# QuentinHuan/ENSEM3A_OpenCLRaytracer

Hardware: AMD Instinct MI355X
Metric: Msamples/s Cornell box 1024x1024 64spp; 1/2/4/8-GPU scaling; HBM %peak (higher is better)
Workload: dtype f32; 1 GPU; cornell_1024_s64; scene=cornell, width=1024, height=1024, spp=64, max_bounce=4, traversal=fast, bvh=sah, parallelism=row-interleaved x1

## Files before the change

### ensem3a_openclraytracer_amd/_native.py

```python
from __future__ import annotations

import ctypes
import os
import threading

import numpy as np

from ._build import LIB

_lock = threading.Lock()
_lib = None
_host = None

RT_TRAVERSAL_FAST = 0
RT_TRAVERSAL_REF = 1
RT_BVH_REFERENCE = 0
RT_BVH_SAH = 1
RT_ERR_ARG = 1
RT_ERR_STATE = 3
RT_ACCUM_MAX_SAMPLES = 1 << 24

EXPORTED = (
    "rt_create", "rt_destroy", "rt_last_error", "rt_set_scene", "rt_set_env", "rt_set_option",
    "rt_render", "rt_render_device", "rt_tile_rows", "rt_count_work", "rt_count_work_detail", "rt_work_bytes", "rt_gamma",
    "rt_render_rgb8", "rt_rgb8_device", "rt_rgb8",
    "rt_accum_begin", "rt_accum_add", "rt_accum_add_rgb8", "rt_accum_read", "rt_accum_samples", "rt_accum_end",
    "rt_accum_begin_device", "rt_accum_add_device",
    "rt_accum_mark", "rt_accum_select", "rt_accum_select_mask", "rt_accum_select_all", "rt_accum_selection",
    "rt_accum_sample_map", "rt_accum_add_selected", "rt_accum_mark_device", "rt_accum_select_device",
    "rt_accum_select_mask_device", "rt_accum_select_all_device", "rt_accum_add_selected_device",
    "rt_accum_guides", "rt_accum_guides_device", "rt_denoise_device", "rt_accum_denoise",
    "rt_trace", "rt_trace_device",
    "rt_bvh_build", "rt_device_count", "rt_debug_math", "rt_debug_fn", "rt_debug_trace", "rt_debug_scene_info", "rt_debug_pixel_log",
    "rt_debug_wave_counts", "rt_debug_quantise_axis", "rt_debug_timings", "rt_debug_brute_layout",
    "rt_debug_brute_clusters", "rt_debug_brute_shell", "rt_debug_brute_near", "rt_debug_brute_slices",
    "rt_debug_last_slices",
    "rt_debug_brute_refill", "rt_debug_last_refill", "rt_debug_last_launch",
    "rt_obj_parse", "rt_obj_size", "rt_obj_copy", "rt_obj_free", "rt_obj_last_error",
    "rt_scene_check", "rt_scene_last_error",
)
HOST_ONLY = ("rt_bvh_build", "rt_obj_parse", "rt_obj_size", "rt_obj_copy", "rt_obj_free", "rt_obj_last_error",
             "rt_scene_check", "rt_scene_last_error", "rt_debug_quantise_axis", "rt_debug_brute_layout",
             "rt_debug_brute_clusters", "rt_debug_brute_shell", "rt_debug_brute_near")

_c_p = ctypes.c_void_p
_i64 = ctypes.c_int64
_i32 = ctypes.c_int


class DenoiseParams(ctypes.Structure):
    _fields_ = [("passes", ctypes.c_int), ("normal_squarings", ctypes.c_int),
                ("sigma_c", ctypes.c_float), ("sigma_p", ctypes.c_float)]

    def __init__(self, passes: int = 5, normal_squarings: int = 5, sigma_c: float = 1.5, sigma_p: float = 0.02):
        super().__init__(int(passes), int(normal_squarings), float(sigma_c), float(sigma_p))


GUIDE_FLOATS = 12

HIT_DTYPE = np.dtype([("k", np.float32), ("tri", np.int32), ("u", np.float32), ("v", np.float32)])
RAY_FLOATS = 8
RT_QUERY_CLOSEST = 0
RT_QUERY_ANY = 1
QUERY_HORIZON = 1000.0


def pack_rays(origins, directions, tmax=None) -> np.ndarray:
    o = np.asarray(origins, dtype=np.float32).reshape(-1, 3)
    d = np.asarray(directions, dtype=np.float32).reshape(-1, 3)
    if len(o) != len(d):
        raise ValueError(f"{len(o)} origins but {len(d)} directions")
    rays = np.zeros((len(o), RAY_FLOATS), np.float32)
    rays[:, 0:3] = d
    rays[:, 3:6] = o
    rays[:, 6] = QUERY_HORIZON if tmax is None else np.asarray(tmax, dtype=np.float32)
    return rays


class NativeError(RuntimeError):

    def __init__(self, status: int, message: str):
        super().__init__(f"[rt status {status}] {message}")
        self.status = status


def _preload_hip_runtime() -> None:
    import importlib.util
    try:
        spec = importlib.util.find_spec("torch")
    except (ImportError, ValueError):
        spec = None
    for d in (spec.submodule_search_locations or []) if spec else []:
        p = os.path.join(d, "lib", "libamdhip64.so")
        if os.path.exists(p):
            ctypes.CDLL(p, mode=ctypes.RTLD_GLOBAL)
            return


def lib():
    global _lib
    if _lib is not None:
        return _lib
    with _lock:
        if _lib is not None:
            return _lib
        _preload_hip_runtime()
        lib_path = os.environ.get("ENSEM3A_RT_LIB", LIB)
        if not os.path.exists(lib_path):
            raise RuntimeError(
                f"native library {lib_path} is missing: build it with "
                "`python -m ensem3a_openclraytracer_amd._build` (there is no CPU fallback)")
        L = ctypes.CDLL(lib_path)
        sig = {
            "rt_create": (_i32, [_i32, _c_p, ctypes.POINTER(_c_p)]),
            "rt_destroy": (None, [_c_p]),
            "rt_last_error": (ctypes.c_char_p, [_c_p]),
            "rt_set_scene": (_i32, [_c_p, _c_p, _i64, _c_p, _i64, _c_p, _i64, _c_p, _i64, _c_p, _i64, _c_p, _i64]),
            "rt_set_env": (_i32, [_c_p, _c_p, _i32, _i32]),
            "rt_set_option": (_i32, [_c_p, ctypes.c_char_p, _i64]),
            "rt_render": (_i32, [_c_p, _c_p, _c_p, _i64, _i32, _i32, _c_p]),
            "rt_render_device": (_i32, [_c_p, _i32, _c_p, _c_p, _i64, _i32, _i32, _i32, _i32, _c_p, _c_p]),
            "rt_tile_rows": (_i64, [_i64, _i32, _i32, _i32]),
            "rt_count_work": (_i32, [_c_p, _c_p, _c_p, _i64, _i32, _i32, _i32, _i32, _c_p]),
            "rt_count_work_detail": (_i32, [_c_p, _c_p, _c_p, _i64, _i32, _i32, _i32, _i32, _c_p]),
            "rt_work_bytes": (_i32, [_c_p, _c_p]),
            "rt_gamma": (_i32, [_c_p, _c_p, _c_p, _i64]),
            "rt_render_rgb8": (_i32, [_c_p, _c_p, _c_p, _i64, _i32, _i32, _i32, _c_p]),
            "rt_rgb8_device": (_i32, [_c_p, _i32, _c_p, _c_p, _i64, _i32, _c_p]),
            "rt_rgb8": (_i32, [_c_p, _c_p, _c_p, _i64, _i32]),
            "rt_accum_begin": (_i32, [_c_p, _c_p, _c_p, _i64, _i32]),
            "rt_accum_add": (_i32, [_c_p, _i32, _c_p]),
            "rt_accum_add_rgb8": (_i32, [_c_p, _i32, _i32, _c_p]),
            "rt_accum_read": (_i32, [_c_p, _c_p]),
            "rt_accum_samples": (_i64, [_c_p]),
            "rt_accum_end": (_i32, [_c_p]),
            "rt_accum_begin_device": (_i32, [_c_p, _i32, _c_p, _c_p, _i64, _i32, _i32, _i32]),
            "rt_accum_add_device": (_i32, [_c_p, _i32, _i32, _c_p, _c_p]),
            "rt_accum_mark": (_i32, [_c_p]),
            "rt_accum_select": (_i32, [_c_p, ctypes.c_float, ctypes.POINTER(_i64)]),
            "rt_accum_select_mask": (_i32, [_c_p, _c_p]),
            "rt_accum_select_all": (_i32, [_c_p]),
            "rt_accum_selection": (_i32, [_c_p, _c_p]),
            "rt_accum_sample_map": (_i32, [_c_p, _c_p]),
            "rt_accum_add_selected": (_i32, [_c_p, _i32, _c_p]),
            "rt_accum_mark_device": (_i32, [_c_p, _i32, _c_p]),
            "rt_accum_select_device": (_i32, [_c_p, _i32, ctypes.c_float, _c_p]),
            "rt_accum_select_mask_device": (_i32, [_c_p, _i32, _c_p, _c_p]),
            "rt_accum_select_all_device": (_i32, [_c_p, _i32, _c_p]),
            "rt_accum_add_selected_device": (_i32, [_c_p, _i32, _i32, _c_p, _c_p]),
            "rt_accum_guides": (_i32, [_c_p, _c_p]),
            "rt_accum_guides_device": (_i32, [_c_p, _i32, _c_p, _c_p]),
            "rt_denoise_device": (_i32, [_c_p, _i32, _c_p, _c_p, _i64, _i32, ctypes.POINTER(DenoiseParams), _c_p, _c_p]),
            "rt_accum_denoise": (_i32, [_c_p, ctypes.POINTER(DenoiseParams), _c_p]),
            "rt_trace": (_i32, [_c_p, _c_p, _i64, _i32, _c_p]),
            "rt_trace_device": (_i32, [_c_p, _i32, _c_p, _i64, _i32, _c_p, _c_p]),
            "rt_bvh_build": (_i32, [_c_p, _i64, _c_p, _i64, _c_p, ctypes.POINTER(_i64)]),
            "rt_device_count": (_i32, []),
            "rt_obj_parse": (_i32, [_c_p, _i64, ctypes.POINTER(_c_p)]),
            "rt_obj_size": (_i64, [_c_p, _i32]),
            "rt_obj_copy": (_i32, [_c_p, _c_p, _c_p, _c_p, _c_p]),
            "rt_obj_free": (None, [_c_p]),
            "rt_obj_last_error": (ctypes.c_char_p, []),
            "rt_scene_check": (_i32, [_c_p, _i64, _c_p, _i64, _c_p, _i64, _c_p, _i64, _c_p, _i64, _i32, _c_p]),
            "rt_scene_last_error": (ctypes.c_char_p, []),
            "rt_debug_brute_layout": (_i32, [_c_p, _i64, _c_p, _i64, _c_p, _i64, _c_p, _i64, _c_p, _i64, _i32, _c_p, _i64,
                                             _c_p]),
            "rt_debug_brute_clusters": (_i32, [_c_p, _i64, _c_p, _i64, _c_p, _i64, _c_p, _i64, _c_p, _i64, _i32, _i32,
                                               _c_p, _i64, _c_p, _i64, _c_p]),
            "rt_debug_brute_shell": (_i32, [_c_p, _i64, _c_p, _i64, _c_p, _i64, _c_p, _i64, _c_p, _i64, _i32, _i32, _i32,
                                            _c_p, _i64, _c_p]),
            "rt_debug_brute_near": (_i32, [_c_p, _i64, _c_p, _i64, _c_p, _i64, _c_p, _i64, _c_p, _i64, _i32, _i32, _i32,
                                           _c_p, _i64, _c_p, _c_p]),
            "rt_debug_brute_slices": (_i32, [_i64, _i64, _i32, _i32, _i32, _c_p]),
            "rt_debug_last_slices": (_i32, []),
            "rt_debug_brute_refill": (_i32, [_i64, _i64, _i32, _c_p]),
            "rt_debug_last_refill": (_i32, [_c_p]),
            "rt_debug_last_launch": (_i32, [_c_p]),
            "rt_debug_math": (_i32, [_c_p, _i32, _c_p, _c_p, _c_p, _i64]),
            "rt_debug_fn": (_i32, [_c_p, _i32, _c_p, _c_p, _i64]),
            "rt_debug_trace": (_i32, [_c_p, _i32, _c_p, _c_p, _i64]),
            "rt_debug_scene_info": (_i32, [_c_p, _c_p]),
            "rt_debug_timings": (_i32, [_c_p, _c_p]),
            "rt_debug_wave_counts": (_i32, [_c_p, _c_p, _c_p, _i64, _i32, _i32, _c_p]),
            "rt_debug_pixel_log": (_i32, [_c_p, _i32, _c_p, _c_p, _i64, _i32, _i32, _i64, _c_p, _i32, _c_p, _c_p]),
        }
        _bind(L, sig)
        _lib = L
    return _lib


_HOST_SIG = {}


def _bind(L, sig, names=None):
    for name, (res, args) in sig.items():
        if names is not None and name not in names:
            continue
        fn = getattr(L, name)
        fn.restype = res
        fn.argtypes = args
        if name in HOST_ONLY:
            _HOST_SIG[name] = (res, args)


def host_lib():
    global _host
    if _host is not None:
        return _host
    L = lib()
    path = os.environ.get("ENSEM3A_HOST_LIB")
    if path:
        with _lock:
            if _host is None:
                H = ctypes.CDLL(path)
                _bind(H, _HOST_SIG)
                _host = H
        return _host
    _host = L
    return _host


def check(status: int, ctx=None) -> None:
    if status != 0:
        msg = lib().rt_last_error(ctx)
        raise NativeError(status, msg.decode(errors="replace") if msg else "unknown error")


def f32(a) -> np.ndarray:
    return np.ascontiguousarray(a, dtype=np.float32)


def i32(a) -> np.ndarray:
    return np.ascontiguousarray(a, dtype=np.int32)


def ptr(a: np.ndarray):
    return a.ctypes.data if a is not None and a.size else None


def device_count() -> int:
    return int(lib().rt_device_count())


class Context:

    def __init__(self, n_devices: int = 1, device_ids=None):
        ids = None
        if device_ids is not None:
            ids = (ctypes.c_int * len(device_ids))(*device_ids)
            n_devices = len(device_ids)
        out = _c_p()
        check(lib().rt_create(int(n_devices), ids, ctypes.byref(out)))
        self._ctx = out
        self.n_devices = int(n_devices)

# ... 286 lines not shown

    def wave_counts(self, cam, env, npix, spp, max_bounce):
        c, e = f32(cam), f32(env)
        out = np.zeros(9, dtype=np.uint64)
        self._check(lib().rt_debug_wave_counts(self.handle, ptr(c), ptr(e), int(npix), int(spp), int(max_bounce),
                                               out.ctypes.data))
        keys = ("node_fetches", "tri_tests", "rays", "env_lookups", "stack_drops", "wave_trav_iters",
                "wave_render_iters", "cycles_shade", "cycles_trav")
        return {k: int(v) for k, v in zip(keys, out)}

    def scene_info(self):
        out = np.zeros(8, dtype=np.int64)
        self._check(lib().rt_debug_scene_info(self.handle, out.ctypes.data))
        return dict(fast_ok=bool(out[0]), depth=int(out[1]), nodes=int(out[2]), tris=int(out[3]),
                    brute_records=int(out[4]), brute_boxes=int(out[5]), wdq_omax=int(out[6]) * 1e-6)

    def timings(self) -> dict:
        out = np.zeros(4, dtype=np.float64)
        self._check(lib().rt_debug_timings(self.handle, out.ctypes.data))
        return dict(pack_ms=float(out[0]), upload_ms=float(out[1]), env_ms=float(out[2]), render_ms=float(out[3]))


def parse_obj(text):
    data = text.encode() if isinstance(text, str) else bytes(text)
    h = _c_p()
    H = host_lib()
    if H.rt_obj_parse(data, len(data), ctypes.byref(h)) != 0:
        raise ValueError("OBJ parse failed: " + H.rt_obj_last_error().decode(errors="replace"))
    try:
        n = [int(H.rt_obj_size(h, k)) for k in range(5)]
        vp, vn, vuv = (np.zeros(n[k], np.float32) for k in range(3))
        face = np.zeros(n[3], np.int32)
        H.rt_obj_copy(h, vp.ctypes.data, vn.ctypes.data, vuv.ctypes.data, face.ctypes.data)
    finally:
        H.rt_obj_free(h)
    return vp, vn, vuv, face, n[4]


def scene_check(V_p, V_n, faceData, materialData, bvh, layout: int = RT_BVH_SAH) -> dict:
    vp, vn, face, mat, b = f32(V_p), f32(V_n), i32(faceData), f32(materialData), f32(bvh)
    info = np.zeros(8, np.int64)
    H = host_lib()
    st = H.rt_scene_check(ptr(vp), vp.size, ptr(vn), vn.size, ptr(face), face.size, ptr(mat), mat.size,
                          ptr(b), b.size, int(layout), info.ctypes.data)
    msg = H.rt_scene_last_error().decode(errors="replace")
    if st != 0:
        raise NativeError(st, msg)
    return dict(tris=int(info[0]), nodes=int(info[1]), depth=int(info[2]), wnodes=int(info[3]),
                wdepth=int(info[4]), brute_records=int(info[5]), brute_boxes=int(info[6]), fast_ok=bool(info[7]),
                note=msg)


def brute_layout(V_p, V_n, faceData, materialData, bvh, layout: int = RT_BVH_SAH):
    vp, vn, face, mat, b = f32(V_p), f32(V_n), i32(faceData), f32(materialData), f32(bvh)
    H = host_lib()
    info = np.zeros(3, np.int64)
    args = (ptr(vp), vp.size, ptr(vn), vn.size, ptr(face), face.size, ptr(mat), mat.size, ptr(b), b.size, int(layout))
    st = H.rt_debug_brute_layout(*args, None, 0, info.ctypes.data)
    if st != 0:
        raise NativeError(st, H.rt_scene_last_error().decode(errors="replace"))
    boxes = np.zeros(int(info[2]), np.float32)
    st = H.rt_debug_brute_layout(*args, boxes.ctypes.data, boxes.size, info.ctypes.data)
    if st != 0:
        raise NativeError(st, H.rt_scene_last_error().decode(errors="replace"))
    return boxes.reshape(-1, 8), int(info[0]), int(info[1])


def brute_clusters(V_p, V_n, faceData, materialData, bvh, cluster: int = -1, layout: int = RT_BVH_SAH):
    vp, vn, face, mat, b = f32(V_p), f32(V_n), i32(faceData), f32(materialData), f32(bvh)
    H = host_lib()
    info = np.zeros(4, np.int64)
    args = (ptr(vp), vp.size, ptr(vn), vn.size, ptr(face), face.size, ptr(mat), mat.size, ptr(b), b.size, int(layout),
            int(cluster))
    st = H.rt_debug_brute_clusters(*args, None, 0, None, 0, info.ctypes.data)
    if st != 0:
        raise NativeError(st, H.rt_scene_last_error().decode(errors="replace"))
    slots, rows = np.zeros(int(info[2]), np.float32), np.zeros(int(info[3]), np.float32)
    st = H.rt_debug_brute_clusters(*args, slots.ctypes.data, slots.size, rows.ctypes.data, rows.size, info.ctypes.data)
    if st != 0:
        raise NativeError(st, H.rt_scene_last_error().decode(errors="replace"))
    return slots.reshape(-1, 8), rows.reshape(-1, 8), int(info[1])


SHELL_REC_FLOATS = 20


def brute_shell(V_p, V_n, faceData, materialData, bvh, cluster: int = -1, shell: int = -1, layout: int = RT_BVH_SAH):
    vp, vn, face, mat, b = f32(V_p), f32(V_n), i32(faceData), f32(materialData), f32(bvh)
    H = host_lib()
    info = np.zeros(3, np.int64)
    args = (ptr(vp), vp.size, ptr(vn), vn.size, ptr(face), face.size, ptr(mat), mat.size, ptr(b), b.size, int(layout),
            int(cluster), int(shell))
    st = H.rt_debug_brute_shell(*args, None, 0, info.ctypes.data)
    if st != 0:
        raise NativeError(st, H.rt_scene_last_error().decode(errors="replace"))
    if int(info[0]) == 0:
        return None
    rec = np.zeros(int(info[2]), np.float32)
    st = H.rt_debug_brute_shell(*args, rec.ctypes.data, rec.size, info.ctypes.data)
    if st != 0:
        raise NativeError(st, H.rt_scene_last_error().decode(errors="replace"))
    ints = rec[:SHELL_REC_FLOATS].view(np.int32)
    return dict(box=rec[:6].copy(), nrest=int(ints[6]), nfaces=int(ints[7]), faces=ints[8:20].reshape(6, 2).copy(),
                rest=rec[SHELL_REC_FLOATS:].reshape(-1, 8).copy())


NEAR_FLOOR = np.float32(0.0001) * (np.float32(1.0) - np.float32(2.0 ** -12))


def brute_near(V_p, V_n, faceData, materialData, bvh, cluster: int = -1, shell: int = -1, layout: int = RT_BVH_SAH):
    vp, vn, face, mat, b = f32(V_p), f32(V_n), i32(faceData), f32(materialData), f32(bvh)
    H = host_lib()
    info = np.zeros(2, np.int64)
    floor = np.zeros(1, np.float32)
    args = (ptr(vp), vp.size, ptr(vn), vn.size, ptr(face), face.size, ptr(mat), mat.size, ptr(b), b.size, int(layout),
            int(cluster), int(shell))
    st = H.rt_debug_brute_near(*args, None, 0, floor.ctypes.data, info.ctypes.data)
    if st != 0:
        raise NativeError(st, H.rt_scene_last_error().decode(errors="replace"))
    flags = np.zeros(int(info[0]), np.int32)
    st = H.rt_debug_brute_near(*args, flags.ctypes.data if flags.size else None, flags.size, floor.ctypes.data,
                               info.ctypes.data)
    if st != 0:
        raise NativeError(st, H.rt_scene_last_error().decode(errors="replace"))
    return flags.astype(bool), np.float32(floor[0]), int(info[1])


def brute_slices(nloc: int, lanes: int, spp: int, option: int = -1, accum_base: int = -1):
    out = np.zeros(3, np.int32)
    st = lib().rt_debug_brute_slices(int(nloc), int(lanes), int(spp), int(option), int(accum_base), out.ctypes.data)
    if st != 0:
        raise NativeError(st, "rt_debug_brute_slices: bad arguments")
    return bool(out[0]), int(out[1]), int(out[2])


def last_slices() -> int:
    return int(lib().rt_debug_last_slices())


def brute_refill(nloc: int, lanes: int, option: int = -1) -> int:
    out = np.zeros(1, np.int32)
    st = lib().rt_debug_brute_refill(int(nloc), int(lanes), int(option), out.ctypes.data)
    if st != 0:
        raise NativeError(st, "rt_debug_brute_refill: bad arguments")
    return int(out[0])


def last_refill():
    out = np.zeros(3, np.int64)
    st = lib().rt_debug_last_refill(out.ctypes.data)
    if st != 0:
        raise NativeError(st, "rt_debug_last_refill: bad arguments")
    return int(out[0]), int(out[1]), int(out[2])


LAUNCH_FIELDS = ("trav", "count", "log", "smem", "ovf", "resume", "step", "wide", "brute", "ts", "acc",
                 "team", "walk_team", "slices", "refill", "grid", "lds", "shell", "near")
BRUTE_SLICED = 4
BRUTE_REFILL = 8


def last_launch() -> dict:
    out = np.zeros(len(LAUNCH_FIELDS), np.int32)
    st = lib().rt_debug_last_launch(out.ctypes.data)
    if st != 0:
        raise NativeError(st, "rt_debug_last_launch: bad arguments")
    return {name: int(v) for name, v in zip(LAUNCH_FIELDS, out)}


def tile_rows(npix: int, width: int, row0: int, row_step: int) -> int:
    return int(lib().rt_tile_rows(int(npix), int(width), int(row0), int(row_step)))
```

### ensem3a_openclraytracer_amd/csrc/rt_api.hip

```cpp
#include <hip/hip_runtime.h>

#include <cmath>
#include <cstdarg>
#include <cstdio>
#include <algorithm>
#include <array>
#include <atomic>
#include <chrono>
#include <cstring>
#include <map>
#include <string>
#include <thread>
#include <vector>

#include "../../include/rt_api.h"
#include "../../include/rt_debug.h"
#include "rt_internal.h"
#include "scene_pack.h"

constexpr int kResumeMinBvh2 = 36, kResumeMinWide = 48;
constexpr int kDenoiseLds = 1;

using rt::HostScene;

namespace {

thread_local std::string g_thread_error;

struct DevBuf {
    void* p = nullptr;
    size_t bytes = 0;
    DevBuf() = default;
    DevBuf(const DevBuf&) = delete;
    DevBuf& operator=(const DevBuf&) = delete;
    DevBuf(DevBuf&& o) noexcept : p(o.p), bytes(o.bytes) { o.p = nullptr, o.bytes = 0; }
    DevBuf& operator=(DevBuf&& o) noexcept {
        std::swap(p, o.p);
        std::swap(bytes, o.bytes);
        return *this;
    }
    ~DevBuf() { release(); }
    void release() {
        if (p) (void)hipFree(p);
        p = nullptr;
        bytes = 0;
    }
};

struct Device {
    int id = 0;
    hipStream_t stream = nullptr;
    int cus = 0;
    DevBuf stack_ovf;
    DevBuf nodes, wnodes, wleaves, tri_fast, brute, brute_box, brute_cbox, brute_crow, bvh9, tri_geo, tri_shade, tri_frame, mat, ibl, ibl_sum, out, out8, counts, work, scratch_a, scratch_b;
    DevBuf pilot;
    DevBuf spec;
    DevBuf slice;
    DevBuf accum;
    bool acc_open = false;
    bool acc_valid = false;
    float acc_cam[10] = {0}, acc_env[5] = {0};
    int64_t acc_npix = 0, acc_nloc = 0, acc_samples = 0;
    int acc_max_bounce = 0, acc_row0 = 0, acc_row_step = 1;
    DevBuf mark, sel, all;
    bool acc_marked = false, acc_selected = false, acc_all_ready = false;
    bool acc_uniform = true;
    bool sel_all = false;
    int64_t sel_known = -1;
    int64_t acc_full = 0;
    DevBuf dn, dn_const, guides, dn_rgb, dn_guides, dn_out;
    DevBuf q_counter, q_rays, q_out;
    char* host_stage = nullptr;
    int* host_pick = nullptr;
    size_t host_stage_bytes = 0;
    hipEvent_t done = nullptr;
    hipStream_t last = nullptr;
    bool pending = false;

    Device() = default;
    Device(const Device&) = delete;
    Device& operator=(const Device&) = delete;
    ~Device() {
        (void)hipSetDevice(id);
        if (host_stage) (void)hipHostFree(host_stage);
        if (host_pick) (void)hipHostFree(host_pick);
        if (stream) (void)hipStreamDestroy(stream);
        if (done) (void)hipEventDestroy(done);
    }
};

}

struct rt_ctx {
    std::vector<Device> devs;
    HostScene hs;
    bool have_scene = false;
    bool have_env = false;
    int ibl_w = 0, ibl_h = 0;
    int traversal = RT_TRAVERSAL_FAST;
    int bvh_layout = RT_BVH_SAH;
    int brute_max = RT_BRUTE_MAX_DEFAULT;
    int brute_cluster = -1;
    int brute_shell = -1;
    int brute_near = -1;
    int resume_min = -1;
    int team = 0;
    int walk_team = 0;
    int max_waves = 0;
    int step = 0;
    int sun_skip = 1;
    int sun_any = 1;
    int block = 128;
    int bvh_width = 0;
    int fixed_point = 1;
    int sun_cache = 1;
    int pilot = -1;
    int pilot_chunk = 0;
    int pilot_levels = 0;
    int stack_lds = 0;
    int ref_stack = 20;
    int spec = -1;
    int wdq = 1;
    int handout = -1;
    int slices = -1;
    int brute_refill = -1;
    int denoise_lds = -1;
    int query_engine = 0;
    int query_grid = 0;
    bool accum_host = false;
    double t_pack_ms = 0, t_upload_ms = 0, t_env_ms = 0, t_render_ms = 0;
    std::string err;
};

namespace {

int set_err(rt_ctx* ctx, int code, const char* fmt, ...) {
    char buf[1024];
    va_list ap;
    va_start(ap, fmt);
    vsnprintf(buf, sizeof buf, fmt, ap);
    va_end(ap);
    if (ctx) ctx->err = buf;
    g_thread_error = buf;
    return code;
}

#define HIP_OR_RET(ctx, call)                                                                           \
    do {                                                                                                \
        hipError_t e_ = (call);                                                                         \
        if (e_ != hipSuccess)                                                                           \
            return set_err((ctx), RT_ERR_HIP, "%s failed: %s", #call, hipGetErrorString(e_));           \
    } while (0)

hipError_t grow(Device& d, DevBuf& b, size_t bytes) {
    bytes = std::max<size_t>(bytes, 16);
    if (b.p && b.bytes >= bytes) return hipSuccess;
    hipError_t e = d.pending ? hipEventSynchronize(d.done) : hipSuccess;
    if (e != hipSuccess) return e;
    if (b.p && (e = hipFree(b.p)) != hipSuccess) return e;
    b.p = nullptr;
    b.bytes = 0;
    if ((e = hipMalloc(&b.p, bytes)) == hipSuccess) b.bytes = bytes;
    return e;
}

hipError_t grow_stage(Device& d, size_t bytes) {
    if (d.host_stage_bytes >= bytes) return hipSuccess;
    hipError_t e = d.host_stage ? hipHostFree(d.host_stage) : hipSuccess;
    if (e != hipSuccess) return e;
    d.host_stage = nullptr;
    d.host_stage_bytes = 0;
    if ((e = hipHostMalloc((void**)&d.host_stage, bytes, hipHostMallocDefault)) == hipSuccess) d.host_stage_bytes = bytes;
    return e;
}

}

namespace {

constexpr int kStackLdsMin = 8;
hipError_t ensure_stack_ovf(Device& d, const HostScene& hs) {
    const int64_t extra = (int64_t)std::max(hs.depth, hs.wdepth) - kStackLdsMin;
    if (extra <= 0) return hipSuccess;
    return grow(d, d.stack_ovf, (size_t)std::max(d.cus, 1) * rt::kMaxLanesPerCu * (size_t)extra * sizeof(int2));
}

hipError_t order_after_last(Device& d, hipStream_t s) {
// ... 6 lines not shown
    d.pending = true;
    return hipEventRecord(d.done, s);
}

template <typename T>
hipError_t upload(Device& d, DevBuf& b, const std::vector<T>& v) {
    const size_t bytes = v.size() * sizeof(T);
    hipError_t e = grow(d, b, bytes);
    if (e != hipSuccess || bytes == 0) return e;
    return hipMemcpyAsync(b.p, v.data(), bytes, hipMemcpyHostToDevice, d.stream);
}

hipError_t upload_cbox(Device& d, const HostScene& hs) {
    if (hs.brute_shell.empty()) return upload(d, d.brute_cbox, hs.brute_cbox);
    std::vector<float> v(hs.brute_cbox);
    v.insert(v.end(), hs.brute_shell.begin(), hs.brute_shell.end());
    const hipError_t e = upload(d, d.brute_cbox, v);
    return e != hipSuccess ? e : hipStreamSynchronize(d.stream);
}

int upload_fast(rt_ctx* ctx, Device& d, const HostScene& hs) {
    HIP_OR_RET(ctx, hipSetDevice(d.id));
    HIP_OR_RET(ctx, order_after_last(d, d.stream));
    HIP_OR_RET(ctx, upload(d, d.nodes, hs.nodes));
    HIP_OR_RET(ctx, upload(d, d.wnodes, hs.wnodes));
    HIP_OR_RET(ctx, upload(d, d.wleaves, hs.wleaves));
    HIP_OR_RET(ctx, upload(d, d.brute, hs.brute));
    HIP_OR_RET(ctx, upload(d, d.brute_box, hs.brute_box));
    HIP_OR_RET(ctx, upload_cbox(d, hs));
    HIP_OR_RET(ctx, upload(d, d.brute_crow, hs.brute_crow));
    HIP_OR_RET(ctx, upload(d, d.tri_geo, hs.tri_geo));
    HIP_OR_RET(ctx, upload(d, d.tri_fast, hs.tri_fast));
    HIP_OR_RET(ctx, ensure_stack_ovf(d, hs));
    return RT_OK;
}

int effective_traversal(const rt_ctx* ctx) {
    return (ctx->traversal == RT_TRAVERSAL_FAST && ctx->hs.fast_ok) ? RT_TRAVERSAL_FAST : RT_TRAVERSAL_REF;
}

bool use_wide(const rt_ctx* ctx) {
    if (ctx->hs.wnodes.empty() || ctx->bvh_width == 2) return false;
    return ctx->bvh_width == 4 || (size_t)ctx->hs.nnodes * 16 * rt::kNodeF4 > rt::kWideMinBytes;
}

int resume_min_of(const rt_ctx* ctx) {
    return ctx->resume_min >= 0 ? ctx->resume_min : use_wide(ctx) ? kResumeMinWide : kResumeMinBvh2;
}

rt::DevScene dev_scene(const rt_ctx* ctx, const Device& d) {
    rt::DevScene s{};
    s.nodes = (const float4*)d.nodes.p;
    s.nnodes = ctx->hs.nnodes;
    s.root_ref = ctx->hs.root_ref;
    const bool wide = use_wide(ctx);
    s.wnodes = wide ? (const float4*)d.wnodes.p : nullptr;
    s.wleaves = wide ? (const float4*)d.wleaves.p : nullptr;
    s.wroot_ref = ctx->hs.wroot_ref;
    s.wdq_omax = wide ? ctx->hs.wdq_omax : 0.0f;
    for (int k = 0; k < 6; ++k) s.root_box[k] = ctx->hs.root_box[k];
    s.bvh9 = (const float*)d.bvh9.p;
    s.nbvh9 = ctx->hs.nbvh9;
    s.ref_stack = ctx->ref_stack;
    s.tri_geo = (const float4*)d.tri_geo.p;
    s.tri_fast = (const float4*)d.tri_fast.p;
    s.tri_shade = (const float4*)d.tri_shade.p;
    s.tri_frame = (const float4*)d.tri_frame.p;
    s.ntri = ctx->hs.ntri;
    s.mat = (const float*)d.mat.p;
    s.nmat = ctx->hs.nmat;
    s.ibl_sum = (const uint32_t*)d.ibl_sum.p;
    s.ibl_w = ctx->ibl_w;
    s.ibl_h = ctx->ibl_h;
    s.depth = wide ? std::max(ctx->hs.depth, ctx->hs.wdepth) : ctx->hs.depth;
    s.brute = (const float4*)d.brute.p;
    s.brute_box = (const float4*)d.brute_box.p;
    s.nbrute = ctx->hs.nbrute;
    s.nbox = ctx->hs.nbox;
    s.brute_cbox = (const float4*)d.brute_cbox.p;
    s.brute_crow = (const float4*)d.brute_crow.p;
    s.ncluster = ctx->hs.ncluster;
    s.ncslot = (int32_t)(ctx->hs.brute_cbox.size() / 8);
    s.nsingle4 = s.ncslot - rt::kClusterSlots * s.ncluster;
    s.cluster_auto = ctx->brute_cluster < 0 ? 1 : 0;
    s.nsingle = ctx->hs.nsingle;
    s.shell = ctx->hs.nshell > 0 ? 2 * s.ncslot : 0;
    s.near_floor = s.shell && ctx->brute_near != 0 ? ctx->hs.shell_floor : 0.0f;
    s.near_mask_lo = s.near_floor != 0.0f ? (uint32_t)ctx->hs.shell_mask : 0u;
    s.near_mask_hi = s.near_floor != 0.0f ? (uint32_t)(ctx->hs.shell_mask >> 32) : 0u;
    s.stack_lds = std::min<int32_t>(s.depth > 0 ? s.depth : 1,
                                    ctx->stack_lds > 0 ? ctx->stack_lds : wide ? rt::kStackLdsWide : rt::kStackLds);
    s.stack_ovf = (int2*)d.stack_ovf.p;
    return s;
}

int check_frame(rt_ctx* ctx, const float* cam, const float* env, int64_t npix, int spp, int max_bounce, int row0,
                int row_step, rt::FrameParams* fp) {
    if (!ctx) return set_err(nullptr, RT_ERR_ARG, "null context");
    if (!ctx->have_scene) return set_err(ctx, RT_ERR_STATE, "rt_set_scene has not been called");
    if (!ctx->have_env) return set_err(ctx, RT_ERR_STATE, "rt_set_env has not been called");
    if (!cam || !env) return set_err(ctx, RT_ERR_ARG, "cam/env must not be NULL");
    if (!(cam[6] >= 1.0f) || !(cam[6] < 2147483648.0f))
        return set_err(ctx, RT_ERR_ARG, "cam[6] (row width) must be >= 1, got %g", (double)cam[6]);
    if (npix <= 0 || npix > 0x7fffffff) return set_err(ctx, RT_ERR_ARG, "pixel count %lld out of range", (long long)npix);
    if (spp < 0) return set_err(ctx, RT_ERR_ARG, "spp must be >= 0");
    if (row0 < 0 || row_step <= 0) return set_err(ctx, RT_ERR_ARG, "bad row tiling (%d, %d)", row0, row_step);
    if (max_bounce > 4096) return set_err(ctx, RT_ERR_ARG, "maxBounce %d > 4096", max_bounce);
    std::memcpy(fp->cam, cam, sizeof fp->cam);
    std::memcpy(fp->env, env, sizeof fp->env);
    fp->width = (int32_t)cam[6];
    fp->npix = npix;
    fp->spp = spp;
    fp->max_bounce = max_bounce;
    fp->row0 = row0;
    fp->row_step = row_step;
    fp->nloc = rt_tile_rows(npix, fp->width, row0, row_step) * fp->width;
    fp->log_pixel = -1;
    fp->resume_min = resume_min_of(ctx);
    fp->step = ctx->step;
    fp->sun_skip = (ctx->sun_skip && env[3] == 0.0f && env[4] >= 0.0f && ctx->hs.colors_finite) ? 1 : 0;
    fp->sun_any = (ctx->sun_any && !ctx->hs.has_glass) ? 1 : 0;
    fp->wide = use_wide(ctx) ? 1 : 0;
    fp->wdq = ctx->wdq;
    fp->fixed_point = ctx->fixed_point;
    fp->sun_cache = ctx->fixed_point && ctx->sun_cache ? 1 : 0;
    fp->pass = 0;
    fp->pilot = 0;
    fp->pilot_chunk = 1;
    fp->pilot_levels = 256;
    fp->pilot_state = nullptr;
    fp->pilot_draws = nullptr;
    fp->spec = 0;
    fp->spec_log = nullptr;
    fp->spec_cap = 0;
    fp->slices = 0;
    fp->refill = ctx->brute_refill;
    fp->slice_state = nullptr;
    fp->slice_ready = nullptr;
    fp->pilot_cost = nullptr;
    fp->pilot_order = nullptr;
    fp->team = ctx->team;
    fp->walk_team = ctx->walk_team;
    fp->max_waves = ctx->max_waves;
    fp->handout = ctx->handout >= 0 ? ctx->handout : (use_wide(ctx) && effective_traversal(ctx) == RT_TRAVERSAL_FAST);
    fp->log_buf = nullptr;
    fp->log_cap = 0;
    fp->log_count = nullptr;
    return RT_OK;
}

void invalidate_accum(rt_ctx* ctx) {
    for (auto& d : ctx->devs) {
        d.acc_valid = false;
        d.acc_marked = false;
        d.acc_selected = false;
    }
}

int slot_of(rt_ctx* ctx, int device_index, Device** d, const char* what = "device index") {
    if (!ctx) return set_err(nullptr, RT_ERR_ARG, "null context");
    if (device_index < 0 || device_index >= (int)ctx->devs.size())
        return set_err(ctx, RT_ERR_ARG, "%s %d out of range", what, device_index);
    *d = &ctx->devs[device_index];
    return RT_OK;
}

int repack_scene(rt_ctx* ctx) {
    if (!ctx->have_scene) return RT_OK;
    HostScene& hs = ctx->hs;
    std::string why;
    rt::pack_checked(hs, hs.bvh9.data(), hs.nbvh9, hs.ntri, ctx->bvh_layout, ctx->brute_max, ctx->brute_cluster,
                     ctx->brute_shell, why);
    for (auto& d : ctx->devs) {
        const int st = upload_fast(ctx, d, hs);
        if (st) return st;
        HIP_OR_RET(ctx, hipStreamSynchronize(d.stream));
    }
    if (!hs.fast_ok) ctx->err = "FAST traversal unavailable (" + why + "); REF traversal will be used";
    return RT_OK;
}

struct Accepts {
    enum Kind { kRange, kZeroOrRange, kSet } kind;
    int n;
    int64_t v[5];
    bool operator()(int64_t x) const {
        if (kind == kSet) return std::find(v, v + n, x) != v + n;
        return (kind == kZeroOrRange && x == 0) || (x >= v[0] && x <= v[1]);
    }
};
Accepts range(int64_t lo, int64_t hi) { return {Accepts::kRange, 2, {lo, hi}}; }
Accepts zero_or(int64_t lo, int64_t hi) { return {Accepts::kZeroOrRange, 2, {lo, hi}}; }
Accepts one_of(std::initializer_list<int64_t> members) {
    Accepts a{Accepts::kSet, (int)members.size(), {}};
    std::copy(members.begin(), members.end(), a.v);
    return a;
}

enum class Effect { kNone, kInvalidate, kRepack };

struct Option {
    const char* key;
    int rt_ctx::*field;
    Accepts accepts;
    std::string message;
    Effect effect;
};

std::string bounds_message(const char* fmt, int a, int b = 0) {
    char buf[128];
    snprintf(buf, sizeof buf, fmt, a, b);
    return buf;
}

const std::vector<Option>& options() {
    constexpr Effect none = Effect::kNone, invalidate = Effect::kInvalidate, repack = Effect::kRepack;
    static const std::vector<Option> table = {
        {"traversal", &rt_ctx::traversal, range(RT_TRAVERSAL_FAST, RT_TRAVERSAL_REF), "traversal must be 0 (fast) or 1 (ref)", invalidate},
        {"brute_near", &rt_ctx::brute_near, range(-1, 1), "brute_near must be -1 (auto), 0 (off) or 1 (auto)", none},
        {"bvh", &rt_ctx::bvh_layout, range(RT_BVH_REFERENCE, RT_BVH_SAH), "bvh must be 0 (reference tree) or 1 (sah)", repack},
        {"brute_cluster", &rt_ctx::brute_cluster, range(-1, 1), "brute_cluster must be -1 (auto), 0 (off) or 1 (force)", repack},
        {"brute_shell", &rt_ctx::brute_shell, range(-1, 1), "brute_shell must be -1 (auto), 0 (off) or 1 (force)", repack},
        {"brute_max", &rt_ctx::brute_max, range(0, 4096), "brute_max must be in 0..4096", repack},
        {"resume_min", &rt_ctx::resume_min, range(-1, 64), "resume_min must be -1 (auto) or 0..64", none},
        {"team", &rt_ctx::team, one_of({0, 1, 2, 4, 8}), "team must be 0 (auto), 1, 2, 4 or 8", none},
        {"walk_team", &rt_ctx::walk_team, one_of({0, 1, 2, 4, 8}), "walk_team must be 0 (auto), 1, 2, 4 or 8", none},
        {"sun_any", &rt_ctx::sun_any, range(0, 1), "sun_any must be 0 or 1", none},
        {"sun_skip", &rt_ctx::sun_skip, range(0, 1), "sun_skip must be 0 or 1", none},
        {"step", &rt_ctx::step, range(0, 2), "step must be 0 (auto), 1 (item) or 2 (round)", none},
        {"waves", &rt_ctx::max_waves, range(0, 8), "waves must be in 0..8", none},
        {"pilot", &rt_ctx::pilot, range(-1, 1 << 20), "pilot must be -1 (auto), 0 (off) or a sample count", none},
        {"pilot_chunk", &rt_ctx::pilot_chunk, range(0, 4096), "pilot_chunk must be in 0..4096 (0 = auto)", none},
        {"pilot_levels", &rt_ctx::pilot_levels, zero_or(2, 256), "pilot_levels must be 0 (auto) or 2..256", none},
        {"stack_lds", &rt_ctx::stack_lds, zero_or(kStackLdsMin, rt::kStackLds),
         bounds_message("stack_lds must be 0 (auto) or %d..%d", kStackLdsMin, rt::kStackLds), none},
        {"sun_cache", &rt_ctx::sun_cache, range(0, 1), "sun_cache must be 0 or 1", none},
        {"fixed_point", &rt_ctx::fixed_point, range(0, 1), "fixed_point must be 0 or 1", none},
        {"bvh_width", &rt_ctx::bvh_width, one_of({0, 2, 4}), "bvh_width must be 0 (auto), 2 or 4", none},
        {"ref_stack", &rt_ctx::ref_stack, range(20, 64), "ref_stack must be in 20..64 (20 = the reference's)", invalidate},
        {"slices", &rt_ctx::slices, range(-1, 16), "slices must be -1 (auto), 0 (off) or 1..16", none},
        {"brute_refill", &rt_ctx::brute_refill, range(-1, rt::kRefillMax),
         bounds_message("brute_refill must be -1 (auto), 0 or 1 (off) or 2..%d", rt::kRefillMax), none},
        {"denoise_lds", &rt_ctx::denoise_lds, range(-1, 1), "denoise_lds must be -1 (auto), 0 or 1", none},
        {"query_engine", &rt_ctx::query_engine, range(0, 2), "query_engine must be 0 (auto), 1 (plain) or 2 (persistent)", none},
        {"query_grid", &rt_ctx::query_grid, range(0, 1 << 20), "query_grid must be 0 (auto) or a block count", none},
        {"wdq", &rt_ctx::wdq, range(0, 1), "wdq must be 0 or 1", none},
        {"handout", &rt_ctx::handout, range(-1, 1), "handout must be -1 (auto), 0 or 1", none},
        {"spec", &rt_ctx::spec, one_of({-1, 0, 2, 4, 8}), "spec must be -1 (auto), 0 (off), 2, 4 or 8", none},
        {"block", &rt_ctx::block, one_of({64, 128, 256}), "block must be 64/128/256", none},
    };
    return table;
}

}

extern "C" {

int rt_device_count(void) {
    int n = 0;
    if (hipGetDeviceCount(&n) != hipSuccess) return 0;
    return n;
}

int rt_create(int n_devices, const int* device_ids, rt_ctx** out) {
    if (!out) return set_err(nullptr, RT_ERR_ARG, "out must not be NULL");
    *out = nullptr;
    int avail = 0;
    hipError_t e = hipGetDeviceCount(&avail);
    if (e != hipSuccess || avail <= 0)
        return set_err(nullptr, RT_ERR_HIP, "no HIP device available (%s)", hipGetErrorString(e));
    if (n_devices <= 0) n_devices = 1;
    if (!device_ids && n_devices > avail)
        return set_err(nullptr, RT_ERR_ARG, "requested %d devices, %d available", n_devices, avail);
    if (n_devices > 64) return set_err(nullptr, RT_ERR_ARG, "at most 64 device slots, got %d", n_devices);
    rt_ctx* ctx = new rt_ctx();
    ctx->devs = std::vector<Device>(n_devices);
    for (int i = 0; i < n_devices; ++i) {
        const int id = device_ids ? device_ids[i] : i;
        if (id < 0 || id >= avail) {
            delete ctx;
            return set_err(nullptr, RT_ERR_ARG, "device id %d out of range", id);
        }
        ctx->devs[i].id = id;
        if ((e = hipSetDevice(id)) != hipSuccess ||
            (e = hipStreamCreateWithFlags(&ctx->devs[i].stream, hipStreamNonBlocking)) != hipSuccess ||
            (e = hipEventCreateWithFlags(&ctx->devs[i].done, hipEventDisableTiming)) != hipSuccess ||
            (e = hipDeviceGetAttribute(&ctx->devs[i].cus, hipDeviceAttributeMultiprocessorCount, id)) != hipSuccess) {
            rt_destroy(ctx);
            return set_err(nullptr, RT_ERR_HIP, "device %d init failed: %s", id, hipGetErrorString(e));
        }
    }
    *out = ctx;
    return RT_OK;
}

void rt_destroy(rt_ctx* ctx) {
    if (!ctx) return;
    for (auto& d : ctx->devs) {
        if (hipSetDevice(d.id) != hipSuccess) continue;
        if (d.pending) (void)hipEventSynchronize(d.done);
        if (d.stream) (void)hipStreamSynchronize(d.stream);
    }
    delete ctx;
}

const char* rt_last_error(rt_ctx* ctx) { return ctx ? ctx->err.c_str() : g_thread_error.c_str(); }

int rt_set_option(rt_ctx* ctx, const char* key, int64_t value) {
    if (!ctx || !key) return set_err(ctx, RT_ERR_ARG, "null argument");
    for (const Option& o : options()) {
        if (std::strcmp(key, o.key)) continue;
        if (!o.accepts(value)) return set_err(ctx, RT_ERR_ARG, "%s", o.message.c_str());
        ctx->*o.field = (int)value;
        if (o.effect == Effect::kInvalidate) invalidate_accum(ctx);
        return o.effect == Effect::kRepack ? repack_scene(ctx) : RT_OK;
    }
    return set_err(ctx, RT_ERR_ARG, "unknown option '%s'", key);
}

int rt_set_scene(rt_ctx* ctx, const float* vp, int64_t nvp, const float* vn, int64_t nvn, const float* vuv,
                 int64_t nvuv, const int32_t* face, int64_t nface, const float* mat, int64_t nmat, const float* bvh9,
                 int64_t nbvh) {
    (void)vuv;
    (void)nvuv;
    if (!ctx) return set_err(nullptr, RT_ERR_ARG, "null context");
    const auto t0 = std::chrono::steady_clock::now();
    HostScene hs;
    std::string msg, why;
    const int rc = rt::scene_prepare(hs, vp, nvp, vn, nvn, face, nface, mat, nmat, bvh9, nbvh, ctx->bvh_layout,
                                     ctx->brute_max, ctx->brute_cluster, ctx->brute_shell, msg, why);
    if (rc != RT_OK) return set_err(ctx, rc, "%s", msg.c_str());
    invalidate_accum(ctx);
    const auto t1 = std::chrono::steady_clock::now();
    for (auto& d : ctx->devs) {
        const int st = upload_fast(ctx, d, hs);
        if (st) return st;
        HIP_OR_RET(ctx, upload(d, d.bvh9, hs.bvh9));
        HIP_OR_RET(ctx, upload(d, d.tri_shade, hs.tri_shade));
        HIP_OR_RET(ctx, upload(d, d.mat, hs.mat));
        HIP_OR_RET(ctx, grow(d, d.tri_frame, (size_t)std::max<int64_t>(hs.ntri, 1) * 3 * sizeof(float4)));
        HIP_OR_RET(ctx, grow(d, d.work, rt::kWorkBytes));
        HIP_OR_RET(ctx, hipStreamSynchronize(d.stream));
    }
    ctx->hs = std::move(hs);
    for (auto& d : ctx->devs) {
        HIP_OR_RET(ctx, hipSetDevice(d.id));
        HIP_OR_RET(ctx, rt::launch_prep_frames(dev_scene(ctx, d), (float4*)d.tri_frame.p, d.stream));
        HIP_OR_RET(ctx, hipStreamSynchronize(d.stream));
    }
    ctx->have_scene = true;
    ctx->t_pack_ms = std::chrono::duration<double, std::milli>(t1 - t0).count();
    ctx->t_upload_ms = std::chrono::duration<double, std::milli>(std::chrono::steady_clock::now() - t1).count();
    if (!ctx->hs.fast_ok) ctx->err = "FAST traversal unavailable (" + why + "); REF traversal will be used";
    return RT_OK;
}

int rt_set_env(rt_ctx* ctx, const uint8_t* rgba, int w, int h) {
    if (!ctx) return set_err(nullptr, RT_ERR_ARG, "null context");
    if (!rgba || w <= 0 || h <= 0) return set_err(ctx, RT_ERR_ARG, "bad IBL image (%d x %d)", w, h);
    const size_t bytes = (size_t)w * h * 4;
    invalidate_accum(ctx);
    const auto t0 = std::chrono::steady_clock::now();
    for (auto& d : ctx->devs) {
        HIP_OR_RET(ctx, hipSetDevice(d.id));
        HIP_OR_RET(ctx, order_after_last(d, d.stream));
        HIP_OR_RET(ctx, grow(d, d.ibl, bytes));
        HIP_OR_RET(ctx, grow(d, d.ibl_sum, (size_t)(w + 1) * (size_t)(h + 1) * sizeof(uint32_t)));
        HIP_OR_RET(ctx, hipMemcpyAsync(d.ibl.p, rgba, bytes, hipMemcpyHostToDevice, d.stream));
        HIP_OR_RET(ctx, rt::launch_ibl_sum((const uchar4*)d.ibl.p, w, h, (uint32_t*)d.ibl_sum.p, d.stream));
        HIP_OR_RET(ctx, hipStreamSynchronize(d.stream));
    }
    ctx->ibl_w = w;
    ctx->ibl_h = h;
    ctx->have_env = true;
    ctx->t_env_ms = std::chrono::duration<double, std::milli>(std::chrono::steady_clock::now() - t0).count();
    return RT_OK;
}

int64_t rt_tile_rows(int64_t npix, int width, int row0, int row_step) {
    if (npix <= 0 || width <= 0 || row0 < 0 || row_step <= 0) return 0;
    const int64_t H = (npix + width - 1) / width;
    if (row0 >= H) return 0;
    return (H - row0 + row_step - 1) / row_step;
}

namespace {
constexpr int kSlicesWide = 8;
constexpr int kSlicesWideSmall = 12;
constexpr int64_t kSlicesMinPerLane = 4;
using rt::kAccumSliceMin;

hipError_t setup_pilot(rt_ctx* ctx, Device& d, rt::FrameParams& fp) {
    if (ctx->pilot == 0 || effective_traversal(ctx) != RT_TRAVERSAL_FAST || fp.nloc <= 0 || use_wide(ctx))
        return hipSuccess;
    int k = ctx->pilot;
    if (k < 0) {
        const int64_t lanes = (int64_t)std::max(d.cus, 1) * rt::kWalkLanesPerCu;
        if (ctx->hs.nbrute > 0 || use_wide(ctx) || fp.spp < 16 || fp.nloc > 16 * lanes) return hipSuccess;
        if (ctx->slices != 0 && fp.nloc >= kSlicesMinPerLane * lanes) return hipSuccess;
        k = fp.spp / 8;
    }
    if (k >= fp.spp) return hipSuccess;
    const size_t n = (size_t)fp.nloc;
    const size_t need = n * 40 + 2 * 256 * sizeof(uint32_t) + 2 * (n + 1) * sizeof(uint32_t) +
                        (n + 256) * sizeof(uint32_t) + n * sizeof(uint32_t);
    hipError_t e = grow(d, d.pilot, need);
    if (e != hipSuccess) return e;
    char* base = (char*)d.pilot.p;
    fp.pilot = k;
    fp.pilot_chunk = ctx->pilot_chunk > 0 ? ctx->pilot_chunk : (ctx->hs.nbrute > 0 ? 64 : 1);
    fp.pilot_levels = ctx->pilot_levels > 0 ? ctx->pilot_levels : 256;
    fp.pilot_state = (float4*)base;
    fp.pilot_cost = (uint32_t*)(base + n * 32);
// ... 973 lines not shown
    Device& d = ctx->devs[0];
    HIP_OR_RET(ctx, hipSetDevice(d.id));
    const size_t ibytes = (size_t)n * wi * sizeof(float);
    const size_t obytes = ((size_t)n * wo * sizeof(float) + 15) & ~(size_t)15;
    HIP_OR_RET(ctx, grow(d, d.scratch_a, ibytes));
    HIP_OR_RET(ctx, grow(d, d.scratch_b, obytes + rt::debug_fn_scratch_bytes(fn, n)));
    HIP_OR_RET(ctx, hipMemcpyAsync(d.scratch_a.p, in, ibytes, hipMemcpyHostToDevice, d.stream));
    HIP_OR_RET(ctx, order_after_last(d, d.stream));
    HIP_OR_RET(ctx, rt::launch_debug_fn(dev_scene(ctx, d), fn, (const float*)d.scratch_a.p, (float*)d.scratch_b.p, n,
                                        (char*)d.scratch_b.p + obytes, d.stream));
    HIP_OR_RET(ctx, hipMemcpyAsync(out, d.scratch_b.p, (size_t)n * wo * sizeof(float), hipMemcpyDeviceToHost, d.stream));
    HIP_OR_RET(ctx, hipStreamSynchronize(d.stream));
    return RT_OK;
}

int rt_debug_trace(rt_ctx* ctx, int traversal, const float* rays, float* out, int64_t n) {
    if (!ctx || !rays || !out || n < 0) return set_err(ctx, RT_ERR_ARG, "bad arguments");
    if (!ctx->have_scene) return set_err(ctx, RT_ERR_STATE, "no scene");
    if (traversal == RT_TRAVERSAL_FAST && !ctx->hs.fast_ok)
        return set_err(ctx, RT_ERR_STATE, "FAST traversal unavailable for this scene");
    if (!n) return RT_OK;
    Device& d = ctx->devs[0];
    HIP_OR_RET(ctx, hipSetDevice(d.id));
    HIP_OR_RET(ctx, grow(d, d.scratch_a, (size_t)n * 6 * sizeof(float)));
    HIP_OR_RET(ctx, grow(d, d.scratch_b, (size_t)n * 2 * sizeof(float)));
    HIP_OR_RET(ctx, hipMemcpyAsync(d.scratch_a.p, rays, (size_t)n * 6 * sizeof(float), hipMemcpyHostToDevice, d.stream));
    HIP_OR_RET(ctx, order_after_last(d, d.stream));
    HIP_OR_RET(ctx, rt::launch_debug_trace(dev_scene(ctx, d), traversal, (const float*)d.scratch_a.p,
                                           (float*)d.scratch_b.p, n, d.stream));
    HIP_OR_RET(ctx, hipMemcpyAsync(out, d.scratch_b.p, (size_t)n * 2 * sizeof(float), hipMemcpyDeviceToHost, d.stream));
    HIP_OR_RET(ctx, hipStreamSynchronize(d.stream));
    return RT_OK;
}

int rt_debug_pixel_log(rt_ctx* ctx, int traversal, const float cam[10], const float env[5], int64_t npix, int spp,
                       int max_bounce, int64_t pixel, float* log, int cap, int* n_events, float out3[3]) {
    rt::FrameParams fp;
    if (!cam) return set_err(ctx, RT_ERR_ARG, "null cam");
    const int W = (int)cam[6];
    if (W <= 0 || pixel < 0 || pixel >= npix) return set_err(ctx, RT_ERR_ARG, "pixel out of range");
    int st = check_frame(ctx, cam, env, npix, spp, 0, (int)(pixel / W), (int)npix, &fp);
    if (st) return st;
    if (!log || cap <= 0 || !n_events || !out3) return set_err(ctx, RT_ERR_ARG, "bad log buffer");
    if (traversal == RT_TRAVERSAL_FAST && !ctx->hs.fast_ok) traversal = RT_TRAVERSAL_REF;
    fp.max_bounce = max_bounce;
    fp.sun_skip = 0;
    fp.sun_any = 0;
    Device& d = ctx->devs[0];
    HIP_OR_RET(ctx, hipSetDevice(d.id));
    const size_t obytes = (size_t)fp.nloc * 3 * sizeof(float);
    const size_t lbytes = (size_t)cap * 16 * sizeof(float);
    HIP_OR_RET(ctx, grow(d, d.scratch_a, obytes + lbytes + 16));
    float* dout = (float*)d.scratch_a.p;
    fp.log_buf = dout + fp.nloc * 3;
    fp.log_count = (int32_t*)(fp.log_buf + (size_t)cap * 16);
    fp.log_cap = cap;
    fp.log_pixel = pixel;
    HIP_OR_RET(ctx, hipMemsetAsync(fp.log_count, 0, sizeof(int32_t), d.stream));
    HIP_OR_RET(ctx, order_after_last(d, d.stream));
    HIP_OR_RET(ctx, rt::launch_debug_log(dev_scene(ctx, d), fp, traversal, dout, (unsigned int*)d.work.p, d.stream));
    HIP_OR_RET(ctx, mark_launch(d, d.stream));
    int32_t n = 0;
    HIP_OR_RET(ctx, hipMemcpyAsync(&n, fp.log_count, sizeof n, hipMemcpyDeviceToHost, d.stream));
    HIP_OR_RET(ctx, hipStreamSynchronize(d.stream));
    if (n > cap) n = cap;
    HIP_OR_RET(ctx, hipMemcpy(log, fp.log_buf, (size_t)n * 16 * sizeof(float), hipMemcpyDeviceToHost));
    HIP_OR_RET(ctx, hipMemcpy(out3, dout + 3 * (pixel % W), 3 * sizeof(float), hipMemcpyDeviceToHost));
    *n_events = n;
    return RT_OK;
}

int rt_debug_brute_slices(int64_t nloc, int64_t lanes, int spp, int option, int accum_base, int32_t out[3]) {
    if (!out || nloc < 0 || lanes < 0 || option < -1 || option > 16) return RT_ERR_ARG;
    const int todo = spp - std::max(accum_base, 0);
    const int v = rt::brute_slice_launch(rt::brute_slice_offer(option, todo, accum_base >= 0), nloc, lanes);
    out[0] = v != 0;
    out[1] = v & 0xff;
    out[2] = v >> 8;
    return RT_OK;
}

int rt_debug_last_slices(void) { return rt::last_launch().slices; }

int rt_debug_last_launch(int32_t out[19]) {
    if (!out) return RT_ERR_ARG;
    const rt::LaunchNote n = rt::last_launch();
    const rt::KernelKey& k = n.key;
    const int64_t v[19] = {k.trav, k.count, k.log,  k.smem,       k.ovf,    k.resume, k.step, k.wide,          k.brute,
                           k.ts,   k.acc,   n.team, n.walk_team,  n.slices, n.refill, n.grid, (int64_t)n.lds,
                           n.shell, n.near};
    for (int i = 0; i < 19; ++i) out[i] = (int32_t)std::min<int64_t>(v[i], INT32_MAX);
    return RT_OK;
}

int rt_debug_brute_refill(int64_t nloc, int64_t lanes, int option, int32_t* out) {
    if (!out || nloc < 0 || lanes < 0 || option < -1 || option > rt::kRefillMax) return RT_ERR_ARG;
    *out = rt::brute_refill_launch(option, nloc, lanes);
    return RT_OK;
}

int rt_debug_last_refill(int64_t out[3]) {
    if (!out) return RT_ERR_ARG;
    out[0] = rt::last_launch().refill;
    out[1] = g_refill_events.load(std::memory_order_relaxed);
    out[2] = g_refill_lanes.load(std::memory_order_relaxed);
    return RT_OK;
}

int rt_debug_timings(rt_ctx* ctx, double out[4]) {
    if (!ctx || !out) return set_err(ctx, RT_ERR_ARG, "bad arguments");
    out[0] = ctx->t_pack_ms;
    out[1] = ctx->t_upload_ms;
    out[2] = ctx->t_env_ms;
    out[3] = ctx->t_render_ms;
    return RT_OK;
}

int rt_debug_scene_info(rt_ctx* ctx, int64_t out[8]) {
    if (!ctx || !out) return set_err(ctx, RT_ERR_ARG, "bad arguments");
    out[0] = ctx->hs.fast_ok ? 1 : 0;
    out[1] = ctx->hs.depth;
    out[2] = ctx->hs.nnodes;
    out[3] = ctx->hs.ntri;
    out[4] = effective_traversal(ctx) == RT_TRAVERSAL_FAST ? ctx->hs.nbrute : 0;
    out[5] = out[4] ? ctx->hs.nbox : 0;
    out[6] = ctx->hs.wnodes.empty() ? 0 : (int64_t)std::llround((double)ctx->hs.wdq_omax * 1e6);
    out[7] = 0;
    return RT_OK;
}

}
```

### ensem3a_openclraytracer_amd/csrc/rt_device.h

```cpp
#pragma once
#include <algorithm>
#include <climits>

#include "rt_internal.h"
#include "rtm.h"

namespace rt {

namespace {

constexpr size_t kLdsSceneMax = 24 * 1024;

constexpr int TRAV_FAST = 0;
constexpr int TRAV_REF = 1;
constexpr int REF_STACK = 20;

struct Hit {
    float k;
    int tri;
};

struct Cnt {
    unsigned long long nodes, tris, rays, env, dropped;
    unsigned long long wave_trav;
// ... 261 lines not shown
    const char* const tb = reinterpret_cast<const char*>(tris);
    const unsigned kstride = SOA ? 16u * (unsigned)S.nnodes : 16u;
    const float ix = dev_recip(d.x), iy = dev_recip(d.y), iz = dev_recip(d.z);
    float tmin, tmax;
    slab(S.root_box[0], S.root_box[3], S.root_box[1], S.root_box[4], S.root_box[2], S.root_box[5], o, ix, iy, iz,
         tmin, tmax);
    if (!(tmax >= tmin && tmax >= 0.0f)) return best;
    int item = S.root_ref;
    unsigned soff = 0;
    while (true) {
        if (COUNT) count_wave(c.wave_trav);
        if (item >= 0) {
            if (COUNT) { c.nodes++; c.boxes += 2; }
            const char* np = nb + (SOA ? 16u : 16u * kNodeF4) * (unsigned)item;
            const int next = node_step<OVF>(np, kstride, o, ix, iy, iz, best.k * CULL_MARGIN, st, soff);
            if (next != INT_MIN) {
                item = next;
                continue;
            }
        } else {
            if (COUNT) c.tris++;
            float k;
            int rank;
            const unsigned toff = ~(unsigned)item;
            int index;
            if (mt_flat(tb, toff, o, d, &k, &rank, &index) && k > 0.0001f &&
                (k < best.k || (k == best.k && rank < best_rank))) {
                best.k = k;
                best.tri = 48 * index;
                best_rank = rank;
            }
        }
        item = 0x7fffffff;
        while (soff > 0) {
            soff -= sstride;
            const int2 en = st.template get<OVF>(soff);
            if (__int_as_float(en.y) <= best.k * CULL_MARGIN) {
                item = en.x;
                break;
            }
        }
        if (item == 0x7fffffff) break;
    }
    if (best.tri >= 0) best.tri = (int)((unsigned)best.tri / 48u);
    return best;
}

typedef const float __attribute__((address_space(4))) const_f;
struct ConstF4 {
    const const_f* p;
    __device__ __forceinline__ float4 operator[](int i) const {
        return make_float4(p[4 * i], p[4 * i + 1], p[4 * i + 2], p[4 * i + 3]);
    }
};
__device__ __forceinline__ ConstF4 as_const(const float4* p) {
    return ConstF4{(const const_f*)(const float*)(p)};
}

__device__ __forceinline__ float sgpr1(float x) {
    return __int_as_float(__builtin_amdgcn_readfirstlane(__float_as_int(x)));
}
__device__ __forceinline__ float4 sgpr4(float4 v) {
    return make_float4(sgpr1(v.x), sgpr1(v.y), sgpr1(v.z), sgpr1(v.w));
}

constexpr unsigned BRUTE_RING = 256u;
constexpr unsigned BRUTE_OWNERS = 128u;
constexpr int BRUTE_INV_OFF = 64 * 6 * 4 + 64 * 8 + (BRUTE_RING + 64) * 4;
constexpr int BRUTE_WAVE_LDS = BRUTE_INV_OFF + 64 * 3 * 4 + BRUTE_OWNERS * 4;
static_assert(kClusterLockNum >= 0 && kClusterLockNum <= 8 && BRUTE_OWNERS >= 64 + 64 / kClusterSlots + 2, "owner list");

__device__ __forceinline__ unsigned lane_prefix(unsigned long long m, unsigned base) {
    return __builtin_amdgcn_mbcnt_hi((unsigned)(m >> 32), __builtin_amdgcn_mbcnt_lo((unsigned)m, base));
}

__device__ __forceinline__ void wave_lds_sync() {
    __builtin_amdgcn_fence(__ATOMIC_SEQ_CST, "wavefront");
    __builtin_amdgcn_wave_barrier();
}

__device__ __forceinline__ float near_floor_of(const DevScene& S, int g) {
    const uint32_t m = g < 32 ? S.near_mask_lo : S.near_mask_hi;
    return g < 64 && ((m >> (g & 31)) & 1u) ? kNearFloor : 0.0f;
}

template <int N> struct IntC { static constexpr int value = N; };
static_assert(kBoxGroup == 1 || kBoxGroup == 2 || kBoxGroup == 4 || kBoxGroup == 8, "the lock-step tail is cut into powers of two");

template <bool COUNT, bool CLU = false>
__device__ Hit trace_brute_compact(const DevScene& S, rtm_f3 o, rtm_f3 d, char* wl, const float4* mtrec,
                                   unsigned mtstride, Cnt& c, int ts = 1, const float4* boxrec = nullptr) {
    const unsigned lane = threadIdx.x & 63;
    const unsigned sub = lane & (unsigned)(ts - 1), tl = lane - sub;
    if (COUNT && sub == 0) c.rays++;
    const unsigned long long act = __ballot(1);
    const int nact = __popcll(act);
    const int myrank = (int)lane_prefix(act, 0u);
    float* ray = reinterpret_cast<float*>(wl);
    unsigned long long* bestk = reinterpret_cast<unsigned long long*>(wl + 64 * 6 * 4);
    unsigned* ring = reinterpret_cast<unsigned*>(wl + 64 * 6 * 4 + 64 * 8);
    ray[0 * 64 + lane] = o.x; ray[1 * 64 + lane] = o.y; ray[2 * 64 + lane] = o.z;
    ray[3 * 64 + lane] = d.x; ray[4 * 64 + lane] = d.y; ray[5 * 64 + lane] = d.z;
    const unsigned long long nokey = ((unsigned long long)__float_as_uint(1000.0f) << 32) | 0xffffffffull;
    bestk[lane] = nokey;
    wave_lds_sync();
    const float ix = dev_recip(d.x), iy = dev_recip(d.y), iz = dev_recip(d.z);
    float bk = 1000.0f;
    unsigned head = 0, tail = 0;
    auto run_batch = [&](int n) __attribute__((always_inline)) {
        if (myrank < n) {
            const unsigned e = ring[(head + myrank) & (BRUTE_RING - 1)];
            const unsigned ow = e >> 16, q = e & 0xffffu;
            const rtm_f3 ro = rtm_v3(ray[ow], ray[64 + ow], ray[128 + ow]);
            const rtm_f3 rd = rtm_v3(ray[192 + ow], ray[256 + ow], ray[320 + ow]);
            const float4* rq = mtrec + mtstride * q;
            const float4 r1 = rq[0], r2 = rq[1], r3 = rq[2];
            const rtm_f3 a = rtm_v3(r1.z, r1.w, r2.x), e1 = rtm_v3(r2.y, r2.z, r2.w), e2 = rtm_v3(r3.x, r3.y, r3.z);
            const rtm_f3 h = rtm_cross(rd, e2);
            const float det = rtm_dot(e1, h);
            const float f = mt_recip(det);
            const rtm_f3 sv = rtm_sub(ro, a);
            const float u = f * rtm_dot(sv, h);
            const rtm_f3 qv = rtm_cross(sv, e1);
            const float v = f * rtm_dot(rd, qv);
            const float k = f * rtm_dot(e2, qv);
            const bool parallel = det > -0.0000001f && det < 0.0000001f;
            const bool hit = !parallel && !(u < 0.0f || u > 1.0f) && !(v < 0.0f || u + v > 1.0f) &&
                             (k > 0.0000001f) && k > 0.0001f && k < 1000.0f;
            if (hit) atomicMin(&bestk[ow], ((unsigned long long)__float_as_uint(k) << 32) | q);
        }
        head += n;
        wave_lds_sync();
    };
    auto enqueue = [&](bool pass, unsigned qa, int qb) __attribute__((always_inline)) {
        const unsigned long long m = __ballot(pass);
        if (m == 0) return;
        const unsigned n = (unsigned)__popcll(m);
        if (COUNT && pass) c.tris += qb >= 0 ? 2 : 1;
        const unsigned r = lane_prefix(m, tail);
        ring[pass ? (r & (BRUTE_RING - 1)) : BRUTE_RING + lane] = (tl << 16) | qa;
        if (qb >= 0) ring[pass ? ((r + n) & (BRUTE_RING - 1)) : BRUTE_RING + lane] = (tl << 16) | (unsigned)qb;
        tail += qb >= 0 ? 2 * n : n;
        wave_lds_sync();
        if ((int)(tail - head) >= nact) {
            do run_batch(nact); while ((int)(tail - head) >= nact);
            bk = __uint_as_float((unsigned)(bestk[tl] >> 32));
        }
    };
    auto group = [&](auto wc, const ConstF4 cb, int g0, int nreal) __attribute__((always_inline)) {
        constexpr int W = decltype(wc)::value;
        float4 bx[2 * W];
#pragma unroll
        for (int j = 0; j < 2 * W; ++j) bx[j] = sgpr4(cb[2 * g0 + j]);
        const float cull = bk * CULL_MARGIN;
        bool pass[W];
#pragma unroll
        for (int j = 0; j < W; ++j) {
            float tn, tx;
            slab(bx[2 * j].x, bx[2 * j].y, bx[2 * j].z, bx[2 * j].w, bx[2 * j + 1].x, bx[2 * j + 1].y, o, ix, iy, iz,
                 tn, tx);
            if constexpr (COUNT && !CLU) pass[j] = fmaxf(tn, near_floor_of(S, g0 + j)) <= fminf(tx, cull);
            else pass[j] = box_hit(tn, tx, cull);
        }
#pragma unroll
        for (int j = 0; j < W; ++j) {
            if (COUNT && g0 + j >= nreal) break;
            const int qa = __float_as_int(bx[2 * j + 1].z), qb = __float_as_int(bx[2 * j + 1].w);
            if (COUNT) {
                c.boxes++;
                count_wave(c.wave_trav); c.nodes++;
                if (qb >= 0) { count_wave(c.wave_trav); c.nodes++; }
            }
            enqueue(pass[j], (unsigned)qa, qb);
        }
    };
    auto lockstep_padded = [&](const ConstF4 cb, int gb, int ge) __attribute__((always_inline)) {
        for (int g0 = gb; g0 < ge; g0 += kBoxGroup) group(IntC<kBoxGroup>{}, cb, g0, ge);
    };
    auto lockstep = [&](const ConstF4 cb, int gb, int ge) __attribute__((always_inline)) {
        int g0 = gb;
        for (; g0 + kBoxGroup <= ge; g0 += kBoxGroup) group(IntC<kBoxGroup>{}, cb, g0, ge);
        const int rem = ge - g0;
        if constexpr (kBoxGroup > 4) if (rem & 4) group(IntC<4>{}, cb, g0 + (rem & ~7), ge);
        if constexpr (kBoxGroup > 2) if (rem & 2) group(IntC<2>{}, cb, g0 + (rem & ~3), ge);
        if constexpr (kBoxGroup > 1) if (rem & 1) group(IntC<1>{}, cb, g0 + (rem & ~1), ge);
    };
    if (CLU) {
        float* inv = reinterpret_cast<float*>(wl + BRUTE_INV_OFF);
        unsigned* olist = reinterpret_cast<unsigned*>(wl + BRUTE_INV_OFF + 64 * 3 * 4);
        const unsigned* besthi = reinterpret_cast<const unsigned*>(bestk) + 1;
        inv[lane] = ix; inv[64 + lane] = iy; inv[128 + lane] = iz;
        const ConstF4 cb = as_const(S.brute_cbox);
        ConstF4 sb = cb;
        int ns = S.nsingle;
        if (S.shell) {
            const ConstF4 sh{cb.p + 4 * S.shell};
            const float4 h0 = sgpr4(sh[0]), h1 = sgpr4(sh[1]), fx = sgpr4(sh[2]), fy = sgpr4(sh[3]), fz = sgpr4(sh[4]);
            const float cull = bk * CULL_MARGIN, nearf = S.near_floor;
            const float x0 = (h0.x - o.x) * ix, x1 = (h0.y - o.x) * ix;
            const float y0 = (h0.z - o.y) * iy, y1 = (h0.w - o.y) * iy;
            const float z0 = (h1.x - o.z) * iz, z1 = (h1.y - o.z) * iz;
            const float t[6] = {x0, x1, y0, y1, z0, z1};
            const float mn[3] = {fminf(x0, x1), fminf(y0, y1), fminf(z0, z1)};
            const float mx[3] = {fmaxf(x0, x1), fmaxf(y0, y1), fmaxf(z0, z1)};
            const int q[12] = {__float_as_int(fx.x), __float_as_int(fx.y), __float_as_int(fx.z), __float_as_int(fx.w),
                               __float_as_int(fy.x), __float_as_int(fy.y), __float_as_int(fy.z), __float_as_int(fy.w),
                               __float_as_int(fz.x), __float_as_int(fz.y), __float_as_int(fz.z), __float_as_int(fz.w)};
            bool pass[6];
#pragma unroll
            for (int f = 0; f < 6; ++f) {
                const int a = f >> 1;
                const float tn = fmaxf(fmaxf(a == 0 ? t[f] : mn[0], a == 1 ? t[f] : mn[1]), a == 2 ? t[f] : mn[2]);
                const float tx = fminf(fminf(a == 0 ? t[f] : mx[0], a == 1 ? t[f] : mx[1]), a == 2 ? t[f] : mx[2]);
                pass[f] = fmaxf(tn, nearf) <= fminf(tx, cull);
            }
            unsigned long long many = 0;
            int npass = 0;
#pragma unroll
            for (int f = 0; f < 6; ++f) {
                const unsigned long long mf = __ballot(pass[f]);
                many |= mf;
                npass += __popcll(mf);
            }
            if (npass == __popcll(many)) {
                unsigned pk = ~0u;
#pragma unroll
                for (int f = 0; f < 6; ++f) pk = pass[f] ? ((unsigned)q[2 * f] | ((unsigned)q[2 * f + 1] << 16)) : pk;
                const bool p1 = pk != ~0u, p2 = pk < 0xffff0000u;
                const unsigned long long m1 = __ballot(p1);
                if (m1 != 0) {
                    const unsigned long long m2 = __ballot(p2);
                    const unsigned n1 = (unsigned)__popcll(m1);
                    if (COUNT && p1) c.tris += p2 ? 2 : 1;
                    const unsigned r1 = lane_prefix(m1, tail), r2 = lane_prefix(m2, tail + n1);
                    ring[p1 ? (r1 & (BRUTE_RING - 1)) : BRUTE_RING + lane] = (tl << 16) | (pk & 0xffffu);
                    ring[p2 ? (r2 & (BRUTE_RING - 1)) : BRUTE_RING + lane] = (tl << 16) | (pk >> 16);
                    tail += n1 + (unsigned)__popcll(m2);
                    wave_lds_sync();
                    if ((int)(tail - head) >= nact) {
                        do run_batch(nact); while ((int)(tail - head) >= nact);
                        bk = __uint_as_float((unsigned)(bestk[tl] >> 32));
                    }
                }
            } else {
#pragma unroll
                for (int f = 0; f < 6; ++f)
                    if (q[2 * f] >= 0) enqueue(pass[f], (unsigned)q[2 * f], q[2 * f + 1]);
            }
            sb = ConstF4{sh.p + kShellRecF};
            ns = __float_as_int(h1.z);
        }
        lockstep(sb, 0, ns);
        unsigned ihead = 0, itail = 0;
        auto run_items = [&](int n) __attribute__((always_inline)) {
            bool pass = false;
            unsigned ow = 0, qa = 0;
            int qb = -1;
            if (myrank < n) {
                const unsigned i = ihead + (unsigned)myrank;
                const unsigned e = olist[(i >> kClusterShift) & (BRUTE_OWNERS - 1)];
                ow = e & 63u;
                const unsigned slot = (e >> 8) + (i & (unsigned)(kClusterSlots - 1));
                const rtm_f3 ro = rtm_v3(ray[ow], ray[64 + ow], ray[128 + ow]);
                const float4 b0 = boxrec[2 * slot], b1 = boxrec[2 * slot + 1];
                float tn, tx;
                slab(b0.x, b0.y, b0.z, b0.w, b1.x, b1.y, ro, inv[ow], inv[64 + ow], inv[128 + ow], tn, tx);
                pass = box_hit(tn, tx, __uint_as_float(besthi[2 * ow]) * CULL_MARGIN);
                qa = (unsigned)__float_as_int(b1.z);
                qb = __float_as_int(b1.w);
            }
            ihead += (unsigned)n;
            const bool pass2 = pass && qb >= 0;
            const unsigned long long m = __ballot(pass), m2 = __ballot(pass2);
            if (m == 0) return;
            const unsigned np = (unsigned)__popcll(m);
            if (pass) ring[lane_prefix(m, tail) & (BRUTE_RING - 1)] = (ow << 16) | qa;
            if (pass2) ring[lane_prefix(m2, tail + np) & (BRUTE_RING - 1)] = (ow << 16) | (unsigned)qb;
            tail += np + (unsigned)__popcll(m2);
            wave_lds_sync();
            if ((int)(tail - head) >= nact) {
                do run_batch(nact); while ((int)(tail - head) >= nact);
                bk = __uint_as_float((unsigned)(bestk[tl] >> 32));
            }
        };
        const ConstF4 cr = as_const(S.brute_crow);
        const int lock = (nact * kClusterLockNum) >> 3;
        for (int cl = 0; cl < S.ncluster; ++cl) {
            const float4 u0 = sgpr4(cr[2 * cl]), u1 = sgpr4(cr[2 * cl + 1]);
            float tn, tx;
            slab(u0.x, u0.y, u0.z, u0.w, u1.x, u1.y, o, ix, iy, iz, tn, tx);
            const bool pass = box_hit(tn, tx, bk * CULL_MARGIN);
            const unsigned long long m = __ballot(pass);
            if (m == 0) continue;
            const int np = __popcll(m);
            const int first = __float_as_int(u1.z);
            if (np > lock) {
                lockstep(cb, first, first + __float_as_int(u1.w));
                continue;
            }
            if (pass) olist[lane_prefix(m, itail >> kClusterShift) & (BRUTE_OWNERS - 1)] = lane | ((unsigned)first << 8);
            itail += (unsigned)np << kClusterShift;
            wave_lds_sync();
            while ((int)(itail - ihead) >= nact) run_items(nact);
        }
        while (itail != ihead) run_items(min((int)(itail - ihead), nact));
    } else if (ts == 1) {
        lockstep_padded(as_const(S.brute_box), 0, S.nbox);
    } else {
        const int rounds = (S.nbox + ts - 1) / ts;
        for (int gg = 0; gg < rounds; ++gg) {
            if (COUNT) { count_wave(c.wave_trav); count_wave(c.wave_trav); }
            const int g = gg * ts + (int)sub;
            bool pass = false;
            int qa = 0, qb = -1;
            if (g < S.nbox) {
                const float4 b0 = boxrec[2 * g], b1 = boxrec[2 * g + 1];
                float tn, tx;
                slab(b0.x, b0.y, b0.z, b0.w, b1.x, b1.y, o, ix, iy, iz, tn, tx);
                if constexpr (COUNT) pass = fmaxf(tn, near_floor_of(S, g)) <= fminf(tx, bk * CULL_MARGIN);
                else pass = box_hit(tn, tx, bk * CULL_MARGIN);
                qa = __float_as_int(b1.z);
                qb = __float_as_int(b1.w);
                if (COUNT) { c.nodes += qb >= 0 ? 2 : 1; c.boxes++; }
            }
            enqueue(pass, (unsigned)qa, -1);
            enqueue(pass && qb >= 0, (unsigned)qb, -1);
        }
    }
    while (tail != head) run_batch(min((int)(tail - head), nact));
    const unsigned long long key = bestk[tl];
    Hit best{1000.0f, -1};
    if (key != nokey) {
        best.k = __uint_as_float((unsigned)(key >> 32));
        best.tri = __float_as_int(mtrec[mtstride * (unsigned)(key & 0xffffffffu) + 2].w);
    }
    return best;
}

template <int TRAV, bool COUNT, bool SOA = false, bool OVF = false, bool BLDS = false, bool CLU = false>
__device__ __forceinline__ Hit trace(const DevScene& S, const float4* nodes, const float4* tris, rtm_f3 o, rtm_f3 d,
                                     int* stk, int B, const LaneStack& st, Cnt& c, const float4* mtrec = nullptr,
                                     int ts = 1, const float4* boxrec = nullptr) {
    if (TRAV == TRAV_REF) return trace_ref<COUNT>(S, o, d, stk, B, c);
    if (S.nbrute > 0)
        return trace_brute_compact<COUNT, CLU>(S, o, d, reinterpret_cast<char*>(stk - threadIdx.x) +
                                                        (threadIdx.x >> 6) * BRUTE_WAVE_LDS,
                                          BLDS ? mtrec : S.brute + 1, BLDS ? 3u : 4u, c, BLDS ? ts : 1, boxrec);
    return trace_fast<COUNT, SOA, OVF>(S, nodes, tris, o, d, st, c);
}

struct LaunchConst {
    rtm_rot cam_rx, cam_ry, cam_rz;
    rtm_rot ibl_x, ibl_y;
    rtm_f3 focal, position, sun;
    float pas;
};

__host__ __device__ inline LaunchConst make_const(const FrameParams& F) {
    LaunchConst c;
    const float* cam = F.cam;
    c.focal = rtm_v3(cam[0], cam[1] - (1.0f / (2.0f * rtm_tan(cam[9] / 2.0f))), cam[2]);
    c.position = rtm_v3(cam[0], cam[1], cam[2]);
    c.pas = 1.0f / cam[6];
    c.cam_rx = rtm_rot_prepare(cam[3] * (3.14f / 180.0f), rtm_v3(1, 0, 0));
    c.cam_ry = rtm_rot_prepare(cam[4] * (3.14f / 180.0f), rtm_v3(0, 1, 0));
    c.cam_rz = rtm_rot_prepare(cam[5] * (3.14f / 180.0f), rtm_v3(0, 0, 1));
    c.ibl_x = rtm_rot_prepare(90.0f * (3.14f / 180.0f), rtm_v3(1, 0, 0));
    c.ibl_y = rtm_rot_prepare(90.0f * (3.14f / 180.0f), rtm_v3(0, 1, 0));
    rtm_f3 sun = rtm_v3(1, 1, 1);
    sun = rtm_rotate(F.env[0] * (3.14f / 180.0f), rtm_v3(1, 0, 0), sun);
    sun = rtm_rotate(F.env[1] * (3.14f / 180.0f), rtm_v3(0, 1, 0), sun);
    sun = rtm_rotate(F.env[2] * (3.14f / 180.0f), rtm_v3(0, 0, 1), sun);
    c.sun = sun;
    return c;
}

__global__ void make_const_kernel(FrameParams F, LaunchConst* __restrict__ out) {
    if (blockIdx.x == 0 && threadIdx.x == 0) *out = make_const(F);
}

inline size_t stack_lds_bytes(const DevScene& sc, int traversal, int block) {
    const int depth = traversal == TRAV_REF ? sc.ref_stack : (sc.nbrute > 0 ? 1 : 2 * std::max(sc.stack_lds, 1));
    const size_t lds = (size_t)depth * block * sizeof(int);
    return traversal == TRAV_FAST && sc.nbrute > 0 ? std::max(lds, (size_t)(block / 64) * BRUTE_WAVE_LDS) : lds;
}
inline size_t brute_lds_bytes(const DevScene& sc, int block) {
    return (size_t)(block / 64) * BRUTE_WAVE_LDS + (size_t)sc.nbrute * 48 + (size_t)sc.nbox * 32 +
           (size_t)sc.ntri * 64 + (size_t)sc.nmat * (4 * kMatF) + (size_t)sc.ncslot * 32;
}
inline size_t staged_scene_bytes(const DevScene& sc) {
    return (size_t)(kNodeF4 * sc.nnodes + 3 * sc.ntri) * sizeof(float4);
}

inline hipError_t setup_work_block(const FrameParams& f, unsigned int* d_work, hipStream_t stream,
                                   const LaunchConst** lconst) {
    static_assert(kConstOffset >= kGroups * kCounterStride && kConstOffset + sizeof(LaunchConst) <= kWorkBytes,
                  "work block layout");
    const hipError_t e = hipMemsetAsync(d_work, 0, (size_t)kGroups * kCounterStride, stream);
    if (e != hipSuccess) return e;
    LaunchConst* lc = reinterpret_cast<LaunchConst*>(reinterpret_cast<char*>(d_work) + kConstOffset);
    hipLaunchKernelGGL(make_const_kernel, dim3(1), dim3(64), 0, stream, f, lc);
    *lconst = lc;
    return hipGetLastError();
}

__device__ __forceinline__ rtm_f3 camera_dir(const LaunchConst& C, int W, int i) {
    const int pixelY = (i + 1) % W;
    const int pixelX = (i - pixelY) / W;
    const rtm_f3 pc = rtm_v3(fmaf((float)pixelY, C.pas, -0.5f), 0.0f, fmaf(-(float)pixelX, C.pas, 0.5f));
    rtm_f3 d = dev_normalize(rtm_sub(rtm_add(C.position, pc), C.focal));
    d = rtm_rot_apply(C.cam_rx, d);
    d = rtm_rot_apply(C.cam_ry, d);
    return rtm_rot_apply(C.cam_rz, d);
}

__global__ void ibl_sum_kernel(const uchar4* __restrict__ rgba, int w, int h, uint32_t* __restrict__ sum) {
    const int64_t n = (int64_t)(w + 1) * (h + 1);
    for (int64_t q = (int64_t)blockIdx.x * blockDim.x + threadIdx.x; q < n; q += (int64_t)gridDim.x * blockDim.x) {
        const int X = (int)(q % (w + 1)), Y = (int)(q / (w + 1));
        const int x0 = max(min(X - 1, w - 1), 0), x1 = min(X, w - 1);
        const int y0 = max(min(Y - 1, h - 1), 0), y1 = min(Y, h - 1);
        const uchar4 t00 = rgba[(int64_t)y0 * w + x0], t10 = rgba[(int64_t)y0 * w + x1];
        const uchar4 t01 = rgba[(int64_t)y1 * w + x0], t11 = rgba[(int64_t)y1 * w + x1];
        const uint32_t r = (uint32_t)t00.x + t10.x + t01.x + t11.x;
        const uint32_t g = (uint32_t)t00.y + t10.y + t01.y + t11.y;
        const uint32_t b = (uint32_t)t00.z + t10.z + t01.z + t11.z;
        sum[q] = r | (g << 10) | (b << 20);
    }
}

template <bool COUNT>
__device__ rtm_f3 sample_ibl(const DevScene& S, const LaunchConst& C, rtm_f3 dir, Cnt& c) {
    if (COUNT) c.env++;
    dir = rtm_rot_apply(C.ibl_x, dir);
    dir = rtm_rot_apply(C.ibl_y, dir);
    float u = rtm_atan2(dir.z, dir.x), v = rtm_asin(dir.y);
    u = u * 0.1591f;
    v = v * 0.3183f;
    u = u + 0.5f;
    v = v + 0.5f;
    const int W = S.ibl_w, H = S.ibl_h;
    const int x = rtm_f2i(u * (float)W);
    const int y = rtm_f2i(v * (float)H);
    const int X = min(max(x, 0), W), Y = min(max(y, 0), H);
    const uint32_t s4 = S.ibl_sum[(int64_t)Y * (W + 1) + X];
    const float sr = (float)(int)(s4 & 1023u);
    const float sg = (float)(int)((s4 >> 10) & 1023u);
    const float sb = (float)(int)(s4 >> 20);
    const float w = 1.0f / 1020.0f;
    return rtm_scale(rtm_v3(sr * w, sg * w, sb * w), 1.0f);
}

template <bool COUNT>
__device__ __forceinline__ rtm_f3 sample_ibl_if(const DevScene& S, const LaunchConst& C, rtm_f3 dir, float power,
                                               Cnt& c) {
    if (power == 0.0f) return rtm_v3(0.0f, 0.0f, 0.0f);
    return sample_ibl<COUNT>(S, C, dir, c);
}

__device__ __forceinline__ rtm_f3 hemi_cosine(rtm_f3 n, float4 f0, float4 f1, float4 f2, uint32_t* s0,
                                              uint32_t* s1, float* invPdf) {
    const float u = rtm_rand(s0, s1);
    const float theta = rtm_rand(s0, s1) * 2.0f * 3.14f;
    const float r = dev_sqrt(u);
    float st, ct;
    rtm_sincos(theta, &st, &ct);
    const rtm_f3 localV = rtm_v3(r * ct, r * st, dev_sqrt(rtm_fmax(0.0f, 1.0f - u)));
    rtm_f3 l;
    if (f2.w != 0.0f) {
        l = rtm_scale(localV, n.z);
    } else {
// ... 755 lines not shown
```

### ensem3a_openclraytracer_amd/csrc/rt_internal.h

```cpp
#pragma once
#include <hip/hip_runtime.h>
#include <cstdint>

#include "rt_layout.h"
#include "rt_slices.h"

namespace rt {

struct DevScene {
    const float4* nodes;
    int32_t nnodes;
    int32_t root_ref;
    const float4* wnodes;
    const float4* wleaves;
    int32_t wroot_ref;
    float wdq_omax;
    float root_box[6];
    const float* bvh9;
    int32_t nbvh9;
    int32_t ref_stack;
    const float4* tri_geo;
    const float4* tri_fast;
    const float4* tri_shade;
    const float4* tri_frame;
    int32_t ntri;
    const float* mat;
    int32_t nmat;
    uint32_t near_mask_hi;
    const uint32_t* ibl_sum;
    int32_t ibl_w, ibl_h;
    int32_t depth;
    int32_t stack_lds;
    int2* stack_ovf;
    const float4* brute;
    int32_t nbrute;
    uint32_t near_mask_lo;
    const float4* brute_box;
    int32_t nbox;
    float near_floor;
    const float4* brute_cbox;
    const float4* brute_crow;
    int32_t ncluster, ncslot, nsingle4;
    int32_t cluster_auto;
    int32_t nsingle;
    int32_t shell;
};

struct FrameParams {
    float cam[10];
    float env[5];
    int32_t width;
    int64_t npix;
    int32_t spp;
    int32_t max_bounce;
    int32_t row0, row_step;
    int64_t nloc;
    int32_t resume_min;
    int32_t team;
    int32_t walk_team;
    int32_t max_waves;
    int32_t handout;
    int32_t step;
    int32_t sun_skip;
    int32_t sun_any;
    int32_t wide;
    int32_t wdq;
    int32_t fixed_point;
    int32_t sun_cache;
    int32_t pass;
    int32_t pilot;
    int32_t pilot_chunk;
    int32_t pilot_levels;
    float4* pilot_state;
    uint32_t* pilot_cost;
    uint32_t* pilot_draws;
    int32_t spec;
    int32_t refill;
    float4* spec_log;
    int32_t spec_cap;
    int32_t slices;
    float4* slice_state;
    uint32_t* slice_ready;
    const uint32_t* pilot_order;
    int64_t log_pixel;
    float* log_buf;
    int32_t log_cap;
    int32_t* log_count;
};

struct RenderPending {
    bool pick = false;
    int* host_pick = nullptr;
    FrameParams b{};
    bool spec_ok = false;
};
hipError_t launch_render(const DevScene& sc, const FrameParams& fp, int traversal, int block,
                         float* d_out, unsigned long long* d_counts, unsigned int* d_work, hipStream_t stream,
                         RenderPending* pend = nullptr);
hipError_t launch_render_finish(const DevScene& sc, int traversal, int block, float* d_out, unsigned int* d_work,
                                hipStream_t stream, RenderPending& pend);
hipError_t launch_accum(const DevScene& sc, const FrameParams& fp, float4* state, int base, int traversal, int block,
                        float* d_out, unsigned int* d_work, hipStream_t stream);
hipError_t launch_accum_listed(const DevScene& sc, const FrameParams& fp, float4* state, const uint32_t* list,
                               const uint32_t* count, int traversal, int block, float* d_out, unsigned int* d_work,
                               hipStream_t stream);
size_t select_scratch_words(int64_t n);
hipError_t launch_accum_mark(const float4* state, float4* mark, int64_t n, hipStream_t stream);
hipError_t launch_select_error(const float4* state, const float4* mark, uint8_t* flag, const FrameParams& fp,
                               float threshold, hipStream_t stream);
hipError_t launch_select_mask(const uint8_t* src, uint8_t* flag, const FrameParams& fp, hipStream_t stream);
hipError_t launch_select_compact(const uint8_t* flag, int64_t n, uint32_t* scratch, uint32_t* list, uint32_t* count,
                                 hipStream_t stream);
hipError_t launch_list_all(uint32_t* list, int64_t n, uint32_t* count, hipStream_t stream);
hipError_t launch_sample_map(const float4* state, int32_t* out, int64_t n, hipStream_t stream);
size_t launch_const_bytes();
hipError_t launch_accum_guides(const DevScene& sc, const FrameParams& fp, const float4* state, void* lconst,
                               float4* d_guides, hipStream_t stream);
size_t denoise_scratch_bytes(int64_t npix);
hipError_t launch_denoise(const float* d_rgb, const float4* d_guides, int64_t npix, int width, int passes, int nsq,
                          float sigma_c, float sigma_p, bool lds, float4* scratch, float* d_out,
                          hipStream_t stream);
hipError_t launch_accum_resolve(const float4* state, float* d_out, int64_t n, hipStream_t stream);
hipError_t launch_prep_frames(const DevScene& sc, float4* frame, hipStream_t stream);
hipError_t launch_ibl_sum(const uchar4* rgba, int w, int h, uint32_t* sum, hipStream_t stream);
hipError_t launch_gamma(const float* d_in, float* d_out, int64_t n, hipStream_t stream);
hipError_t launch_rgb8(const float* d_in, uint8_t* d_out, int64_t n, bool gamma, hipStream_t stream);
constexpr int kSpecTrails = 8;
constexpr int kSpecPick = 10;
constexpr int kSpecCapMax = 256;
constexpr int kWalkLanesPerCu = 4 * 4 * 64;
size_t spec_log_bytes(const FrameParams& fp, int cus);
hipError_t launch_spec(const DevScene& sc, const FrameParams& fp, int block, float* d_out, unsigned int* d_work,
                       hipStream_t stream);
constexpr int kRefillBrute = 4;
constexpr int kRefillMax = 64;
inline int brute_refill_launch(int option, int64_t nloc, int64_t lanes) {
    if (option >= 0) return option >= 2 ? (int)std::min<int64_t>(option, kRefillMax) : 0;
    return brute_auto_slices(nloc, lanes) ? kRefillBrute : 0;
}
struct KernelKey {
    int trav;
    int count;
    int log;
    int smem;
    int ovf;
    int resume;
    int step;
    int wide;
    int brute;
    int ts;
    int acc;
};
inline bool operator==(const KernelKey& a, const KernelKey& b) {
    return a.trav == b.trav && a.count == b.count && a.log == b.log && a.smem == b.smem && a.ovf == b.ovf &&
           a.resume == b.resume && a.step == b.step && a.wide == b.wide && a.brute == b.brute && a.ts == b.ts &&
           a.acc == b.acc;
}
KernelKey choose_kernel(const DevScene& sc, const FrameParams& fp, int traversal, bool count, bool log, int acc,
                        int block);
int64_t resident_blocks(const void* fn, int block, size_t lds, int max_waves, hipError_t* err);
struct QueryOptions {
    int engine;
    int grid_cap;
    int resume_min;
    int max_waves;
    int block;
};
hipError_t launch_query(const DevScene& sc, int traversal, int any, const float4* rays, float4* out, int64_t n,
                        const QueryOptions& q, unsigned int* counter, hipStream_t stream);
struct LaunchNote {
    KernelKey key;
    int team, walk_team, slices, refill;
    int64_t grid;
    size_t lds;
    int shell;
    int near;
};
void note_launch(const LaunchNote& n);
LaunchNote last_launch();
hipError_t launch_debug_math(int fn, const float* x, const float* y, float* out, int64_t n, hipStream_t stream);
hipError_t launch_debug_log(const DevScene& sc, const FrameParams& fp, int traversal, float* d_out,
                            unsigned int* d_work, hipStream_t stream);
hipError_t launch_debug_trace(const DevScene& sc, int traversal, const float* rays, float* out, int64_t n,
                              hipStream_t stream);
constexpr int kDebugFns = 9;
constexpr int debug_fn_in(int fn) {
    constexpr int w[kDebugFns] = {11, 5, 6, 13, 4, 24, 24, 12, 13};
    return fn >= 0 && fn < kDebugFns ? w[fn] : 0;
}
constexpr int debug_fn_out(int fn) {
    constexpr int w[kDebugFns] = {3, 3, 24, 3, 6, 2, 2, 1, 3};
    return fn >= 0 && fn < kDebugFns ? w[fn] : 0;
}
size_t debug_fn_scratch_bytes(int fn, int64_t n);
hipError_t launch_debug_fn(const DevScene& sc, int fn, const float* in, float* out, int64_t n, void* scratch,
                           hipStream_t stream);

}
```

### ensem3a_openclraytracer_amd/csrc/rt_kernels.hip

```cpp
#include <mutex>
#include <vector>

#include "rt_device.h"

namespace rt {

namespace {

__device__ __forceinline__ void save_state(float4* __restrict__ st, int p, rtm_f3 acc, float kc, uint32_t seed0,
                                           uint32_t seed1, int tc, int s) {
    st[2 * (int64_t)p] = make_float4(acc.x, acc.y, acc.z, kc);
    st[2 * (int64_t)p + 1] =
        make_float4(__uint_as_float(seed0), __uint_as_float(seed1), __int_as_float(tc), __int_as_float(s));
}

[[maybe_unused]] constexpr int kAccAdd = 1;
constexpr int kAccListed = 2;
constexpr int kBruteSliced = 4;
constexpr int kBruteRefill = 8;
template <int TRAV, bool COUNT, bool LOG = false, bool SMEM = false, bool OVF = false, int BRUTE_ = 0, int ACC = 0>
#ifndef RT_RENDER_WAVES
#define RT_RENDER_WAVES 5
#endif
__global__ void __launch_bounds__(256) __attribute__((amdgpu_waves_per_eu(RT_RENDER_WAVES))) render_kernel(DevScene S, FrameParams F, float* __restrict__ out,
                                               unsigned long long* __restrict__ counts,
                                               unsigned int* __restrict__ work_counter,
                                               const LaunchConst* __restrict__ lconst) {
    constexpr int BRUTE = BRUTE_ & 3;
    constexpr bool SLICED = (BRUTE_ & kBruteSliced) != 0;
    static_assert(!SLICED || BRUTE == 1 || BRUTE == 3, "sample slices: the one-lane brute-force loops");
    constexpr bool kRefill = (BRUTE == 1 || BRUTE == 3) && ((BRUTE_ & kBruteRefill) != 0 || COUNT || LOG);
    static_assert(!(BRUTE_ & kBruteRefill) || BRUTE == 1 || BRUTE == 3, "refill threshold: the one-lane brute-force loops");
    extern __shared__ int lds_stack[];
    const int B = blockDim.x;
    int* stk = lds_stack + threadIdx.x;
    const LaneStack lst = lane_stack(S, lds_stack);
    Cnt c{};
    const float4* mtrec = nullptr;
    const float4* boxrec = nullptr;
    const float4* tshade = S.tri_shade;
    const float4* tframe = S.tri_frame;
    const float* tmat = S.mat;
    if (BRUTE) {
        float4* lr = reinterpret_cast<float4*>(reinterpret_cast<char*>(lds_stack) + (B / 64) * BRUTE_WAVE_LDS);
        float4* lb = lr + 3 * S.nbrute;
        if (BRUTE == 2) {
            for (int q = threadIdx.x; q < 2 * S.nbox; q += B) lb[q] = S.brute_box[q];
            boxrec = lb;
        }
        float4* ls = lb + 2 * S.nbox;
        float4* lf = ls + S.ntri;
        float* lm = reinterpret_cast<float*>(lf + 3 * S.ntri);
        for (int q = threadIdx.x; q < 3 * S.nbrute; q += B) lr[q] = S.brute[4 * (q / 3) + 1 + q % 3];
        for (int q = threadIdx.x; q < S.ntri; q += B) ls[q] = S.tri_shade[q];
        for (int q = threadIdx.x; q < 3 * S.ntri; q += B) lf[q] = S.tri_frame[q];
        for (int q = threadIdx.x; q < kMatF * S.nmat; q += B) lm[q] = S.mat[q];
        if (BRUTE == 3) {
            float4* lc = reinterpret_cast<float4*>(lm + kMatF * S.nmat);
            for (int q = threadIdx.x; q < 2 * S.ncslot; q += B) lc[q] = S.brute_cbox[q];
            boxrec = lc;
        }
        __syncthreads();
        mtrec = lr;
        tshade = ls;
        tframe = lf;
        tmat = lm;
    }
    const LaunchConst& C = *lconst;
    const float4* nodes = S.nodes;
    const float4* tris = S.tri_fast;
    if (SMEM) {
        float4* ln = reinterpret_cast<float4*>(lds_stack + 2 * S.stack_lds * B);
        float4* lt = ln + kNodeF4 * S.nnodes;
        for (int q = threadIdx.x; q < kNodeF4 * S.nnodes; q += B)
            ln[(q % kNodeF4) * S.nnodes + q / kNodeF4] = S.nodes[q];
        for (int q = threadIdx.x; q < 3 * S.ntri; q += B) lt[q] = S.tri_fast[q];
        __syncthreads();
        nodes = ln;
        tris = lt;
    }
    const int W = F.width;
    const int imgSize = (int)F.npix;
    const float e3 = F.env[3], e4 = F.env[4];
    const int spp = F.spp, maxB = F.max_bounce;
    const unsigned int nloc = ACC == kAccListed ? (unsigned int)__builtin_amdgcn_readfirstlane((int)*F.pilot_cost)
                                                : (unsigned int)F.nloc;
    const int lane = threadIdx.x & 63;
    const int ts = BRUTE == 2 ? F.team : 1;
    const int team_lane0 = lane & ~(ts - 1);
    const bool team_leader = lane == team_lane0;
    const unsigned long long team_leaders = ts == 1 ? ~0ull : ts == 2 ? 0x5555555555555555ull
                                             : ts == 4 ? 0x1111111111111111ull : 0x0101010101010101ull;

    int phase = FETCH;
    PixelQueue pq;
    pq.per = (F.handout && F.pass != 2) ? (unsigned)(((ACC == kAccListed ? (int64_t)nloc : F.nloc) + kGroups - 1) / kGroups) : 0u;
    if constexpr (kRefill) pq.dry = F.refill > 1 ? (unsigned)min(F.refill, 64) << kQueueRefillShift : 0u;
    int p = 0, i = 0;
    bool logme = false;
    uint32_t seed0 = 0, seed1 = 0;
    rtm_f3 cd = rtm_v3(0, 0, 0);
    float kc = 1000.0f;
    int tc = -1;
    rtm_f3 so = rtm_v3(1, 1, 1);
    float k = 1000.0f;
    int tri = -1, j = 0;
    rtm_f3 Bo = rtm_v3(0, 0, 0), Bd = rtm_v3(0, 0, 0);
    rtm_f3 acc = rtm_v3(0, 0, 0);
    int s = 0;
    [[maybe_unused]] int plim = 0;
    auto slimit = [&]() __attribute__((always_inline)) { if constexpr (ACC == kAccListed) return plim; else return spp; };
    int cost = 0;
    int sun0 = -2;
    unsigned long long t_prev = 0;
    [[maybe_unused]] unsigned long long refill_ev = 0, refill_lanes = 0;
    auto save_pilot = [&]() __attribute__((always_inline)) {
        F.pilot_state[2 * (int64_t)p] = make_float4(acc.x, acc.y, acc.z, kc);
        F.pilot_state[2 * (int64_t)p + 1] =
            make_float4(__uint_as_float(seed0), __uint_as_float(seed1), __int_as_float(tc), __int_as_float(s));
        F.pilot_cost[p] = s >= spp ? 0u : (unsigned)cost;
    };

    const unsigned nsl = SLICED ? (unsigned)F.slices & 0xffu : 1u;
    const unsigned stail = SLICED ? (unsigned)F.slices >> 8 : 0u;
    const int sb = ACC ? F.pilot : 0;
    const unsigned sl_q = (unsigned)(spp - sb) / nsl, sl_r = (unsigned)(spp - sb) % nsl, sl_m = (65536u + nsl - 1u) / nsl;
    auto send = [&](unsigned k) { return sb + (int)((k + 1u) * sl_q + (((k + 1u) * sl_r * sl_m) >> 16)); };
    int lim = spp;
    auto save_slice = [&](rtm_f3 cdv) __attribute__((always_inline)) {
        slice_publish(F, (gu64*)(F.slice_state + 3 * (int64_t)p), p, acc, kc, seed0, seed1,
                      (unsigned)(tc + 1) | ((unsigned)(sun0 + 2) << 16), s, true, cdv);
    };

    while (true) {
        if (COUNT && lane == 0) {
            const unsigned long long now = clock64();
            if (t_prev) c.cyc_shade += now - t_prev;
            t_prev = now;
        }
        unsigned long long need = __ballot(phase == FETCH) & team_leaders;
        if constexpr (kRefill) {
            if (need && (unsigned)__popcll(need) < (pq.dry >> kQueueRefillShift)) {
// ... 872 lines not shown
hipError_t launch_prep_frames(const DevScene& sc, float4* frame, hipStream_t stream) {
    if (sc.ntri <= 0) return hipSuccess;
    hipLaunchKernelGGL(prep_frames_kernel, dim3((unsigned)((sc.ntri + 255) / 256)), dim3(256), 0, stream, sc.tri_shade,
                       sc.mat, sc.ntri, frame);
    return hipGetLastError();
}

hipError_t launch_debug_trace(const DevScene& sc, int traversal, const float* rays, float* out, int64_t n,
                              hipStream_t stream) {
    if (n <= 0) return hipSuccess;
    const int block = 128;
    DevScene s2 = sc;
    s2.stack_lds = sc.depth > 0 ? sc.depth : 1;
    s2.stack_ovf = nullptr;
    const size_t lds = stack_lds_bytes(s2, traversal == TRAV_REF ? TRAV_REF : TRAV_FAST, block);
    if (traversal == TRAV_REF)
        hipLaunchKernelGGL(debug_trace_kernel<TRAV_REF>, dim3((unsigned)((n + block - 1) / block)), dim3(block), lds,
                           stream, s2, rays, out, n);
    else
        hipLaunchKernelGGL(debug_trace_kernel<TRAV_FAST>, dim3((unsigned)((n + block - 1) / block)), dim3(block), lds,
                           stream, s2, rays, out, n);
    return hipGetLastError();
}

static bool stage_in_lds(const DevScene& sc) {
    const size_t scene_bytes = (size_t)(kNodeF4 * sc.nnodes + 3 * sc.ntri) * sizeof(float4);
    return sc.ntri > 0 && sc.nbrute == 0 && scene_bytes <= kLdsSceneMax && sc.stack_lds >= sc.depth;
}

KernelKey choose_kernel(const DevScene& sc, const FrameParams& fp, int traversal, bool count, bool log, int acc,
                        int block) {
    KernelKey k{traversal, count, log,  0,  0,  0,  1,  0,  0,  1, acc};
    if (traversal == TRAV_REF) return k;
    k.ovf = sc.nbrute == 0 && sc.stack_lds < sc.depth;
    if (log) return k;
    if (sc.ntri > 0 && sc.nbrute == 0 && fp.resume_min > 0) {
        k.resume = 1;
        if (fp.wide && sc.wnodes && !stage_in_lds(sc)) {
            const bool cam_in = std::fabs(fp.cam[0]) <= sc.wdq_omax && std::fabs(fp.cam[1]) <= sc.wdq_omax &&
                                std::fabs(fp.cam[2]) <= sc.wdq_omax;
            k.step = fp.step != 2;
            k.wide = (k.step && fp.wdq != 0 && sc.wdq_omax > 0.0f && cam_in) ? 2 : 1;
            return k;
        }
        k.step = fp.step == 1 || (fp.step == 0 && (size_t)sc.nnodes * kNodeF4 * 16 <= kStepMaxBytes);
        k.smem = stage_in_lds(sc);
        return k;
    }
    if (sc.ntri > 0 && sc.nbrute > 0 && brute_lds_bytes(sc, block) <= 80 * 1024) k.brute = 1;
    else k.smem = stage_in_lds(sc);
    return k;
}

#endif

namespace {
const void* kernel_fn(const KernelKey& k) {
    static const std::vector<KernelRow> table = [] {
        std::vector<KernelRow> t;
#ifndef RT_ACCUM_TU
        log_rows(t);
        head_rows<true>(t);
        head_rows<false>(t);
        engine_rows<true>(t);
#else
        head_rows<false>(t);
#endif
        engine_rows<false>(t);
        return t;
    }();
    for (const KernelRow& r : table)
        if (r.key == k) return r.fn;
    return nullptr;
}

hipError_t launch_pick(const DevScene& sc, const FrameParams& fp, KernelKey k, int block, float* d_out,
                       unsigned long long* d_counts, unsigned int* d_work, hipStream_t stream) {
    if (fp.nloc <= 0) return hipSuccess;
    const bool brute = k.brute != 0, product = !k.count && !k.log, listed = k.acc == kAccListed;
    const size_t lds = (brute ? brute_lds_bytes(sc, block) : stack_lds_bytes(sc, k.trav, block)) +
                       (k.smem ? staged_scene_bytes(sc) : 0);
    hipError_t e = hipSuccess;
    auto resident = [&](int max_waves) { return resident_blocks(kernel_fn(k), block, lds, max_waves, &e); };
    if (brute && product && sc.ncluster > 0 && !(sc.cluster_auto && fp.nloc < resident(0) * block)) k.brute = 3;
    const int64_t lanes = resident(fp.max_waves) * block;
    if (e != hipSuccess) return e;
    FrameParams f = fp;
    int bslices = 0;
    if (brute && !listed && fp.pass == 0 && fp.team <= 1 && fp.slice_state && fp.slice_ready &&
        sc.ntri + 2 < 65536 && fp.npix <= INT_MAX)
        bslices = brute_slice_launch(fp.slices, fp.nloc, lanes);
    if (!k.resume) f.slices = bslices;
    f.team = !brute ? 1 : bslices ? 1 : fp.team;
    if (f.team == 0) f.team = (!listed && fp.nloc * 4 <= lanes) ? 4 : 1;
    f.walk_team = 1;
    if (k.resume && k.step && !k.wide && !k.log) {
        f.walk_team = fp.walk_team ? fp.walk_team : listed ? 1 : auto_walk_team(fp.nloc, lanes);
        if (f.walk_team != 2 && f.walk_team != 4 && f.walk_team != 8) f.walk_team = 1;
    }
    f.refill = (brute && f.team <= 1) ? brute_refill_launch(fp.refill, fp.nloc, lanes) : 0;
    k.ts = f.walk_team;
    if (brute && f.team > 1) k.brute = 2;
    else if (brute) k.brute |= (bslices ? kBruteSliced : 0) | (product && f.refill > 1 ? kBruteRefill : 0);
    const void* fn = kernel_fn(k);
    const int64_t need = (fp.nloc * f.team * f.walk_team + block - 1) / block;
    const int64_t grid = std::min(need, resident(fp.max_waves));
    if (e != hipSuccess) return e;
    if (bslices) e = hipMemsetAsync(f.slice_ready, 0, (size_t)fp.nloc * sizeof(uint32_t), stream);
    const LaunchConst* lc = nullptr;
    if (e == hipSuccess) e = setup_work_block(f, d_work, stream, &lc);
    if (e != hipSuccess) return e;
    const int shell = (k.brute & 3) == 3 && sc.shell != 0;
    note_launch({k, f.team, f.walk_team, f.slices, f.refill, grid, lds, shell, shell && sc.near_floor != 0.0f});
    DevScene a0 = sc;
    void* args[] = {&a0, &f, &d_out, &d_counts, &d_work, &lc};
    return hipLaunchKernel(fn, dim3((unsigned)grid), dim3(block), args, lds, stream);
}

}

#ifndef RT_ACCUM_TU
hipError_t launch_debug_log(const DevScene& sc, const FrameParams& fp, int traversal, float* d_out,
                            unsigned int* d_work, hipStream_t stream) {
    return launch_pick(sc, fp, choose_kernel(sc, fp, traversal, false, true, 0, 64), 64, d_out, nullptr, d_work, stream);
}

constexpr int kCostBins = 256;

__global__ void pilot_chunk_kernel(const uint32_t* __restrict__ cost, int64_t nfull, int chunk,
                                   uint32_t* __restrict__ ccost) {
    for (int64_t c = (int64_t)blockIdx.x * blockDim.x + threadIdx.x; c < nfull; c += (int64_t)gridDim.x * blockDim.x) {
        uint32_t t = 0;
        for (int k = 0; k < chunk; ++k) t += cost[c * chunk + k];
        ccost[c] = t;
    }
}

__device__ __forceinline__ uint32_t cost_bin(uint32_t v, uint32_t scale, uint32_t maxbin) {
    return min(maxbin, (uint32_t)(((uint64_t)v * scale) >> 16));
}

constexpr int kSortSeg = kCostBins;

__global__ void pilot_seg_hist_kernel(const uint32_t* __restrict__ ccost, int64_t n, int64_t nseg, uint32_t scale,
                                      uint32_t maxbin, uint32_t* __restrict__ seghist) {
    __shared__ uint32_t h[kCostBins];
    const int64_t seg = blockIdx.x;
    h[threadIdx.x] = 0;
    __syncthreads();
    const int64_t q = seg * kSortSeg + threadIdx.x;
    if (q < n) atomicAdd(&h[cost_bin(ccost[q], scale, maxbin)], 1u);
    __syncthreads();
    seghist[threadIdx.x * nseg + seg] = h[threadIdx.x];
}

__global__ void pilot_seg_scan_kernel(uint32_t* __restrict__ seghist, int64_t nseg, uint32_t* __restrict__ total) {
    __shared__ uint32_t t[kCostBins];
    uint32_t* row = seghist + (int64_t)blockIdx.x * nseg;
    const int i0 = threadIdx.x;
    uint32_t carry = 0;
    for (int64_t base = 0; base < nseg; base += kCostBins) {
        const int64_t i = base + i0;
        const uint32_t v = i < nseg ? row[i] : 0u;
        t[i0] = v;
        __syncthreads();
        for (int off = 1; off < kCostBins; off <<= 1) {
            const uint32_t a = i0 >= off ? t[i0 - off] : 0u;
            __syncthreads();
            t[i0] += a;
            __syncthreads();
        }
        if (i < nseg) row[i] = carry + t[i0] - v;
        carry += t[kCostBins - 1];
        __syncthreads();
    }
    if (i0 == 0) total[blockIdx.x] = carry;
}

__global__ void pilot_scan_kernel(const uint32_t* __restrict__ hist, uint32_t* __restrict__ offs) {
    __shared__ uint32_t t[kCostBins];
    const int b = threadIdx.x;
    t[b] = hist[b];
    __syncthreads();
    uint32_t above = 0;
    for (int c = b + 1; c < kCostBins; ++c) above += t[c];
    offs[b] = above;
}

__global__ void pilot_seg_scatter_kernel(const uint32_t* __restrict__ ccost, int64_t n, int64_t nseg, uint32_t scale,
                                         uint32_t maxbin, const uint32_t* __restrict__ seghist,
                                         const uint32_t* __restrict__ offs, uint32_t* __restrict__ corder) {
    __shared__ uint32_t bins[kSortSeg];
    const int64_t seg = blockIdx.x;
    const int64_t q = seg * kSortSeg + threadIdx.x;
    const uint32_t b = q < n ? cost_bin(ccost[q], scale, maxbin) : 0xffffffffu;
    bins[threadIdx.x] = b;
// ... 341 lines not shown
```

### ensem3a_openclraytracer_amd/csrc/rt_layout.h

```cpp
#pragma once
#include <cstddef>
#include <cstdint>

namespace rt {

constexpr int kStackLds = 20;
constexpr int kStackLdsWide = 11;
#ifndef RT_WIDE_WAVES
#define RT_WIDE_WAVES 7
#endif
constexpr int kWideWaves = RT_WIDE_WAVES;
constexpr int kNodeF4 = 4;
constexpr int kMaxLanesPerCu = 2048;
#ifndef RT_BOX_GROUP
#define RT_BOX_GROUP 4
#endif
constexpr int kBoxGroup = RT_BOX_GROUP;
constexpr int kClusterShift = 3;
constexpr int kClusterSlots = 1 << kClusterShift;
constexpr double kClusterKappa = 1.9;
constexpr double kClusterGain = 0.75;
constexpr int kClusterLockNum = 4;
constexpr int kShellRecF = 20;
constexpr int kShellMinFaces = 3;
constexpr float kNearFloor = 0.0001f * (1.0f - 0x1p-12f);
constexpr double kNearKappa = 256.0;
constexpr int kNearExp = 40;
#ifndef RT_BRUTE_MAX_DEFAULT
#define RT_BRUTE_MAX_DEFAULT 64
#endif
constexpr int kMatF = 8;
constexpr size_t kWideMinBytes = 16u << 20;

constexpr int kGroups = 8;
constexpr int kCounterStride = 64;
constexpr int kTeamOffset = 512;
constexpr int kConstOffset = 1024;
constexpr int kWorkBytes = 2048;
constexpr int kChunkShift = 10;

}
```

### ensem3a_openclraytracer_amd/csrc/scene_pack.cpp

```cpp
#include "scene_pack.h"

#include <algorithm>
#include <array>
#include <cmath>
#include <cstdarg>
#include <cstdio>
#include <cstring>
#include <atomic>
#include <functional>
#include <map>
#include <mutex>
#include <new>
#include <stdexcept>
#include <string>
#include <system_error>
#include <thread>
#include <vector>

#include "../../include/rt_api.h"
#include "../../include/rt_debug.h"
#include "../../include/rt_scene.h"
#include "bvh_sah.h"

using rt::HostScene;
// ... 361 lines not shown
            for (int32_t g : mem)
                for (int k = 0; k < 6; ++k) take = take && std::isfinite(hs.brute_box[8 * (size_t)g + k]);
            if (take && mode < 0) {
                const double p = root > 0.0 && std::isfinite(root) ? std::min(1.0, area(i) / root) : 1.0;
                take = 1.0 + rt::kClusterKappa * p * rt::kClusterSlots < rt::kClusterGain * m;
            }
            if (take) {
                std::sort(mem.begin(), mem.end());
                clusters.push_back(mem);
                return;
            }
        }
        cut(st.L[i]);
        cut(st.R[i]);
    };
    cut(0);
    if (clusters.empty()) return;
    std::sort(singles.begin(), singles.end());
    std::sort(clusters.begin(), clusters.end());
    const size_t ns4 = (singles.size() + rt::kBoxGroup - 1) / rt::kBoxGroup * rt::kBoxGroup;
    const size_t nslot = ns4 + clusters.size() * rt::kClusterSlots;
    hs.brute_cbox.assign(8 * nslot, 0.0f);
    for (size_t s = 0; s < nslot; ++s) pad_box(hs.brute_cbox.data() + 8 * s);
    auto put = [&](size_t s, int32_t g) {
        std::memcpy(hs.brute_cbox.data() + 8 * s, hs.brute_box.data() + 8 * (size_t)g, 8 * sizeof(float));
    };
    for (size_t s = 0; s < singles.size(); ++s) put(s, singles[s]);
    hs.brute_crow.assign(8 * clusters.size(), 0.0f);
    for (size_t c = 0; c < clusters.size(); ++c) {
        const size_t first = ns4 + c * rt::kClusterSlots;
        float* r = hs.brute_crow.data() + 8 * c;
        for (size_t j = 0; j < clusters[c].size(); ++j) {
            put(first + j, clusters[c][j]);
            const float* b = hs.brute_box.data() + 8 * (size_t)clusters[c][j];
            for (int k = 0; k < 6; ++k)
                r[k] = j == 0 ? b[k] : (k & 1) ? std::max(r[k], b[k]) : std::min(r[k], b[k]);
        }
        for (int32_t g : clusters[c]) {
            const float* b = hs.brute_box.data() + 8 * (size_t)g;
            for (int a = 0; a < 3; ++a) {
                if (b[2 * a] != b[2 * a + 1]) continue;
                if (r[2 * a] == b[2 * a]) r[2 * a] = std::nextafterf(r[2 * a], -INFINITY);
                if (r[2 * a + 1] == b[2 * a]) r[2 * a + 1] = std::nextafterf(r[2 * a + 1], INFINITY);
            }
        }
        r[6] = as_f32((int32_t)first);
        r[7] = as_f32((int32_t)clusters[c].size());
    }
    hs.ncluster = (int32_t)clusters.size();
    hs.nsingle = (int32_t)singles.size();
}

bool near_safe(const HostScene& hs, const float* b) {
    int nf = 0, ax = -1;
    const double lim_lo = std::ldexp(1.0, -rt::kNearExp), lim_hi = std::ldexp(1.0, rt::kNearExp);
    auto in_range = [&](double v) { return v == 0.0 || (std::fabs(v) >= lim_lo && std::fabs(v) <= lim_hi); };
    for (int a = 0; a < 3; ++a) {
        if (!std::isfinite(b[2 * a]) || !std::isfinite(b[2 * a + 1])) return false;
        if (!in_range(b[2 * a]) || !in_range(b[2 * a + 1])) return false;
        if (b[2 * a] == b[2 * a + 1]) { ++nf; ax = a; }
        else if (!(b[2 * a] < b[2 * a + 1])) return false;
    }
    if (nf != 1) return false;
    const double h = b[2 * ax];
    const int u = (ax + 1) % 3, v = (ax + 2) % 3;
    int32_t q[2];
    std::memcpy(q, b + 6, 8);
    for (int j = 0; j < 2; ++j) {
        if (j == 1 && q[1] < 0) break;
        if (q[j] < 0 || q[j] >= hs.nbrute) return false;
        const float* r = hs.brute.data() + 16 * (size_t)q[j];
        const float *p0 = r + 6, *e1 = r + 9, *e2 = r + 12;
        for (int k = 0; k < 3; ++k)
            if (!std::isfinite(p0[k]) || !std::isfinite(e1[k]) || !std::isfinite(e2[k]) || !in_range(p0[k]) ||
                !in_range(e1[k]) || !in_range(e2[k]))
                return false;
        if ((double)p0[ax] != h || e1[ax] != 0.0f || e2[ax] != 0.0f) return false;
        const double t1 = (double)e1[u] * e2[v], t2 = (double)e1[v] * e2[u], N = t1 - t2;
        if (N == 0.0 || !((std::fabs(t1) + std::fabs(t2)) <= rt::kNearKappa * std::fabs(N))) return false;
    }
    return true;
}

void build_shell(HostScene& hs, int mode) {
    hs.brute_shell.clear();
    hs.nshell = 0;
    hs.nrest = 0;
    hs.shell_floor = 0.0f;
    hs.shell_mask = 0;
    if (mode == 0 || hs.ncluster == 0) return;
    const int32_t n = hs.nsingle;
    auto bits = [](float f) {
        uint32_t u;
        std::memcpy(&u, &f, 4);
        return u;
    };
    auto same = [&](float a, float b) { return bits(a) == bits(b); };
    auto box = [&](int32_t s) { return hs.brute_cbox.data() + 8 * (size_t)s; };
    std::vector<int> flat((size_t)n, -1);
    for (int32_t s = 0; s < n; ++s) {
        const float* b = box(s);
        int nf = 0, ax = -1;
        bool ok = true;
        for (int a = 0; a < 3; ++a) {
            ok = ok && std::isfinite(b[2 * a]) && std::isfinite(b[2 * a + 1]);
            if (same(b[2 * a], b[2 * a + 1])) { ++nf; ax = a; }
            else ok = ok && b[2 * a] < b[2 * a + 1];
        }
        if (ok && nf == 1) flat[s] = ax;
    }
    typedef std::array<uint32_t, 6> Key;
    std::map<Key, std::array<int32_t, 6>> shells;
    auto add_face = [&](std::array<int32_t, 6>& f, const float* S, int32_t s) {
        const int a = flat[s];
        const int pos = 2 * a + (same(box(s)[2 * a], S[2 * a]) ? 0 : 1);
        if (f[pos] < 0 || s < f[pos]) f[pos] = s;
    };
    for (int32_t s = 0; s < n; ++s) {
        if (flat[s] < 0) continue;
        for (int32_t t = s + 1; t < n; ++t) {
            if (flat[t] < 0) continue;
            const float *p = box(s), *q = box(t);
            const int a = flat[s], b = flat[t];
            float S[6];
            if (a == b) {
                bool ok = !same(p[2 * a], q[2 * a]);
                for (int k = 0; k < 3; ++k)
                    if (k != a) ok = ok && same(p[2 * k], q[2 * k]) && same(p[2 * k + 1], q[2 * k + 1]);
                if (!ok) continue;
                for (int k = 0; k < 6; ++k) S[k] = p[k];
                S[2 * a] = std::min(p[2 * a], q[2 * a]);
                S[2 * a + 1] = std::max(p[2 * a], q[2 * a]);
                if (!(S[2 * a] < S[2 * a + 1])) continue;
            } else {
                const int c = 3 - a - b;
                if (!(same(p[2 * a], q[2 * a]) || same(p[2 * a], q[2 * a + 1]))) continue;
                if (!(same(q[2 * b], p[2 * b]) || same(q[2 * b], p[2 * b + 1]))) continue;
                if (!(same(p[2 * c], q[2 * c]) && same(p[2 * c + 1], q[2 * c + 1]))) continue;
                S[2 * a] = q[2 * a]; S[2 * a + 1] = q[2 * a + 1];
                S[2 * b] = p[2 * b]; S[2 * b + 1] = p[2 * b + 1];
                S[2 * c] = p[2 * c]; S[2 * c + 1] = p[2 * c + 1];
            }
            Key key;
            for (int k = 0; k < 6; ++k) key[k] = bits(S[k]);
            auto it = shells.find(key);
            if (it == shells.end()) it = shells.emplace(key, std::array<int32_t, 6>{-1, -1, -1, -1, -1, -1}).first;
            add_face(it->second, S, s);
            add_face(it->second, S, t);
        }
    }
    const Key* best = nullptr;
    std::vector<int32_t> best_slots;
    for (const auto& kv : shells) {
        std::vector<int32_t> slots;
        for (int32_t s : kv.second)
            if (s >= 0) slots.push_back(s);
        std::sort(slots.begin(), slots.end());
        if (!best || slots.size() > best_slots.size() || (slots.size() == best_slots.size() && slots < best_slots)) {
            best = &kv.first;
            best_slots = slots;
        }
    }
    const int need = mode < 0 ? rt::kShellMinFaces : 2;
    if (!best || (int)best_slots.size() < need) return;
    const std::array<int32_t, 6>& face = shells[*best];
    const int32_t nrest = n - (int32_t)best_slots.size();
    const size_t nr4 = ((size_t)nrest + rt::kBoxGroup - 1) / rt::kBoxGroup * rt::kBoxGroup;
    hs.brute_shell.assign(rt::kShellRecF + 8 * nr4, 0.0f);
    float* r = hs.brute_shell.data();
    for (int k = 0; k < 6; ++k) std::memcpy(r + k, &(*best)[k], 4);
    r[6] = as_f32(nrest);
    r[7] = as_f32((int32_t)best_slots.size());
    for (int f = 0; f < 6; ++f) {
        r[8 + 2 * f] = face[f] < 0 ? as_f32(-1) : box(face[f])[6];
        r[9 + 2 * f] = face[f] < 0 ? as_f32(-1) : box(face[f])[7];
    }
    float* o = r + rt::kShellRecF;
    for (size_t s = 0; s < nr4; ++s) pad_box(o + 8 * s);
    for (int32_t s = 0; s < n; ++s)
        if (!std::binary_search(best_slots.begin(), best_slots.end(), s)) {
            std::memcpy(o, box(s), 8 * sizeof(float));
            o += 8;
        }
    hs.nshell = (int32_t)best_slots.size();
    hs.nrest = nrest;
    bool near = true;
    for (int32_t s : best_slots) near = near && near_safe(hs, box(s));
    hs.shell_floor = near ? rt::kNearFloor : 0.0f;
    for (int32_t s : best_slots)
        for (int32_t g = 0; g < hs.nbox && g < 64; ++g)
            if (as_i32(hs.brute_box[8 * (size_t)g + 6]) == as_i32(box(s)[6])) hs.shell_mask |= 1ull << g;
}

bool pack_fast(HostScene& hs, const float* bvh9, int64_t nn, int64_t ntri, int layout, int brute_max, int cluster,
               int shell, std::string& why) {
    if (nn <= 0) {
        why = "empty BVH";
        return false;
    }
    if (ntri > 0x7fffffff / 48) {
        why = "more than 44.7M triangles";
        return false;
    }
    std::vector<int32_t> L(nn), R(nn), T(nn);
    for (int64_t i = 0; i < nn; ++i) {
        if (!fidx(bvh9[9 * i + 0], nn, &L[i]) || !fidx(bvh9[9 * i + 1], nn, &R[i]) ||
            !fidx(bvh9[9 * i + 8], ntri, &T[i])) {
            why = "index out of range";
            return false;
        }
    }
    std::vector<uint8_t> seen(nn, 0);
    auto is_leaf = [&](int64_t i) { return L[i] == -1 && R[i] == -1 && T[i] >= 0; };
    auto is_inner = [&](int64_t i) { return L[i] >= 0 && R[i] >= 0 && T[i] == -1; };
    if (!is_leaf(0) && !is_inner(0)) {
        why = "root is neither a one-triangle leaf nor a two-child node";
        return false;
    }
    std::vector<int32_t> tri_seen(ntri, 0), leaves;
    std::vector<int32_t> queue{0};
    seen[0] = 1;
    for (size_t h = 0; h < queue.size(); ++h) {
        const int32_t n = queue[h];
        if (is_leaf(n)) {
            if (tri_seen[T[n]]++) {
                why = "triangle in two leaves";
                return false;
            }
            leaves.push_back(n);
            continue;
        }
        if (!is_inner(n)) {
            why = "node with one child, or with both a triangle and children";
            return false;
        }
        for (int32_t ch : {L[n], R[n]}) {
            if (seen[ch]) {
                why = "node reachable twice (not a tree)";
                return false;
            }
            seen[ch] = 1;
            queue.push_back(ch);
        }
    }
    std::vector<int32_t> rank(ntri, 0x7fffffff);
    {
        std::vector<int32_t> st;
        st.push_back(0);
        int32_t r = 0;
        while (!st.empty()) {
            const int32_t n = st.back();
            st.pop_back();
            if (T[n] >= 0) rank[T[n]] = r++;
            if (L[n] >= 0) st.push_back(L[n]);
            if (R[n] >= 0) st.push_back(R[n]);
        }
    }
    for (int64_t t = 0; t < ntri; ++t) {
        hs.tri_geo[12 * t + 3] = as_f32(rank[t]);
        hs.tri_geo[12 * t + 7] = as_f32((int32_t)t);
    }
    hs.brute.clear();
    hs.brute_box.clear();
    hs.nbrute = 0;
    hs.nbox = 0;
    hs.brute_cbox.clear();
    hs.brute_crow.clear();
    hs.ncluster = 0;
    hs.nsingle = 0;
    hs.brute_shell.clear();
    hs.nshell = 0;
    hs.nrest = 0;
    hs.brute_near.clear();
    hs.shell_floor = 0.0f;
    hs.shell_mask = 0;
    if ((int64_t)leaves.size() <= (int64_t)brute_max) {
        std::vector<int32_t> by_rank(leaves.size());
        for (int32_t n : leaves) by_rank[rank[T[n]]] = n;
        hs.brute.assign(16 * by_rank.size(), 0.0f);
        for (size_t q = 0; q < by_rank.size(); ++q) {
            const float* nd = bvh9 + 9 * (int64_t)by_rank[q];
            const int32_t t = T[by_rank[q]];
            const float* g = hs.tri_geo.data() + 12 * t;
            float* r = hs.brute.data() + 16 * q;
            r[0] = nd[2]; r[1] = nd[3]; r[2] = nd[4]; r[3] = nd[5];
            r[4] = nd[6]; r[5] = nd[7]; r[6] = g[0]; r[7] = g[1];
            r[8] = g[2]; r[9] = g[4]; r[10] = g[5]; r[11] = g[6];
            r[12] = g[8]; r[13] = g[9]; r[14] = g[10]; r[15] = as_f32(t);
        }
        hs.nbrute = (int32_t)by_rank.size();
        std::vector<std::array<int32_t, 2>> groups;
        {
            std::map<std::array<uint32_t, 6>, size_t> open;
            for (size_t q = 0; q < by_rank.size(); ++q) {
                const float* r = hs.brute.data() + 16 * q;
                std::array<uint32_t, 6> key;
                for (int k = 0; k < 6; ++k) std::memcpy(&key[k], r + k, 4);
                auto it = open.find(key);
                if (it != open.end()) {
                    groups[it->second][1] = (int32_t)q;
                    open.erase(it);
                } else {
                    open[key] = groups.size();
                    groups.push_back({(int32_t)q, -1});
                }
            }
        }
        hs.nbox = (int32_t)groups.size();
        const size_t ng = (groups.size() + rt::kBoxGroup - 1) / rt::kBoxGroup * rt::kBoxGroup;
        hs.brute_box.assign(8 * ng, 0.0f);
        for (size_t g = 0; g < ng; ++g) {
            float* b = hs.brute_box.data() + 8 * g;
            if (g < groups.size()) {
                const float* r = hs.brute.data() + 16 * groups[g][0];
                b[0] = r[0]; b[1] = r[3];
                b[2] = r[1]; b[3] = r[4];
                b[4] = r[2]; b[5] = r[5];
                b[6] = as_f32(groups[g][0]); b[7] = as_f32(groups[g][1]);
            } else {
                pad_box(b);
            }
        }
        hs.brute_near.assign((size_t)hs.nbox, 0);
        for (int32_t g = 0; g < hs.nbox; ++g) hs.brute_near[g] = near_safe(hs, hs.brute_box.data() + 8 * (size_t)g);
        build_clusters(hs, cluster);
        build_shell(hs, shell);
    }
    if (layout == RT_BVH_SAH && leaves.size() > 1) {
        std::vector<float> lb(6 * leaves.size());
        std::vector<int32_t> ids(leaves.size());
        for (size_t q = 0; q < leaves.size(); ++q) {
            const float* nd = bvh9 + 9 * (int64_t)leaves[q];
            for (int k = 0; k < 6; ++k) lb[6 * q + k] = nd[2 + k];
            ids[q] = T[leaves[q]];
        }
        rt::SahTree st;
        rt::sah_build(lb.data(), ids.data(), (int64_t)leaves.size(), st);
        emit_bvh(hs, st.L.data(), st.R.data(), st.leaf.data(), st.box.data(), (int64_t)st.L.size());
        return true;
    }
    std::vector<float> box(6 * nn);
    for (int64_t i = 0; i < nn; ++i)
        for (int k = 0; k < 6; ++k) box[6 * i + k] = bvh9[9 * i + 2 + k];
    emit_bvh(hs, L.data(), R.data(), T.data(), box.data(), nn);
    return true;
}

}

namespace rt {

void pack_checked(HostScene& hs, const float* bvh9, int64_t nb, int64_t ntri, int layout, int brute_max, int cluster,
                  int shell, std::string& why) {
    hs.fast_ok = (ntri > 0) ? pack_fast(hs, bvh9, nb, ntri, layout, brute_max, cluster, shell, why) : true;
    if (hs.fast_ok && ntri > 0) {
        double m1 = 0.0, m2 = 0.0;
        for (int64_t t = 0; t < ntri; ++t) {
            const float* g = hs.tri_geo.data() + 12 * t;
            const double l1 = std::sqrt((double)g[4] * g[4] + (double)g[5] * g[5] + (double)g[6] * g[6]);
            const double l2 = std::sqrt((double)g[8] * g[8] + (double)g[9] * g[9] + (double)g[10] * g[10]);
            if (std::isfinite(l1)) m1 = std::max(m1, l1);
            if (std::isfinite(l2)) m2 = std::max(m2, l2);
        }
        if (!(m1 * m2 <= std::ldexp(1.0, 120))) {
            hs.fast_ok = false;
            why = "triangle edges beyond 2^60 (the FAST reciprocal needs |e1 . (d x e2)| <= 2^126)";
        }
    }
    if (ntri == 0) {
        hs.nnodes = 0; hs.root_ref = 0; hs.depth = 1; hs.nodes.clear();
        hs.nwnodes = 0; hs.wroot_ref = 0; hs.wdepth = 1; hs.wnodes.clear(); hs.wleaves.clear();
        hs.brute.clear(); hs.brute_box.clear(); hs.nbrute = 0; hs.nbox = 0;
    }
    if (!hs.fast_ok) { hs.brute.clear(); hs.brute_box.clear(); hs.nbrute = 0; hs.nbox = 0; }
    if (hs.nbrute == 0) { hs.brute_cbox.clear(); hs.brute_crow.clear(); hs.ncluster = 0; hs.nsingle = 0; hs.brute_near.clear(); }
    if (hs.ncluster == 0) { hs.brute_shell.clear(); hs.nshell = 0; hs.nrest = 0; hs.shell_floor = 0.0f; hs.shell_mask = 0; }
    if (!hs.fast_ok || hs.wdepth > 64) { hs.wnodes.clear(); hs.wleaves.clear(); hs.nwnodes = 0; hs.wdepth = 1; }
    if (hs.fast_ok && hs.depth > 64) {
        hs.fast_ok = false;
        why = "tree deeper than 64 levels";
    }
    if (hs.nodes.empty()) hs.nodes.assign(4 * rt::kNodeF4, 0.0f);
    if (hs.brute.empty()) hs.brute.assign(16, 0.0f);
    if (hs.brute_box.empty()) {
        hs.brute_box.assign(8 * rt::kBoxGroup, 0.0f);
        for (int g = 0; g < rt::kBoxGroup; ++g) pad_box(hs.brute_box.data() + 8 * g);
    }
}

namespace {

int scene_prepare_(HostScene& hs, const float* vp, int64_t nvp, const float* vn, int64_t nvn, const int32_t* face,
                   int64_t nface, const float* mat, int64_t nmat, const float* bvh9, int64_t nbvh, int layout,
                   int brute_max, int cluster, int shell, std::string& msg, std::string& why) {
    if (nvp < 0 || nvp % 3 || nvn < 0 || nvn % 3 || nface < 0 || nface % 10 || nmat <= 0 || nmat % 6 || nbvh < 0 ||
        nbvh % 9)
        return fail(msg, RT_ERR_ARG,
                       "bad array sizes (V_p %lld, V_n %lld, faceData %lld, materialData %lld, BVH %lld)",
                       (long long)nvp, (long long)nvn, (long long)nface, (long long)nmat, (long long)nbvh);
    if ((nface && (!vp || !vn || !face)) || !mat || (nbvh && !bvh9))
        return fail(msg, RT_ERR_ARG, "null array");
    const int64_t T = nface / 10, NV = nvp / 3, NN = nvn / 3, M = nmat / 6, NB = nbvh / 9;
    if (T > 0x3fffffff || NB > 0x7fffffff) return fail(msg, RT_ERR_ARG, "scene too large");
    if (T > 0 && NB == 0) return fail(msg, RT_ERR_SCENE, "triangles given without a BVH");
    for (int64_t m = 0; m < M; ++m) {
        const float tf = mat[6 * m];
        if (!(tf > -1.0f && tf < 4.0f))
            return fail(msg, RT_ERR_SCENE, "material %lld has type %g; the kernel defines types 0..3", (long long)m,
                           (double)tf);
    }
    hs.ntri = (int32_t)T;
    hs.nmat = (int32_t)M;
    hs.nbvh9 = (int32_t)NB;
    hs.mat.assign((size_t)rt::kMatF * M, 0.0f);
    for (int64_t m = 0; m < M; ++m) {
        for (int k = 0; k < 6; ++k) hs.mat[(size_t)rt::kMatF * m + k] = mat[6 * m + k];
        for (int k = 1; k < 4; ++k) hs.colors_finite = hs.colors_finite && std::isfinite(mat[6 * m + k]);
        hs.has_glass = hs.has_glass || (int)mat[6 * m] == 3;
    }
    if (bvh9) hs.bvh9.assign(bvh9, bvh9 + nbvh);
    hs.tri_geo.assign((size_t)T * 12, 0.0f);
    hs.tri_shade.assign((size_t)T * 4, 0.0f);
    for (int64_t t = 0; t < T; ++t) {
        const int32_t* f = face + 10 * t;
        if (f[0] < 0 || f[0] >= M)
            return fail(msg, RT_ERR_ARG, "triangle %lld: material %d out of range [0,%lld)", (long long)t, f[0],
                           (long long)M);
        for (int j = 7; j < 10; ++j)
            if (f[j] < 0 || f[j] >= NV)
                return fail(msg, RT_ERR_ARG, "triangle %lld: position index %d out of range", (long long)t, f[j]);
        if (f[4] < 0 || f[4] >= NN)
            return fail(msg, RT_ERR_ARG, "triangle %lld: normal index %d out of range", (long long)t, f[4]);
        const float* a = vp + 3 * (int64_t)f[7];
        const float* b = vp + 3 * (int64_t)f[8];
        const float* c = vp + 3 * (int64_t)f[9];
        float* g = hs.tri_geo.data() + 12 * t;
        g[0] = a[0]; g[1] = a[1]; g[2] = a[2]; g[3] = 0.0f;
        g[4] = b[0] - a[0]; g[5] = b[1] - a[1]; g[6] = b[2] - a[2]; g[7] = 0.0f;
        g[8] = c[0] - a[0]; g[9] = c[1] - a[1]; g[10] = c[2] - a[2]; g[11] = 0.0f;
        const float* n = vn + 3 * (int64_t)f[4];
        float* sh = hs.tri_shade.data() + 4 * t;
        sh[0] = n[0]; sh[1] = n[1]; sh[2] = n[2]; sh[3] = as_f32(f[0]);
    }
    for (int64_t i = 0; i < NB; ++i) {
        int32_t l, r, t;
        if (!fidx(bvh9[9 * i + 0], NB, &l) || !fidx(bvh9[9 * i + 1], NB, &r) || !fidx(bvh9[9 * i + 8], T, &t))
            return fail(msg, RT_ERR_SCENE, "BVH node %lld has an index out of range", (long long)i);
    }
    if (NB > 0) {
        std::vector<uint8_t> color(NB, 0);
        std::vector<std::pair<int32_t, int>> st;
        st.push_back({0, 0});
        color[0] = 1;
        while (!st.empty()) {
            auto& top = st.back();
            const int32_t n = top.first;
            if (top.second < 2) {
                const int32_t ch = (int32_t)bvh9[9 * (int64_t)n + top.second];
                ++top.second;
                if (ch < 0) continue;
                if (color[ch] == 1) return fail(msg, RT_ERR_SCENE, "BVH node graph has a cycle through node %d", ch);
                if (color[ch] == 0) { color[ch] = 1; st.push_back({ch, 0}); }
            } else {
                color[n] = 2;
                st.pop_back();
            }
        }
    }
    pack_checked(hs, bvh9, NB, T, layout, brute_max, cluster, shell, why);
    return RT_OK;
}

}

int scene_prepare(HostScene& hs, const float* vp, int64_t nvp, const float* vn, int64_t nvn, const int32_t* face,
                  int64_t nface, const float* mat, int64_t nmat, const float* bvh9, int64_t nbvh, int layout,
                  int brute_max, int cluster, int shell, std::string& msg, std::string& why) {
    try {
        return scene_prepare_(hs, vp, nvp, vn, nvn, face, nface, mat, nmat, bvh9, nbvh, layout, brute_max, cluster, shell,
                              msg, why);
    } catch (const std::bad_alloc&) {
        hs = HostScene();
        return fail(msg, RT_ERR_ARG, "scene too large for host memory");
    } catch (const std::exception& e) {
        hs = HostScene();
        return fail(msg, RT_ERR_ARG, "scene preparation failed: %s", e.what());
    }
}

}

namespace {
thread_local std::string g_check_error;
}

extern "C" int rt_scene_check(const float* vp, int64_t nvp, const float* vn, int64_t nvn, const int32_t* face,
                              int64_t nface, const float* mat, int64_t nmat, const float* bvh9, int64_t nbvh,
                              int layout, int64_t info[8]) {
    HostScene hs;
    std::string msg, why;
    if (layout != RT_BVH_REFERENCE && layout != RT_BVH_SAH) {
        g_check_error = "layout must be RT_BVH_REFERENCE or RT_BVH_SAH";
        return RT_ERR_ARG;
    }
    const int rc = rt::scene_prepare(hs, vp, nvp, vn, nvn, face, nface, mat, nmat, bvh9, nbvh, layout,
                                     RT_BRUTE_MAX_DEFAULT, -1, -1, msg, why);
    g_check_error = rc != RT_OK ? msg : hs.fast_ok ? std::string() : "FAST traversal unavailable (" + why + ")";
    if (rc == RT_OK && info) {
        info[0] = hs.ntri;
        info[1] = hs.nnodes;
        info[2] = hs.depth;
        info[3] = hs.nwnodes;
        info[4] = hs.wdepth;
        info[5] = hs.nbrute;
        info[6] = hs.nbox;
        info[7] = hs.fast_ok ? 1 : 0;
    }
    return rc;
}

extern "C" const char* rt_scene_last_error(void) { return g_check_error.c_str(); }

extern "C" int rt_debug_brute_layout(const float* vp, int64_t nvp, const float* vn, int64_t nvn, const int32_t* face,
                                     int64_t nface, const float* mat, int64_t nmat, const float* bvh9, int64_t nbvh,
                                     int layout, float* boxes, int64_t cap, int64_t info[3]) {
    HostScene hs;
    std::string msg, why;
    if (layout != RT_BVH_REFERENCE && layout != RT_BVH_SAH) {
        g_check_error = "layout must be RT_BVH_REFERENCE or RT_BVH_SAH";
        return RT_ERR_ARG;
    }
    if (!info || cap < 0 || (cap > 0 && !boxes)) {
        g_check_error = "null info, or a box capacity without an array";
        return RT_ERR_ARG;
    }
    const int rc = rt::scene_prepare(hs, vp, nvp, vn, nvn, face, nface, mat, nmat, bvh9, nbvh, layout,
                                     RT_BRUTE_MAX_DEFAULT, -1, -1, msg, why);
    g_check_error = rc != RT_OK ? msg : hs.fast_ok ? std::string() : "FAST traversal unavailable (" + why + ")";
    if (rc != RT_OK) return rc;
    info[0] = hs.nbox;
    info[1] = hs.nbrute;
    info[2] = (int64_t)hs.brute_box.size();
    const int64_t n = std::min<int64_t>(cap, info[2]);
    if (n > 0) std::memcpy(boxes, hs.brute_box.data(), (size_t)n * sizeof(float));
    return RT_OK;
}

extern "C" int rt_debug_brute_clusters(const float* vp, int64_t nvp, const float* vn, int64_t nvn, const int32_t* face,
                                       int64_t nface, const float* mat, int64_t nmat, const float* bvh9, int64_t nbvh,
                                       int layout, int cluster, float* slots, int64_t slot_cap, float* rows,
                                       int64_t row_cap, int64_t info[4]) {
    HostScene hs;
    std::string msg, why;
    if (layout != RT_BVH_REFERENCE && layout != RT_BVH_SAH) {
        g_check_error = "layout must be RT_BVH_REFERENCE or RT_BVH_SAH";
        return RT_ERR_ARG;
    }
    if (cluster < -1 || cluster > 1) {
        g_check_error = "brute_cluster must be -1 (auto), 0 (off) or 1 (force)";
        return RT_ERR_ARG;
    }
    if (!info || slot_cap < 0 || row_cap < 0 || (slot_cap > 0 && !slots) || (row_cap > 0 && !rows)) {
        g_check_error = "null info, or a capacity without an array";
        return RT_ERR_ARG;
    }
    const int rc = rt::scene_prepare(hs, vp, nvp, vn, nvn, face, nface, mat, nmat, bvh9, nbvh, layout,
                                     RT_BRUTE_MAX_DEFAULT, cluster, -1, msg, why);
    g_check_error = rc != RT_OK ? msg : hs.fast_ok ? std::string() : "FAST traversal unavailable (" + why + ")";
    if (rc != RT_OK) return rc;
    info[0] = hs.ncluster;
    info[1] = hs.nsingle;
    info[2] = (int64_t)hs.brute_cbox.size();
    info[3] = (int64_t)hs.brute_crow.size();
    const int64_t ns = std::min<int64_t>(slot_cap, info[2]), nr = std::min<int64_t>(row_cap, info[3]);
    if (ns > 0) std::memcpy(slots, hs.brute_cbox.data(), (size_t)ns * sizeof(float));
    if (nr > 0) std::memcpy(rows, hs.brute_crow.data(), (size_t)nr * sizeof(float));
    return RT_OK;
}

extern "C" int rt_debug_brute_shell(const float* vp, int64_t nvp, const float* vn, int64_t nvn, const int32_t* face,
                                    int64_t nface, const float* mat, int64_t nmat, const float* bvh9, int64_t nbvh,
                                    int layout, int cluster, int shell, float* rec, int64_t cap, int64_t info[3]) {
    HostScene hs;
    std::string msg, why;
    if (layout != RT_BVH_REFERENCE && layout != RT_BVH_SAH) {
        g_check_error = "layout must be RT_BVH_REFERENCE or RT_BVH_SAH";
        return RT_ERR_ARG;
    }
    if (cluster < -1 || cluster > 1 || shell < -1 || shell > 1) {
        g_check_error = "brute_cluster and brute_shell must be -1 (auto), 0 (off) or 1 (force)";
        return RT_ERR_ARG;
    }
    if (!info || cap < 0 || (cap > 0 && !rec)) {
        g_check_error = "null info, or a capacity without an array";
        return RT_ERR_ARG;
    }
    const int rc = rt::scene_prepare(hs, vp, nvp, vn, nvn, face, nface, mat, nmat, bvh9, nbvh, layout,
                                     RT_BRUTE_MAX_DEFAULT, cluster, shell, msg, why);
    g_check_error = rc != RT_OK ? msg : hs.fast_ok ? std::string() : "FAST traversal unavailable (" + why + ")";
    if (rc != RT_OK) return rc;
    info[0] = hs.nshell;
    info[1] = hs.nrest;
    info[2] = (int64_t)hs.brute_shell.size();
    const int64_t n = std::min<int64_t>(cap, info[2]);
    if (n > 0) std::memcpy(rec, hs.brute_shell.data(), (size_t)n * sizeof(float));
    return RT_OK;
}

extern "C" int rt_debug_brute_near(const float* vp, int64_t nvp, const float* vn, int64_t nvn, const int32_t* face,
                                   int64_t nface, const float* mat, int64_t nmat, const float* bvh9, int64_t nbvh,
                                   int layout, int cluster, int shell, int32_t* flags, int64_t cap, float* floor,
                                   int64_t info[2]) {
    HostScene hs;
    std::string msg, why;
    if (layout != RT_BVH_REFERENCE && layout != RT_BVH_SAH) {
        g_check_error = "layout must be RT_BVH_REFERENCE or RT_BVH_SAH";
        return RT_ERR_ARG;
    }
    if (cluster < -1 || cluster > 1 || shell < -1 || shell > 1) {
        g_check_error = "brute_cluster and brute_shell must be -1 (auto), 0 (off) or 1 (force)";
        return RT_ERR_ARG;
    }
    if (!info || !floor || cap < 0 || (cap > 0 && !flags)) {
        g_check_error = "null info or floor, or a capacity without an array";
        return RT_ERR_ARG;
    }
    const int rc = rt::scene_prepare(hs, vp, nvp, vn, nvn, face, nface, mat, nmat, bvh9, nbvh, layout,
                                     RT_BRUTE_MAX_DEFAULT, cluster, shell, msg, why);
    g_check_error = rc != RT_OK ? msg : hs.fast_ok ? std::string() : "FAST traversal unavailable (" + why + ")";
    if (rc != RT_OK) return rc;
    info[0] = (int64_t)hs.brute_near.size();
    info[1] = hs.nshell;
    *floor = hs.shell_floor;
    const int64_t n = std::min<int64_t>(cap, info[0]);
    for (int64_t g = 0; g < n; ++g) flags[g] = hs.brute_near[(size_t)g];
    return RT_OK;
}
```

### ensem3a_openclraytracer_amd/csrc/scene_pack.h

```cpp
#pragma once
#include <cstdint>
#include <string>
#include <vector>

#include "rt_layout.h"

namespace rt {

struct HostScene {
    std::vector<float> nodes;
    std::vector<float> wnodes;
    std::vector<float> wleaves;
    int32_t nwnodes = 0, wroot_ref = 0, wdepth = 1;
    float wdq_omax = 0.0f;
    std::vector<float> bvh9;
    std::vector<float> tri_geo;
    std::vector<float> tri_fast;
    std::vector<float> tri_shade;
    std::vector<float> mat;
    std::vector<float> brute;
    std::vector<float> brute_box;
    int32_t nbrute = 0;
    int32_t nbox = 0;
    std::vector<float> brute_cbox;
    std::vector<float> brute_crow;
    int32_t ncluster = 0, nsingle = 0;
    std::vector<float> brute_shell;
    int32_t nshell = 0, nrest = 0;
    std::vector<uint8_t> brute_near;
    float shell_floor = 0.0f;
    uint64_t shell_mask = 0;
    int32_t nnodes = 0, root_ref = 0, ntri = 0, nmat = 0, nbvh9 = 0, depth = 1;
    float root_box[6] = {0, 0, 0, 0, 0, 0};
    bool fast_ok = false;
    bool colors_finite = true;
    bool has_glass = false;
};


int scene_prepare(HostScene& hs, const float* vp, int64_t nvp, const float* vn, int64_t nvn, const int32_t* face,
                  int64_t nface, const float* mat, int64_t nmat, const float* bvh9, int64_t nbvh, int layout,
                  int brute_max, int cluster, int shell, std::string& msg, std::string& why);

void pack_checked(HostScene& hs, const float* bvh9, int64_t nb, int64_t ntri, int layout, int brute_max, int cluster,
                  int shell, std::string& why);

}
```

### include/rt_debug.h

```cpp
#ifndef RT_DEBUG_H
#define RT_DEBUG_H

#include <stdint.h>
#include "rt_api.h"


#ifdef __cplusplus
extern "C" {
#endif

int rt_debug_math(rt_ctx* ctx, int fn, const float* x, const float* y, float* out, int64_t n);

int rt_debug_trace(rt_ctx* ctx, int traversal, const float* rays, float* out, int64_t n);

enum {
    RT_FN_CAMERA = 0, RT_FN_SUN = 1, RT_FN_HEMI = 2, RT_FN_GGX = 3, RT_FN_IBL = 4, RT_FN_MT_REF = 5,
    RT_FN_MT_FAST = 6, RT_FN_BOX_REF = 7, RT_FN_BOX_FAST = 8, RT_FN_COUNT = 9
};
int rt_debug_fn(rt_ctx* ctx, int fn, const float* in, float* out, int64_t n);

int rt_debug_pixel_log(rt_ctx* ctx, int traversal, const float cam[10], const float env[5], int64_t npix, int spp,
                       int max_bounce, int64_t pixel, float* log, int cap, int* n_events, float out3[3]);

int rt_debug_wave_counts(rt_ctx* ctx, const float cam[10], const float env[5], int64_t npix, int spp,
                         int max_bounce, uint64_t out[9]);

int rt_debug_scene_info(rt_ctx* ctx, int64_t out[8]);

int rt_debug_timings(rt_ctx* ctx, double out[4]);

int rt_debug_quantise_axis(float p, const float* lo, const float* hi, int n, float gap, uint8_t* qlo, uint8_t* qhi);

int rt_debug_brute_layout(const float* V_p, int64_t n_vp, const float* V_n, int64_t n_vn, const int32_t* faceData,
                          int64_t n_face, const float* materialData, int64_t n_mat, const float* bvh, int64_t n_bvh,
                          int layout, float* boxes, int64_t cap, int64_t info[3]);

int rt_debug_brute_clusters(const float* V_p, int64_t n_vp, const float* V_n, int64_t n_vn, const int32_t* faceData,
                            int64_t n_face, const float* materialData, int64_t n_mat, const float* bvh, int64_t n_bvh,
                            int layout, int cluster, float* slots, int64_t slot_cap, float* rows, int64_t row_cap,
                            int64_t info[4]);

int rt_debug_brute_shell(const float* V_p, int64_t n_vp, const float* V_n, int64_t n_vn, const int32_t* faceData,
                         int64_t n_face, const float* materialData, int64_t n_mat, const float* bvh, int64_t n_bvh,
                         int layout, int cluster, int shell, float* rec, int64_t cap, int64_t info[3]);

int rt_debug_brute_near(const float* V_p, int64_t n_vp, const float* V_n, int64_t n_vn, const int32_t* faceData,
                        int64_t n_face, const float* materialData, int64_t n_mat, const float* bvh, int64_t n_bvh,
                        int layout, int cluster, int shell, int32_t* flags, int64_t cap, float* floor, int64_t info[2]);

int rt_debug_brute_slices(int64_t nloc, int64_t lanes, int spp, int option, int accum_base, int32_t out[3]);

int rt_debug_last_slices(void);

int rt_debug_last_launch(int32_t out[19]);

int rt_debug_brute_refill(int64_t nloc, int64_t lanes, int option, int32_t* out);

int rt_debug_last_refill(int64_t out[3]);

#ifdef __cplusplus
}
#endif
#endif
```

Before: 11930 Msamples/s.

## Split shell faces into quads to pick a single brute record per ray

Adds a 'quad' refinement to the brute-force shell path. Each shell face is split by a plane line, so a ray entering through that face can be sent to just one of the two candidate triangle records instead of both, provided the guards (band, graze angle, direction magnitude) show the choice is safe. Shell rows are extended, staged into LDS, and the selection uses the v_max3/v_min3 instructions. The aim is fewer triangle tests per ray in the Cornell box. In exchange it adds per-ray plane evaluation, extra LDS, and a risk of correctness problems near the split line.

```diff
diff --git a/ensem3a_openclraytracer_amd/_native.py b/ensem3a_openclraytracer_amd/_native.py
--- a/ensem3a_openclraytracer_amd/_native.py
+++ b/ensem3a_openclraytracer_amd/_native.py
@@ -33,7 +33,8 @@
     "rt_trace", "rt_trace_device",
     "rt_bvh_build", "rt_device_count", "rt_debug_math", "rt_debug_fn", "rt_debug_trace", "rt_debug_scene_info", "rt_debug_pixel_log",
     "rt_debug_wave_counts", "rt_debug_quantise_axis", "rt_debug_timings", "rt_debug_brute_layout",
-    "rt_debug_brute_clusters", "rt_debug_brute_shell", "rt_debug_brute_near", "rt_debug_brute_slices",
+    "rt_debug_brute_clusters", "rt_debug_brute_shell", "rt_debug_brute_near", "rt_debug_brute_quad",
+    "rt_debug_brute_slices",
     "rt_debug_last_slices",
     "rt_debug_brute_refill", "rt_debug_last_refill", "rt_debug_last_launch",
     "rt_obj_parse", "rt_obj_size", "rt_obj_copy", "rt_obj_free", "rt_obj_last_error",
@@ -41,7 +42,7 @@
 )
 HOST_ONLY = ("rt_bvh_build", "rt_obj_parse", "rt_obj_size", "rt_obj_copy", "rt_obj_free", "rt_obj_last_error",
              "rt_scene_check", "rt_scene_last_error", "rt_debug_quantise_axis", "rt_debug_brute_layout",
-             "rt_debug_brute_clusters", "rt_debug_brute_shell", "rt_debug_brute_near")
+             "rt_debug_brute_clusters", "rt_debug_brute_shell", "rt_debug_brute_near", "rt_debug_brute_quad")
 
 _c_p = ctypes.c_void_p
 _i64 = ctypes.c_int64
@@ -171,6 +172,8 @@
                                             _c_p, _i64, _c_p]),
             "rt_debug_brute_near": (_i32, [_c_p, _i64, _c_p, _i64, _c_p, _i64, _c_p, _i64, _c_p, _i64, _i32, _i32, _i32,
                                            _c_p, _i64, _c_p, _c_p]),
+            "rt_debug_brute_quad": (_i32, [_c_p, _i64, _c_p, _i64, _c_p, _i64, _c_p, _i64, _c_p, _i64, _i32, _i32, _i32,
+                                           _i32, _c_p, _c_p, _c_p, _c_p, _c_p, _c_p]),
             "rt_debug_brute_slices": (_i32, [_i64, _i64, _i32, _i32, _i32, _c_p]),
             "rt_debug_last_slices": (_i32, []),
             "rt_debug_brute_refill": (_i32, [_i64, _i64, _i32, _c_p]),
@@ -623,7 +626,7 @@
     return slots.reshape(-1, 8), rows.reshape(-1, 8), int(info[1])
 
 
-SHELL_REC_FLOATS = 20
+SHELL_REC_FLOATS = 76
 
 
 def brute_shell(V_p, V_n, faceData, materialData, bvh, cluster: int = -1, shell: int = -1, layout: int = RT_BVH_SAH):
@@ -642,7 +645,7 @@
     if st != 0:
         raise NativeError(st, H.rt_scene_last_error().decode(errors="replace"))
     ints = rec[:SHELL_REC_FLOATS].view(np.int32)
-    return dict(box=rec[:6].copy(), nrest=int(ints[6]), nfaces=int(ints[7]), faces=ints[8:20].reshape(6, 2).copy(),
+    return dict(box=rec[:6].copy(), nrest=int(ints[6]), nfaces=int(ints[7]) & 0xff, faces=ints[8:20].reshape(6, 2).copy(),
                 rest=rec[SHELL_REC_FLOATS:].reshape(-1, 8).copy())
 
 
@@ -667,6 +670,25 @@
     return flags.astype(bool), np.float32(floor[0]), int(info[1])
 
 
+QUAD_BAND, QUAD_GRAZE, QUAD_DIR_MAX = np.float32(2.0 ** -8), np.float32(2.0 ** -6), np.float32(2.0)
+
+
+def brute_quad(V_p, V_n, faceData, materialData, bvh, cluster: int = -1, shell: int = -1, quad: int = -1,
+               layout: int = RT_BVH_SAH):
+    vp, vn, face, mat, b = f32(V_p), f32(V_n), i32(faceData), f32(materialData), f32(bvh)
+    flags, lines, words = np.zeros(6, np.int32), np.zeros(24, np.float32), np.zeros(18, np.int32)
+    recs, guard, info = np.zeros(108, np.float32), np.zeros(3, np.float32), np.zeros(2, np.int64)
+    st = host_lib().rt_debug_brute_quad(ptr(vp), vp.size, ptr(vn), vn.size, ptr(face), face.size, ptr(mat), mat.size,
+                                        ptr(b), b.size, int(layout), int(cluster), int(shell), int(quad),
+                                        flags.ctypes.data, lines.ctypes.data, words.ctypes.data, recs.ctypes.data,
+                                        guard.ctypes.data,
+                                        info.ctypes.data)
+    if st != 0:
+        raise NativeError(st, host_lib().rt_scene_last_error().decode(errors="replace"))
+    return dict(split=(flags & 1).astype(bool), side=((flags >> 1) & 1).astype(bool), lines=lines.reshape(6, 4),
+                words=words.view(np.uint32).reshape(6, 3), recs=recs.reshape(6, 2, 3, 3), guard=guard, nfaces=int(info[0]), nsplit=int(info[1]))
+
+
 def brute_slices(nloc: int, lanes: int, spp: int, option: int = -1, accum_base: int = -1):
     out = np.zeros(3, np.int32)
     st = lib().rt_debug_brute_slices(int(nloc), int(lanes), int(spp), int(option), int(accum_base), out.ctypes.data)
@@ -696,7 +718,7 @@
 
 
 LAUNCH_FIELDS = ("trav", "count", "log", "smem", "ovf", "resume", "step", "wide", "brute", "ts", "acc",
-                 "team", "walk_team", "slices", "refill", "grid", "lds", "shell", "near")
+                 "team", "walk_team", "slices", "refill", "grid", "lds", "shell", "near", "quad")
 BRUTE_SLICED = 4
 BRUTE_REFILL = 8
 
diff --git a/ensem3a_openclraytracer_amd/csrc/rt_api.hip b/ensem3a_openclraytracer_amd/csrc/rt_api.hip
--- a/ensem3a_openclraytracer_amd/csrc/rt_api.hip
+++ b/ensem3a_openclraytracer_amd/csrc/rt_api.hip
@@ -103,6 +103,7 @@
     int brute_cluster = -1;
     int brute_shell = -1;
     int brute_near = -1;
+    int brute_quad = -1;
     int resume_min = -1;
     int team = 0;
     int walk_team = 0;
@@ -275,7 +276,7 @@
     s.ncluster = ctx->hs.ncluster;
     s.ncslot = (int32_t)(ctx->hs.brute_cbox.size() / 8);
     s.nsingle4 = s.ncslot - rt::kClusterSlots * s.ncluster;
-    s.cluster_auto = ctx->brute_cluster < 0 ? 1 : 0;
+    s.host_flags = (ctx->brute_cluster < 0 ? rt::kHostClusterAuto : 0) | (ctx->hs.nquad > 0 ? rt::kHostQuad : 0);
     s.nsingle = ctx->hs.nsingle;
     s.shell = ctx->hs.nshell > 0 ? 2 * s.ncslot : 0;
     s.near_floor = s.shell && ctx->brute_near != 0 ? ctx->hs.shell_floor : 0.0f;
@@ -363,7 +364,7 @@
     HostScene& hs = ctx->hs;
     std::string why;
     rt::pack_checked(hs, hs.bvh9.data(), hs.nbvh9, hs.ntri, ctx->bvh_layout, ctx->brute_max, ctx->brute_cluster,
-                     ctx->brute_shell, why);
+                     ctx->brute_shell, ctx->brute_quad, why);
     for (auto& d : ctx->devs) {
         const int st = upload_fast(ctx, d, hs);
         if (st) return st;
@@ -411,6 +412,7 @@
     static const std::vector<Option> table = {
         {"traversal", &rt_ctx::traversal, range(RT_TRAVERSAL_FAST, RT_TRAVERSAL_REF), "traversal must be 0 (fast) or 1 (ref)", invalidate},
         {"brute_near", &rt_ctx::brute_near, range(-1, 1), "brute_near must be -1 (auto), 0 (off) or 1 (auto)", none},
+        {"brute_quad", &rt_ctx::brute_quad, range(-1, 1), "brute_quad must be -1 (auto), 0 (off) or 1 (auto)", repack},
         {"bvh", &rt_ctx::bvh_layout, range(RT_BVH_REFERENCE, RT_BVH_SAH), "bvh must be 0 (reference tree) or 1 (sah)", repack},
         {"brute_cluster", &rt_ctx::brute_cluster, range(-1, 1), "brute_cluster must be -1 (auto), 0 (off) or 1 (force)", repack},
         {"brute_shell", &rt_ctx::brute_shell, range(-1, 1), "brute_shell must be -1 (auto), 0 (off) or 1 (force)", repack},
@@ -521,7 +523,7 @@
     HostScene hs;
     std::string msg, why;
     const int rc = rt::scene_prepare(hs, vp, nvp, vn, nvn, face, nface, mat, nmat, bvh9, nbvh, ctx->bvh_layout,
-                                     ctx->brute_max, ctx->brute_cluster, ctx->brute_shell, msg, why);
+                                     ctx->brute_max, ctx->brute_cluster, ctx->brute_shell, ctx->brute_quad, msg, why);
     if (rc != RT_OK) return set_err(ctx, rc, "%s", msg.c_str());
     invalidate_accum(ctx);
     const auto t1 = std::chrono::steady_clock::now();
@@ -1661,14 +1663,14 @@
 
 int rt_debug_last_slices(void) { return rt::last_launch().slices; }
 
-int rt_debug_last_launch(int32_t out[19]) {
+int rt_debug_last_launch(int32_t out[20]) {
     if (!out) return RT_ERR_ARG;
     const rt::LaunchNote n = rt::last_launch();
     const rt::KernelKey& k = n.key;
-    const int64_t v[19] = {k.trav, k.count, k.log,  k.smem,       k.ovf,    k.resume, k.step, k.wide,          k.brute,
+    const int64_t v[20] = {k.trav, k.count, k.log,  k.smem,       k.ovf,    k.resume, k.step, k.wide,          k.brute,
                            k.ts,   k.acc,   n.team, n.walk_team,  n.slices, n.refill, n.grid, (int64_t)n.lds,
-                           n.shell, n.near};
-    for (int i = 0; i < 19; ++i) out[i] = (int32_t)std::min<int64_t>(v[i], INT32_MAX);
+                           n.shell, n.near, n.quad};
+    for (int i = 0; i < 20; ++i) out[i] = (int32_t)std::min<int64_t>(v[i], INT32_MAX);
     return RT_OK;
 }
 
diff --git a/ensem3a_openclraytracer_amd/csrc/rt_device.h b/ensem3a_openclraytracer_amd/csrc/rt_device.h
--- a/ensem3a_openclraytracer_amd/csrc/rt_device.h
+++ b/ensem3a_openclraytracer_amd/csrc/rt_device.h
@@ -367,6 +367,25 @@
 __device__ __forceinline__ float near_floor_of(const DevScene& S, int g) {
     const uint32_t m = g < 32 ? S.near_mask_lo : S.near_mask_hi;
     return g < 64 && ((m >> (g & 31)) & 1u) ? kNearFloor : 0.0f;
+}
+
+__device__ __forceinline__ float max3_f32(float a, float b, float c) {
+    float r;
+    asm("v_max3_f32 %0, %1, %2, %3" : "=v"(r) : "v"(a), "v"(b), "v"(c));
+    return r;
+}
+__device__ __forceinline__ float min3_f32(float a, float b, float c) {
+    float r;
+    asm("v_min3_f32 %0, %1, %2, %3" : "=v"(r) : "v"(a), "v"(b), "v"(c));
+    return r;
+}
+
+__device__ __forceinline__ unsigned quad_pick(float4 ln, float4 wd, rtm_f3 o, rtm_f3 d, float tin, float T, float da) {
+    const float sg = fmaf(ln.x, fmaf(T, d.x, o.x), fmaf(ln.y, fmaf(T, d.y, o.y), fmaf(ln.z, fmaf(T, d.z, o.z), ln.w)));
+    const float dm = fmaxf(fmaxf(fabsf(d.x), fabsf(d.y)), fabsf(d.z));
+    const bool sure = (tin <= 0.0f) & (T >= 0.0f) & (fabsf(da) >= kQuadGraze * dm) & (dm <= kQuadDirMax) &
+                      (fabsf(sg) >= kQuadBand);
+    return __float_as_uint(sure ? (sg >= 0.0f ? wd.y : wd.z) : wd.x);
 }
 
 template <int N> struct IntC { static constexpr int value = N; };
@@ -432,6 +451,7 @@
             bk = __uint_as_float((unsigned)(bestk[tl] >> 32));
         }
     };
+    unsigned cq_pk = 0;
     auto group = [&](auto wc, const ConstF4 cb, int g0, int nreal) __attribute__((always_inline)) {
         constexpr int W = decltype(wc)::value;
         float4 bx[2 * W];
@@ -456,7 +476,14 @@
                 count_wave(c.wave_trav); c.nodes++;
                 if (qb >= 0) { count_wave(c.wave_trav); c.nodes++; }
             }
-            enqueue(pass[j], (unsigned)qa, qb);
+            if constexpr (COUNT && !CLU) {
+                const unsigned keep = cq_pk & 0xffffu;
+                const bool one = pass[j] && qb >= 0 && cq_pk >= 0xffff0000u && (keep == (unsigned)qa || keep == (unsigned)qb);
+                enqueue(pass[j] && !one, (unsigned)qa, qb);
+                enqueue(one, keep, -1);
+            } else {
+                enqueue(pass[j], (unsigned)qa, qb);
+            }
         }
     };
     auto lockstep_padded = [&](const ConstF4 cb, int gb, int ge) __attribute__((always_inline)) {
@@ -481,6 +508,7 @@
         if (S.shell) {
             const ConstF4 sh{cb.p + 4 * S.shell};
             const float4 h0 = sgpr4(sh[0]), h1 = sgpr4(sh[1]), fx = sgpr4(sh[2]), fy = sgpr4(sh[3]), fz = sgpr4(sh[4]);
+            const int nquad = __float_as_int(h1.w) >> 8;
             const float cull = bk * CULL_MARGIN, nearf = S.near_floor;
             const float x0 = (h0.x - o.x) * ix, x1 = (h0.y - o.x) * ix;
             const float y0 = (h0.z - o.y) * iy, y1 = (h0.w - o.y) * iy;
@@ -508,9 +536,17 @@
                 npass += __popcll(mf);
             }
             if (npass == __popcll(many)) {
-                unsigned pk = ~0u;
+                int row = 2 * 6;
 #pragma unroll
-                for (int f = 0; f < 6; ++f) pk = pass[f] ? ((unsigned)q[2 * f] | ((unsigned)q[2 * f + 1] << 16)) : pk;
+                for (int f = 0; f < 6; ++f) row = pass[f] ? 2 * f : row;
+                const float4* rw = boxrec + S.shell + row;
+                unsigned pk;
+                if (nquad) {
+                    const float da = (pass[0] || pass[1]) ? d.x : (pass[2] || pass[3]) ? d.y : d.z;
+                    pk = quad_pick(rw[0], rw[1], o, d, max3_f32(mn[0], mn[1], mn[2]), min3_f32(mx[0], mx[1], mx[2]), da);
+                } else {
+                    pk = __float_as_uint(rw[1].x);
+                }
                 const bool p1 = pk != ~0u, p2 = pk < 0xffff0000u;
                 const unsigned long long m1 = __ballot(p1);
                 if (m1 != 0) {
@@ -590,6 +626,37 @@
         }
         while (itail != ihead) run_items(min((int)(itail - ihead), nact));
     } else if (ts == 1) {
+        if constexpr (COUNT) {
+            if (S.shell) {
+                const ConstF4 sh{as_const(S.brute_cbox).p + 4 * S.shell};
+                const float4 h0 = sgpr4(sh[0]), h1 = sgpr4(sh[1]);
+                const float cull = bk * CULL_MARGIN, nearf = S.near_floor;
+                const float x0 = (h0.x - o.x) * ix, x1 = (h0.y - o.x) * ix;
+                const float y0 = (h0.z - o.y) * iy, y1 = (h0.w - o.y) * iy;
+                const float z0 = (h1.x - o.z) * iz, z1 = (h1.y - o.z) * iz;
+                const float t[6] = {x0, x1, y0, y1, z0, z1};
+                const float mn[3] = {fminf(x0, x1), fminf(y0, y1), fminf(z0, z1)};
+                const float mx[3] = {fmaxf(x0, x1), fmaxf(y0, y1), fmaxf(z0, z1)};
+                unsigned long long many = 0;
+                int npass = 0, row = 2 * 6;
+                bool pass[6];
+                for (int f = 0; f < 6; ++f) {
+                    const int a = f >> 1;
+                    const float tn = fmaxf(fmaxf(a == 0 ? t[f] : mn[0], a == 1 ? t[f] : mn[1]), a == 2 ? t[f] : mn[2]);
+                    const float tx = fminf(fminf(a == 0 ? t[f] : mx[0], a == 1 ? t[f] : mx[1]), a == 2 ? t[f] : mx[2]);
+                    pass[f] = fmaxf(tn, nearf) <= fminf(tx, cull);
+                    const unsigned long long mf = __ballot(pass[f]);
+                    many |= mf;
+                    npass += __popcll(mf);
+                    row = pass[f] ? 2 * f : row;
+                }
+                if (npass == __popcll(many)) {
+                    const float4* rw = S.brute_cbox + S.shell + kShellRowF4 + row;
+                    const float da = (pass[0] || pass[1]) ? d.x : (pass[2] || pass[3]) ? d.y : d.z;
+                    cq_pk = quad_pick(rw[0], rw[1], o, d, max3_f32(mn[0], mn[1], mn[2]), min3_f32(mx[0], mx[1], mx[2]), da);
+                }
+            }
+        }
         lockstep_padded(as_const(S.brute_box), 0, S.nbox);
     } else {
         const int rounds = (S.nbox + ts - 1) / ts;
@@ -671,7 +738,8 @@
 }
 inline size_t brute_lds_bytes(const DevScene& sc, int block) {
     return (size_t)(block / 64) * BRUTE_WAVE_LDS + (size_t)sc.nbrute * 48 + (size_t)sc.nbox * 32 +
-           (size_t)sc.ntri * 64 + (size_t)sc.nmat * (4 * kMatF) + (size_t)sc.ncslot * 32;
+           (size_t)sc.ntri * 64 + (size_t)sc.nmat * (4 * kMatF) + (size_t)sc.ncslot * 32 +
+           (sc.shell ? (size_t)kShellRows * 32 : 0);
 }
 inline size_t staged_scene_bytes(const DevScene& sc) {
     return (size_t)(kNodeF4 * sc.nnodes + 3 * sc.ntri) * sizeof(float4);
diff --git a/ensem3a_openclraytracer_amd/csrc/rt_internal.h b/ensem3a_openclraytracer_amd/csrc/rt_internal.h
--- a/ensem3a_openclraytracer_amd/csrc/rt_internal.h
+++ b/ensem3a_openclraytracer_amd/csrc/rt_internal.h
@@ -7,6 +7,8 @@
 
 namespace rt {
 
+constexpr int32_t kHostClusterAuto = 1;
+constexpr int32_t kHostQuad = 2;
 struct DevScene {
     const float4* nodes;
     int32_t nnodes;
@@ -41,7 +43,7 @@
     const float4* brute_cbox;
     const float4* brute_crow;
     int32_t ncluster, ncslot, nsingle4;
-    int32_t cluster_auto;
+    int32_t host_flags;
     int32_t nsingle;
     int32_t shell;
 };
@@ -175,6 +177,7 @@
     size_t lds;
     int shell;
     int near;
+    int quad;
 };
 void note_launch(const LaunchNote& n);
 LaunchNote last_launch();
diff --git a/ensem3a_openclraytracer_amd/csrc/rt_kernels.hip b/ensem3a_openclraytracer_amd/csrc/rt_kernels.hip
--- a/ensem3a_openclraytracer_amd/csrc/rt_kernels.hip
+++ b/ensem3a_openclraytracer_amd/csrc/rt_kernels.hip
@@ -58,6 +58,8 @@
         if (BRUTE == 3) {
             float4* lc = reinterpret_cast<float4*>(lm + kMatF * S.nmat);
             for (int q = threadIdx.x; q < 2 * S.ncslot; q += B) lc[q] = S.brute_cbox[q];
+            if (S.shell)
+                for (int q = threadIdx.x; q < 2 * kShellRows; q += B) lc[S.shell + q] = S.brute_cbox[S.shell + kShellRowF4 + q];
             boxrec = lc;
         }
         __syncthreads();
@@ -1096,7 +1098,7 @@
                        (k.smem ? staged_scene_bytes(sc) : 0);
     hipError_t e = hipSuccess;
     auto resident = [&](int max_waves) { return resident_blocks(kernel_fn(k), block, lds, max_waves, &e); };
-    if (brute && product && sc.ncluster > 0 && !(sc.cluster_auto && fp.nloc < resident(0) * block)) k.brute = 3;
+    if (brute && product && sc.ncluster > 0 && !((sc.host_flags & kHostClusterAuto) && fp.nloc < resident(0) * block)) k.brute = 3;
     const int64_t lanes = resident(fp.max_waves) * block;
     if (e != hipSuccess) return e;
     FrameParams f = fp;
@@ -1125,7 +1127,8 @@
     if (e == hipSuccess) e = setup_work_block(f, d_work, stream, &lc);
     if (e != hipSuccess) return e;
     const int shell = (k.brute & 3) == 3 && sc.shell != 0;
-    note_launch({k, f.team, f.walk_team, f.slices, f.refill, grid, lds, shell, shell && sc.near_floor != 0.0f});
+    note_launch({k, f.team, f.walk_team, f.slices, f.refill, grid, lds, shell, shell && sc.near_floor != 0.0f,
+                 shell && (sc.host_flags & kHostQuad) != 0});
     DevScene a0 = sc;
     void* args[] = {&a0, &f, &d_out, &d_counts, &d_work, &lc};
     return hipLaunchKernel(fn, dim3((unsigned)grid), dim3(block), args, lds, stream);
diff --git a/ensem3a_openclraytracer_amd/csrc/rt_layout.h b/ensem3a_openclraytracer_amd/csrc/rt_layout.h
--- a/ensem3a_openclraytracer_amd/csrc/rt_layout.h
+++ b/ensem3a_openclraytracer_amd/csrc/rt_layout.h
@@ -21,8 +21,18 @@
 constexpr double kClusterKappa = 1.9;
 constexpr double kClusterGain = 0.75;
 constexpr int kClusterLockNum = 4;
-constexpr int kShellRecF = 20;
+constexpr int kShellRows = 7;
+constexpr int kShellRowF4 = 5;
+constexpr int kShellRecF = 20 + 8 * kShellRows;
 constexpr int kShellMinFaces = 3;
+constexpr float kQuadBand = 0x1p-8f;
+constexpr float kQuadGraze = 0x1p-6f;
+constexpr float kQuadDirMax = 2.0f;
+constexpr double kQuadSafety = 8.0;
+constexpr double kQuadSlack = 0x1p-20;
+constexpr double kQuadRatio = 4.0;
+constexpr double kQuadKappa = 4.0;
+constexpr int kQuadExp = 24;
 constexpr float kNearFloor = 0.0001f * (1.0f - 0x1p-12f);
 constexpr double kNearKappa = 256.0;
 constexpr int kNearExp = 40;
diff --git a/ensem3a_openclraytracer_amd/csrc/scene_pack.cpp b/ensem3a_openclraytracer_amd/csrc/scene_pack.cpp
--- a/ensem3a_openclraytracer_amd/csrc/scene_pack.cpp
+++ b/ensem3a_openclraytracer_amd/csrc/scene_pack.cpp
@@ -467,12 +467,111 @@
     return true;
 }
 
-void build_shell(HostScene& hs, int mode) {
+struct QuadLine { float A[3] = {0, 0, 0}; float gamma = 0; int side = 0; };
+bool quad_split(const HostScene& hs, const float* b, const float* S, QuadLine& out) {
+    if (!near_safe(hs, b)) return false;
+    int32_t q[2];
+    std::memcpy(q, b + 6, 8);
+    if (q[1] < 0) return false;
+    int a = 0;
+    for (int k = 0; k < 3; ++k) if (b[2 * k] == b[2 * k + 1]) a = k;
+    const int ax[2] = {(a + 1) % 3, (a + 2) % 3};
+    const double lo = std::ldexp(1.0, -rt::kQuadExp), hi = std::ldexp(1.0, rt::kQuadExp);
+    auto in_range = [&](double v) { return v == 0.0 || (std::fabs(v) >= lo && std::fabs(v) <= hi); };
+    for (int k = 0; k < 6; ++k) if (!in_range(S[k])) return false;
+    const double eps = std::ldexp(1.0, -24) * (1.0 + std::ldexp(1.0, -10));
+    double W[2], Cm[2], corner[4][2];
+    for (int j = 0; j < 2; ++j) {
+        W[j] = (double)S[2 * ax[j] + 1] - (double)S[2 * ax[j]];
+        Cm[j] = std::max(std::fabs((double)S[2 * ax[j]]), std::fabs((double)S[2 * ax[j] + 1]));
+    }
+    for (int c = 0; c < 4; ++c) {
+        corner[c][0] = S[2 * ax[0] + (c & 1)];
+        corner[c][1] = S[2 * ax[1] + (c >> 1)];
+    }
+    struct Coord { double g[2], c, err; };
+    Coord L[2][3];
+    double V[2][3][2];
+    for (int t = 0; t < 2; ++t) {
+        const float* r = hs.brute.data() + 16 * (size_t)q[t];
+        double p0[2], e1[2], e2[2];
+        for (int j = 0; j < 2; ++j) {
+            p0[j] = r[6 + ax[j]]; e1[j] = r[9 + ax[j]]; e2[j] = r[12 + ax[j]];
+            if (!in_range(p0[j]) || !in_range(e1[j]) || !in_range(e2[j])) return false;
+            const double s1 = p0[j] + e1[j], s2 = p0[j] + e2[j];
+            if (s1 - p0[j] != e1[j] || s1 - e1[j] != p0[j] || s2 - p0[j] != e2[j] || s2 - e2[j] != p0[j]) return false;
+            V[t][0][j] = p0[j]; V[t][1][j] = s1; V[t][2][j] = s2;
+        }
+        const double t1 = e1[0] * e2[1], t2 = e1[1] * e2[0], N = t1 - t2;
+        if (N == 0.0 || !((std::fabs(t1) + std::fabs(t2)) <= rt::kQuadKappa * std::fabs(N))) return false;
+        Coord& u = L[t][0]; Coord& v = L[t][1]; Coord& w = L[t][2];
+        u.g[0] = e2[1] / N; u.g[1] = -e2[0] / N; u.c = -(p0[0] * e2[1] - p0[1] * e2[0]) / N;
+        v.g[0] = -e1[1] / N; v.g[1] = e1[0] / N; v.c = -(e1[0] * p0[1] - e1[1] * p0[0]) / N;
+        w.g[0] = -u.g[0] - v.g[0]; w.g[1] = -u.g[1] - v.g[1]; w.c = 1.0 - u.c - v.c;
+        double mx[2] = {0.0, 0.0};
+        for (int k = 0; k < 2; ++k)
+            for (int c = 0; c < 4; ++c)
+                mx[k] = std::max(mx[k], std::fabs(L[t][k].g[0] * corner[c][0] + L[t][k].g[1] * corner[c][1] + L[t][k].c));
+        const double Qu = (W[0] * std::fabs(e2[1]) + W[1] * std::fabs(e2[0])) / std::fabs(N);
+        const double Qv = (W[0] * std::fabs(e1[1]) + W[1] * std::fabs(e1[0])) / std::fabs(N);
+        u.err = eps * (24.0 * mx[0] + 16.0 * Qu);
+        v.err = eps * (24.0 * mx[1] + 16.0 * Qv);
+        w.err = u.err + v.err + eps * (mx[0] + mx[1]);
+    }
+    auto at = [](const Coord& l, const double* P) { return l.g[0] * P[0] + l.g[1] * P[1] + l.c; };
+    for (int k1 = 0; k1 < 3; ++k1) {
+        const Coord& l1 = L[0][k1];
+        double mu = 0.0;
+        bool ok = true;
+        for (int j = 0; j < 3; ++j) {
+            const double x = at(l1, V[1][j]);
+            ok = ok && x <= rt::kQuadSlack;
+            mu = std::max(mu, -x);
+        }
+        if (!ok || !(mu > 0.0)) continue;
+        const double r1 = std::max(1.0, 1.0 / mu), r2 = std::max(1.0, mu);
+        if (!(r1 <= rt::kQuadRatio && r2 <= rt::kQuadRatio)) continue;
+        QuadLine ln;
+        ln.A[ax[0]] = (float)(r1 * l1.g[0]);
+        ln.A[ax[1]] = (float)(r1 * l1.g[1]);
+        ln.gamma = (float)(r1 * l1.c);
+        ln.side = 1;
+        for (int k = 0; k < 3; ++k) {
+            if (ln.A[k] == 0.0f) continue;
+            if (ln.A[k] < 0.0f) {
+                for (int m = 0; m < 3; ++m) ln.A[m] = -ln.A[m];
+                ln.gamma = -ln.gamma;
+                ln.side = 0;
+            }
+            break;
+        }
+        const double s = ln.side ? 1.0 : -1.0, A0 = ln.A[ax[0]], A1 = ln.A[ax[1]], G = ln.gamma;
+        auto sigma = [&](const double* P) { return A0 * P[0] + A1 * P[1] + G; };
+        for (int c = 0; c < 4; ++c) ok = ok && std::fabs(at(l1, corner[c]) - s * sigma(corner[c]) / r1) <= rt::kQuadSlack;
+        if (!ok) continue;
+        for (int k2 = 0; k2 < 3; ++k2) {
+            const Coord& l2 = L[1][k2];
+            bool ok2 = true;
+            for (int c = 0; c < 4; ++c) ok2 = ok2 && std::fabs(at(l2, corner[c]) + s * sigma(corner[c]) / r2) <= rt::kQuadSlack;
+            if (!ok2) continue;
+            const double Ms = std::fabs(A0) * Cm[0] + std::fabs(A1) * Cm[1] + std::fabs(G);
+            const double Ecls = eps * (std::fabs(A0) * (4.0 * W[0] + Cm[0]) + std::fabs(A1) * (4.0 * W[1] + Cm[1]) + 3.0 * Ms);
+            const double E = std::max(Ecls + r1 * (rt::kQuadSlack + l1.err), Ecls + r2 * (rt::kQuadSlack + l2.err));
+            if (!((double)rt::kQuadBand >= rt::kQuadSafety * E)) return false;
+            out = ln;
+            return true;
+        }
+    }
+    return false;
+}
+
+void build_shell(HostScene& hs, int mode, int quad) {
     hs.brute_shell.clear();
     hs.nshell = 0;
     hs.nrest = 0;
     hs.shell_floor = 0.0f;
     hs.shell_mask = 0;
+    hs.nquad = 0;
     if (mode == 0 || hs.ncluster == 0) return;
     const int32_t n = hs.nsingle;
     auto bits = [](float f) {
@@ -560,6 +659,28 @@
         r[8 + 2 * f] = face[f] < 0 ? as_f32(-1) : box(face[f])[6];
         r[9 + 2 * f] = face[f] < 0 ? as_f32(-1) : box(face[f])[7];
     }
+    float S6[6];
+    for (int k = 0; k < 6; ++k) std::memcpy(S6 + k, &(*best)[k], 4);
+    for (int f = 0; f < rt::kShellRows; ++f) {
+        float* row = r + 4 * rt::kShellRowF4 + 8 * f;
+        uint32_t both = ~0u, pos = ~0u, neg = ~0u, flags = 0;
+        if (f < 6 && face[f] >= 0) {
+            const uint32_t q0 = (uint32_t)as_i32(box(face[f])[6]), q1 = (uint32_t)as_i32(box(face[f])[7]);
+            both = pos = neg = (q0 & 0xffffu) | (q1 << 16);
+            QuadLine ln;
+            if (quad != 0 && q1 < 0xffffu && quad_split(hs, box(face[f]), S6, ln)) {
+                for (int k = 0; k < 3; ++k) row[k] = ln.A[k];
+                row[3] = ln.gamma;
+                pos = (ln.side ? q0 : q1) | 0xffff0000u;
+                neg = (ln.side ? q1 : q0) | 0xffff0000u;
+                flags = 1u | (ln.side ? 2u : 0u);
+                ++hs.nquad;
+            }
+        }
+        row[4] = as_f32((int32_t)both); row[5] = as_f32((int32_t)pos);
+        row[6] = as_f32((int32_t)neg); row[7] = as_f32((int32_t)flags);
+    }
+    r[7] = as_f32((int32_t)best_slots.size() | (hs.nquad << 8));
     float* o = r + rt::kShellRecF;
     for (size_t s = 0; s < nr4; ++s) pad_box(o + 8 * s);
     for (int32_t s = 0; s < n; ++s)
@@ -578,7 +699,7 @@
 }
 
 bool pack_fast(HostScene& hs, const float* bvh9, int64_t nn, int64_t ntri, int layout, int brute_max, int cluster,
-               int shell, std::string& why) {
+               int shell, int quad, std::string& why) {
     if (nn <= 0) {
         why = "empty BVH";
         return false;
@@ -659,6 +780,7 @@
     hs.brute_near.clear();
     hs.shell_floor = 0.0f;
     hs.shell_mask = 0;
+    hs.nquad = 0;
     if ((int64_t)leaves.size() <= (int64_t)brute_max) {
         std::vector<int32_t> by_rank(leaves.size());
         for (int32_t n : leaves) by_rank[rank[T[n]]] = n;
@@ -709,7 +831,7 @@
         hs.brute_near.assign((size_t)hs.nbox, 0);
         for (int32_t g = 0; g < hs.nbox; ++g) hs.brute_near[g] = near_safe(hs, hs.brute_box.data() + 8 * (size_t)g);
         build_clusters(hs, cluster);
-        build_shell(hs, shell);
+        build_shell(hs, shell, quad);
     }
     if (layout == RT_BVH_SAH && leaves.size() > 1) {
         std::vector<float> lb(6 * leaves.size());
@@ -736,8 +858,8 @@
 namespace rt {
 
 void pack_checked(HostScene& hs, const float* bvh9, int64_t nb, int64_t ntri, int layout, int brute_max, int cluster,
-                  int shell, std::string& why) {
-    hs.fast_ok = (ntri > 0) ? pack_fast(hs, bvh9, nb, ntri, layout, brute_max, cluster, shell, why) : true;
+                  int shell, int quad, std::string& why) {
+    hs.fast_ok = (ntri > 0) ? pack_fast(hs, bvh9, nb, ntri, layout, brute_max, cluster, shell, quad, why) : true;
     if (hs.fast_ok && ntri > 0) {
         double m1 = 0.0, m2 = 0.0;
         for (int64_t t = 0; t < ntri; ++t) {
@@ -759,7 +881,7 @@
     }
     if (!hs.fast_ok) { hs.brute.clear(); hs.brute_box.clear(); hs.nbrute = 0; hs.nbox = 0; }
     if (hs.nbrute == 0) { hs.brute_cbox.clear(); hs.brute_crow.clear(); hs.ncluster = 0; hs.nsingle = 0; hs.brute_near.clear(); }
-    if (hs.ncluster == 0) { hs.brute_shell.clear(); hs.nshell = 0; hs.nrest = 0; hs.shell_floor = 0.0f; hs.shell_mask = 0; }
+    if (hs.ncluster == 0) { hs.brute_shell.clear(); hs.nshell = 0; hs.nrest = 0; hs.shell_floor = 0.0f; hs.shell_mask = 0; hs.nquad = 0; }
     if (!hs.fast_ok || hs.wdepth > 64) { hs.wnodes.clear(); hs.wleaves.clear(); hs.nwnodes = 0; hs.wdepth = 1; }
     if (hs.fast_ok && hs.depth > 64) {
         hs.fast_ok = false;
@@ -777,7 +899,7 @@
 
 int scene_prepare_(HostScene& hs, const float* vp, int64_t nvp, const float* vn, int64_t nvn, const int32_t* face,
                    int64_t nface, const float* mat, int64_t nmat, const float* bvh9, int64_t nbvh, int layout,
-                   int brute_max, int cluster, int shell, std::string& msg, std::string& why) {
+                   int brute_max, int cluster, int shell, int quad, std::string& msg, std::string& why) {
     if (nvp < 0 || nvp % 3 || nvn < 0 || nvn % 3 || nface < 0 || nface % 10 || nmat <= 0 || nmat % 6 || nbvh < 0 ||
         nbvh % 9)
         return fail(msg, RT_ERR_ARG,
@@ -852,7 +974,7 @@
             }
         }
     }
-    pack_checked(hs, bvh9, NB, T, layout, brute_max, cluster, shell, why);
+    pack_checked(hs, bvh9, NB, T, layout, brute_max, cluster, shell, quad, why);
     return RT_OK;
 }
 
@@ -860,10 +982,10 @@
 
 int scene_prepare(HostScene& hs, const float* vp, int64_t nvp, const float* vn, int64_t nvn, const int32_t* face,
                   int64_t nface, const float* mat, int64_t nmat, const float* bvh9, int64_t nbvh, int layout,
-                  int brute_max, int cluster, int shell, std::string& msg, std::string& why) {
+                  int brute_max, int cluster, int shell, int quad, std::string& msg, std::string& why) {
     try {
         return scene_prepare_(hs, vp, nvp, vn, nvn, face, nface, mat, nmat, bvh9, nbvh, layout, brute_max, cluster, shell,
-                              msg, why);
+                              quad, msg, why);
     } catch (const std::bad_alloc&) {
         hs = HostScene();
         return fail(msg, RT_ERR_ARG, "scene too large for host memory");
@@ -889,7 +1011,7 @@
         return RT_ERR_ARG;
     }
     const int rc = rt::scene_prepare(hs, vp, nvp, vn, nvn, face, nface, mat, nmat, bvh9, nbvh, layout,
-                                     RT_BRUTE_MAX_DEFAULT, -1, -1, msg, why);
+                                     RT_BRUTE_MAX_DEFAULT, -1, -1, -1, msg, why);
     g_check_error = rc != RT_OK ? msg : hs.fast_ok ? std::string() : "FAST traversal unavailable (" + why + ")";
     if (rc == RT_OK && info) {
         info[0] = hs.ntri;
@@ -920,7 +1042,7 @@
         return RT_ERR_ARG;
     }
     const int rc = rt::scene_prepare(hs, vp, nvp, vn, nvn, face, nface, mat, nmat, bvh9, nbvh, layout,
-                                     RT_BRUTE_MAX_DEFAULT, -1, -1, msg, why);
+                                     RT_BRUTE_MAX_DEFAULT, -1, -1, -1, msg, why);
     g_check_error = rc != RT_OK ? msg : hs.fast_ok ? std::string() : "FAST traversal unavailable (" + why + ")";
     if (rc != RT_OK) return rc;
     info[0] = hs.nbox;
@@ -950,7 +1072,7 @@
         return RT_ERR_ARG;
     }
     const int rc = rt::scene_prepare(hs, vp, nvp, vn, nvn, face, nface, mat, nmat, bvh9, nbvh, layout,
-                                     RT_BRUTE_MAX_DEFAULT, cluster, -1, msg, why);
+                                     RT_BRUTE_MAX_DEFAULT, cluster, -1, -1, msg, why);
     g_check_error = rc != RT_OK ? msg : hs.fast_ok ? std::string() : "FAST traversal unavailable (" + why + ")";
     if (rc != RT_OK) return rc;
     info[0] = hs.ncluster;
@@ -981,7 +1103,7 @@
         return RT_ERR_ARG;
     }
     const int rc = rt::scene_prepare(hs, vp, nvp, vn, nvn, face, nface, mat, nmat, bvh9, nbvh, layout,
-                                     RT_BRUTE_MAX_DEFAULT, cluster, shell, msg, why);
+                                     RT_BRUTE_MAX_DEFAULT, cluster, shell, -1, msg, why);
     g_check_error = rc != RT_OK ? msg : hs.fast_ok ? std::string() : "FAST traversal unavailable (" + why + ")";
     if (rc != RT_OK) return rc;
     info[0] = hs.nshell;
@@ -1011,7 +1133,7 @@
         return RT_ERR_ARG;
     }
     const int rc = rt::scene_prepare(hs, vp, nvp, vn, nvn, face, nface, mat, nmat, bvh9, nbvh, layout,
-                                     RT_BRUTE_MAX_DEFAULT, cluster, shell, msg, why);
+                                     RT_BRUTE_MAX_DEFAULT, cluster, shell, -1, msg, why);
     g_check_error = rc != RT_OK ? msg : hs.fast_ok ? std::string() : "FAST traversal unavailable (" + why + ")";
     if (rc != RT_OK) return rc;
     info[0] = (int64_t)hs.brute_near.size();
@@ -1021,3 +1143,52 @@
     for (int64_t g = 0; g < n; ++g) flags[g] = hs.brute_near[(size_t)g];
     return RT_OK;
 }
+
+extern "C" int rt_debug_brute_quad(const float* vp, int64_t nvp, const float* vn, int64_t nvn, const int32_t* face,
+                                   int64_t nface, const float* mat, int64_t nmat, const float* bvh9, int64_t nbvh,
+                                   int layout, int cluster, int shell, int quad, int32_t flags[6], float lines[24],
+                                   int32_t words[18], float recs[108], float guard[3], int64_t info[2]) {
+    HostScene hs;
+    std::string msg, why;
+    if (layout != RT_BVH_REFERENCE && layout != RT_BVH_SAH) {
+        g_check_error = "layout must be RT_BVH_REFERENCE or RT_BVH_SAH";
+        return RT_ERR_ARG;
+    }
+    if (cluster < -1 || cluster > 1 || shell < -1 || shell > 1) {
+        g_check_error = "brute_cluster and brute_shell must be -1 (auto), 0 (off) or 1 (force)";
+        return RT_ERR_ARG;
+    }
+    if (quad < -1 || quad > 1) {
+        g_check_error = "brute_quad must be -1 (auto), 0 (off) or 1 (auto)";
+        return RT_ERR_ARG;
+    }
+    if (!info || !flags || !lines || !words || !recs || !guard) {
+        g_check_error = "null info, flags, lines, words, recs or guard";
+        return RT_ERR_ARG;
+    }
+    const int rc = rt::scene_prepare(hs, vp, nvp, vn, nvn, face, nface, mat, nmat, bvh9, nbvh, layout,
+                                     RT_BRUTE_MAX_DEFAULT, cluster, shell, quad, msg, why);
+    g_check_error = rc != RT_OK ? msg : hs.fast_ok ? std::string() : "FAST traversal unavailable (" + why + ")";
+    if (rc != RT_OK) return rc;
+    info[0] = hs.nshell;
+    info[1] = hs.nquad;
+    guard[0] = rt::kQuadBand; guard[1] = rt::kQuadGraze; guard[2] = rt::kQuadDirMax;
+    for (int f = 0; f < 6; ++f) {
+        flags[f] = 0;
+        for (int k = 0; k < 4; ++k) lines[4 * f + k] = 0.0f;
+        for (int k = 0; k < 3; ++k) words[3 * f + k] = -1;
+        for (int k = 0; k < 18; ++k) recs[18 * f + k] = 0.0f;
+        if (hs.nshell == 0) continue;
+        const float* row = hs.brute_shell.data() + 4 * rt::kShellRowF4 + 8 * f;
+        std::memcpy(lines + 4 * f, row, 16);
+        std::memcpy(words + 3 * f, row + 4, 12);
+        std::memcpy(flags + f, row + 7, 4);
+        const uint32_t both = (uint32_t)words[3 * f];
+        for (int j = 0; j < 2; ++j) {
+            const uint32_t q = j ? both >> 16 : both & 0xffffu;
+            if (both != ~0u && q != 0xffffu && (int32_t)q < hs.nbrute)
+                std::memcpy(recs + 18 * f + 9 * j, hs.brute.data() + 16 * (size_t)q + 6, 9 * sizeof(float));
+        }
+    }
+    return RT_OK;
+}
diff --git a/ensem3a_openclraytracer_amd/csrc/scene_pack.h b/ensem3a_openclraytracer_amd/csrc/scene_pack.h
--- a/ensem3a_openclraytracer_amd/csrc/scene_pack.h
+++ b/ensem3a_openclraytracer_amd/csrc/scene_pack.h
@@ -27,6 +27,7 @@
     int32_t ncluster = 0, nsingle = 0;
     std::vector<float> brute_shell;
     int32_t nshell = 0, nrest = 0;
+    int32_t nquad = 0;
     std::vector<uint8_t> brute_near;
     float shell_floor = 0.0f;
     uint64_t shell_mask = 0;
@@ -40,9 +41,9 @@
 
 int scene_prepare(HostScene& hs, const float* vp, int64_t nvp, const float* vn, int64_t nvn, const int32_t* face,
                   int64_t nface, const float* mat, int64_t nmat, const float* bvh9, int64_t nbvh, int layout,
-                  int brute_max, int cluster, int shell, std::string& msg, std::string& why);
+                  int brute_max, int cluster, int shell, int quad, std::string& msg, std::string& why);
 
 void pack_checked(HostScene& hs, const float* bvh9, int64_t nb, int64_t ntri, int layout, int brute_max, int cluster,
-                  int shell, std::string& why);
+                  int shell, int quad, std::string& why);
 
 }
diff --git a/include/rt_debug.h b/include/rt_debug.h
--- a/include/rt_debug.h
+++ b/include/rt_debug.h
@@ -48,11 +48,16 @@
                         int64_t n_face, const float* materialData, int64_t n_mat, const float* bvh, int64_t n_bvh,
                         int layout, int cluster, int shell, int32_t* flags, int64_t cap, float* floor, int64_t info[2]);
 
+int rt_debug_brute_quad(const float* V_p, int64_t n_vp, const float* V_n, int64_t n_vn, const int32_t* faceData,
+                        int64_t n_face, const float* materialData, int64_t n_mat, const float* bvh, int64_t n_bvh,
+                        int layout, int cluster, int shell, int quad, int32_t flags[6], float lines[24],
+                        int32_t words[18], float recs[108], float guard[3], int64_t info[2]);
+
 int rt_debug_brute_slices(int64_t nloc, int64_t lanes, int spp, int option, int accum_base, int32_t out[3]);
 
 int rt_debug_last_slices(void);
 
-int rt_debug_last_launch(int32_t out[19]);
+int rt_debug_last_launch(int32_t out[20]);
 
 int rt_debug_brute_refill(int64_t nloc, int64_t lanes, int option, int32_t* out);
 
```

Result: faster. 12130 Msamples/s (median of 6 runs) (+1.6%).
